# nh2/housescan

Hardware: AMD Instinct MI355X
Metric: frames/sec fused (640x480 into 512^3 TSDF): integrate+ICP+raycast (higher is better)
Workload: dtype f32 (int16 fixed-point TSDF storage, f64 ICP sums)

## Files before the change

### housescan_amd/_lib.py

```python
import ctypes as C
import importlib.util
import os
import sys

_HERE = os.path.dirname(os.path.abspath(__file__))
LIB_PATH = os.path.join(_HERE, "libhskinfu.so")

HSK_LEVELS = 3
HSK_NSTAGES = 4
HSK_KEY_NONE = 0x7FFFFFFF


class HskConfig(C.Structure):

    _fields_ = [
        ("vol_x", C.c_int), ("vol_y", C.c_int), ("vol_z", C.c_int),
        ("vol_size_m", C.c_float * 3),
        ("trunc_dist_m", C.c_float),
        ("width", C.c_int), ("height", C.c_int),
        ("fx", C.c_float), ("fy", C.c_float), ("cx", C.c_float), ("cy", C.c_float),
        ("icp_iters", C.c_int * HSK_LEVELS),
        ("icp_dist_thresh_m", C.c_float),
        ("icp_angle_thresh_sin", C.c_float),
        ("integrate_move_thresh", C.c_float),
# ... 35 lines not shown
        ("clip", (C.c_float * 4) * HSK_MAX_CLIP),
        ("cut_rgb", C.c_uint8 * 3),
    ]


class HskFuseStats(C.Structure):

    _fields_ = [
        ("n_fused", C.c_uint64), ("n_colored", C.c_uint64),
        ("chunks_total", C.c_uint64), ("chunks_swept", C.c_uint64),
        ("box", C.c_int32 * 6),
    ]


HSK_ALIGN_CONVERGED, HSK_ALIGN_MAX_ITERS, HSK_ALIGN_FEW, HSK_ALIGN_DEGENERATE, HSK_ALIGN_DIVERGED = 0, 1, 2, 3, 4
HSK_ALIGN_STATUS = ("converged", "max_iters", "few", "degenerate", "diverged")
HSK_ALIGN_MAX_ITERS_CAP = 64
HSK_ALIGN_DIRECT = -1


class HskAlignParams(C.Structure):

    _fields_ = [
        ("max_iters", C.c_int), ("probes", C.c_int),
        ("cos_gate", C.c_float),
        ("max_points", C.c_uint32), ("min_points", C.c_uint32),
        ("eps_rot", C.c_float), ("eps_trans_m", C.c_float), ("max_rot", C.c_float), ("max_shift_m", C.c_float),
    ]


class HskAlignStats(C.Structure):

    _fields_ = [
        ("status", C.c_int), ("iterations", C.c_int),
        ("n_points", C.c_uint32), ("stride", C.c_uint32),
        ("n_used", C.c_uint32 * HSK_ALIGN_MAX_ITERS_CAP),
        ("rms_m", C.c_float * HSK_ALIGN_MAX_ITERS_CAP),
        ("x_last", C.c_float * 6),
        ("sums_last", C.c_double * 28),
    ]


class HskVolumeInfo(C.Structure):

    _fields_ = [
        ("version", C.c_uint32), ("header_bytes", C.c_uint32), ("flags", C.c_uint32),
        ("dims", C.c_int32 * 3), ("z0", C.c_int32), ("nz", C.c_int32),
        ("size_m", C.c_float * 3),
        ("trunc_dist_m", C.c_float), ("trunc_eff_m", C.c_float),
        ("width", C.c_int32), ("height", C.c_int32),
        ("fx", C.c_float), ("fy", C.c_float), ("cx", C.c_float), ("cy", C.c_float),
        ("pose", C.c_float * 16),
        ("frame", C.c_int32),
        ("color_max_weight", C.c_int32), ("color_band_m", C.c_float),
        ("n_bricks", C.c_uint64),
        ("tsdf_bricks", C.c_uint64 * 4), ("color_bricks", C.c_uint64 * 2),
        ("tsdf_table_bytes", C.c_uint64), ("tsdf_payload_bytes", C.c_uint64),
        ("color_table_bytes", C.c_uint64), ("color_payload_bytes", C.c_uint64),
        ("total_bytes", C.c_uint64),
        ("pass_reused", C.c_int32),
    ]


_P = C.c_void_p
_F = C.POINTER(C.c_float)
_D = C.POINTER(C.c_double)
_I = C.POINTER(C.c_int)
SYMBOLS = {
    "hsk_build_id": (C.c_char_p, []),
    "hsk_default_config": (None, [C.POINTER(HskConfig), C.c_int]),
    "hsk_create": (C.c_int, [C.POINTER(HskConfig), C.POINTER(_P)]),
    "hsk_destroy": (None, [_P]),
    "hsk_reset": (C.c_int, [_P]),
    "hsk_last_error": (C.c_char_p, [_P]),
    "hsk_process_frame": (C.c_int, [_P, _P, C.c_int, C.c_int, _F, _I]),
    "hsk_process_frame_dev": (C.c_int, [_P, _P, C.c_int, C.c_int, _F, _I]),
    "hsk_submit_frame_dev": (C.c_int, [_P, _P, C.c_int, C.c_int]),
    "hsk_submit_frame": (C.c_int, [_P, _P, C.c_int, C.c_int]),
    "hsk_wait_frame": (C.c_int, [_P, _F, _I]),
    "hsk_integrate": (C.c_int, [_P, _P, C.c_int, C.c_int, _F]),
    "hsk_raycast": (C.c_int, [_P, _F, _P, _P, _P]),
    "hsk_preprocess": (C.c_int, [_P, _P, C.c_int, C.c_int]),
    "hsk_icp_accumulate": (C.c_int, [_P, C.c_int, _F, C.c_int, C.c_int, _D]),
    "hsk_icp_solve": (C.c_int, [_D, _F, _I]),
    "hsk_count_updates": (C.c_int, [_P, _P, C.c_int, C.c_int, _F, C.POINTER(C.c_uint64)]),
    "hsk_download_tsdf": (C.c_int, [_P, _P]),
    "hsk_upload_tsdf": (C.c_int, [_P, _P]),
    "hsk_flush_weights": (C.c_int, [_P]),
    "hsk_prepare_readout": (C.c_int, [_P, C.c_size_t]),
    "hsk_stored_planes": (C.c_int, [_P, _I, _I]),
    "hsk_get_pose": (C.c_int, [_P, _F]),
    "hsk_set_pose": (C.c_int, [_P, _F]),
    "hsk_download_map": (C.c_int, [_P, C.c_int, C.c_int, _P]),
    "hsk_upload_map": (C.c_int, [_P, C.c_int, C.c_int, _P]),
    "hsk_download_depth_level": (C.c_int, [_P, C.c_int, _P]),
    "hsk_download_scaled_depth": (C.c_int, [_P, _P]),
    "hsk_extract_cloud": (C.c_int, [_P, _P, C.c_size_t, C.POINTER(C.c_size_t)]),
    "hsk_extract_mesh": (C.c_int, [_P, _P, C.c_size_t, C.POINTER(C.c_size_t)]),
    "hsk_extract_mesh_cubes": (C.c_int, [_P, _P, C.c_size_t, C.POINTER(C.c_size_t)]),
    "hsk_enable_color": (C.c_int, [_P, C.c_int, C.c_float]),
    "hsk_process_frame_rgbd": (C.c_int, [_P, _P, _P, C.c_int, C.c_int, _F, _I]),
    "hsk_submit_frame_rgbd": (C.c_int, [_P, _P, _P, C.c_int, C.c_int]),
    "hsk_integrate_color": (C.c_int, [_P, _P, _P, C.c_int, C.c_int, _F]),
    "hsk_download_color": (C.c_int, [_P, _P]),
    "hsk_upload_color": (C.c_int, [_P, _P]),
    "hsk_extract_cloud_attrs": (C.c_int, [_P, _P, _P, _P, C.c_size_t, C.POINTER(C.c_size_t), C.POINTER(C.c_size_t)]),
    "hsk_extract_mesh_indexed": (C.c_int, [_P, _P, _P, _P, C.c_size_t, C.POINTER(C.c_size_t), _P, C.c_size_t, C.POINTER(C.c_size_t),
                                            C.POINTER(C.c_size_t)]),
    "hsk_default_view": (None, [_P, C.POINTER(HskView)]),
    "hsk_render_view": (C.c_int, [_P, C.POINTER(HskView), _P, _P, _P, _P, C.POINTER(C.c_size_t), C.POINTER(C.c_size_t)]),
    "hsk_default_section": (None, [_P, C.POINTER(HskSection)]),
    "hsk_render_section": (C.c_int, [_P, C.POINTER(HskSection), _P, _P, _P, _P, C.POINTER(C.c_size_t), C.POINTER(C.c_size_t),
                                      C.POINTER(C.c_size_t)]),
    "hsk_section_in_room": (C.c_int, [C.POINTER(HskSection), _F, C.POINTER(HskSection)]),
    "hsk_composite_views": (C.c_int, [C.c_int, C.POINTER(_P), C.POINTER(_P), C.c_int, C.c_int, _P, _P, _P, _P]),
    "hsk_fuse_volume": (C.c_int, [_P, _P, _F, C.POINTER(HskFuseStats)]),
    "hsk_pack_volume": (C.c_int, [_P, _P, C.c_size_t, C.POINTER(C.c_size_t), C.POINTER(HskVolumeInfo)]),
    "hsk_unpack_volume": (C.c_int, [_P, _P, C.c_size_t]),
    "hsk_save_volume": (C.c_int, [_P, C.c_char_p, C.POINTER(HskVolumeInfo)]),
    "hsk_load_volume": (C.c_int, [_P, C.c_char_p]),
    "hsk_volume_image_info": (C.c_int, [_P, C.c_size_t, C.POINTER(HskVolumeInfo)]),
    "hsk_volume_file_info": (C.c_int, [C.c_char_p, C.POINTER(HskVolumeInfo)]),
    "hsk_config_from_volume": (C.c_int, [C.POINTER(HskVolumeInfo), C.POINTER(HskConfig)]),
    "hsk_resume_scan": (C.c_int, [_P, _F]),
    "hsk_default_align_params": (None, [_P, C.POINTER(HskAlignParams)]),
    "hsk_align_cloud": (C.c_int, [_P, _P, _P, C.c_size_t, _F, C.POINTER(HskAlignParams), _F, C.POINTER(HskAlignStats)]),
    "hsk_align_volume": (C.c_int, [_P, _P, _F, C.POINTER(HskAlignParams), _F, C.POINTER(HskAlignStats)]),
    "hsk_align_step": (C.c_int, [_D, _F, _F, _F, _F, _I]),
    "hsk_invert_rigid": (C.c_int, [_F, _F]),
    "hsk_fuse_footprint": (C.c_int, [_I, _F, _I, _F, _F, C.POINTER(C.c_int32)]),
    "hsk_write_ppm": (C.c_int, [C.c_char_p, _P, C.c_int, C.c_int]),
    "hsk_write_pgm16": (C.c_int, [C.c_char_p, _P, C.c_int, C.c_int]),
    "hsk_mgpu_frame_begin": (C.c_int, [_P, _P, C.c_int, C.c_int]),
    "hsk_mgpu_prefetch": (C.c_int, [_P, _P, C.c_int, C.c_int]),
    "hsk_mgpu_frame_front": (C.c_int, [_P, _P, C.c_int, C.c_int, _P]),
    "hsk_mgpu_icp_accumulate": (C.c_int, [_P, C.c_int, C.c_int, C.c_int, _P]),
    "hsk_mgpu_icp_update": (C.c_int, [_P, _P]),
    "hsk_mgpu_icp_replicated": (C.c_int, [_P]),
    "hsk_mgpu_integrate": (C.c_int, [_P]),
    "hsk_mgpu_raycast_local": (C.c_int, [_P, _P]),
    "hsk_mgpu_raycast_resolve": (C.c_int, [_P, _P, _P]),
    "hsk_mgpu_raycast_push": (C.c_int, [_P, _P, C.POINTER(_P), C.c_int]),
    "hsk_mgpu_frame_end": (C.c_int, [_P, _P, _P, _F, _I]),
    "hsk_mgpu_frame_index": (C.c_int, [_P]),
    "hsk_mgpu_frame_end_async": (C.c_int, [_P, _P, _P]),
    "hsk_mgpu_restart_pending": (C.c_int, [_P]),
    "hsk_stream": (_P, [_P]),
    "hsk_set_stream": (C.c_int, [_P, _P]),
    "hsk_synchronize": (C.c_int, [_P]),
    "hsk_set_profiling": (C.c_int, [_P, C.c_int]),
    "hsk_stage_ms": (C.c_int, [_P, _D, C.POINTER(C.c_uint64), C.c_int]),
    "hsk_icp_level_ms": (C.c_int, [_P, _D]),
    "hsk_submit_host_us": (C.c_int, [_P, _D, C.POINTER(C.c_uint64), C.c_int]),
    "hsk_integrate_queue_entries": (C.c_int, [_P, C.POINTER(C.c_uint64)]),
    "hsk_integrate_light_entries": (C.c_int, [_P, C.POINTER(C.c_uint64)]),
    "hsk_integrate_coarse_counts": (C.c_int, [_P, C.POINTER(C.c_uint64)]),
    "hsk_bilateral_tables": (C.c_int, [_F, _F]),
    "hsk_selftest_exact_ops": (C.c_int, [C.c_int, C.POINTER(C.c_uint64)]),
    "hsk_group_create": (C.c_int, [C.POINTER(HskConfig), C.c_int, _I, C.c_int, C.POINTER(_P)]),
    "hsk_group_unique_id": (C.c_int, [_P]),
    "hsk_group_create_rank": (C.c_int, [C.POINTER(HskConfig), C.c_int, C.c_int, _P, C.c_int, C.POINTER(_P)]),
    "hsk_group_destroy": (None, [_P]),
    "hsk_group_last_error": (C.c_char_p, [_P]),
    "hsk_group_reset": (C.c_int, [_P]),
    "hsk_group_process_frame": (C.c_int, [_P, _P, C.c_int, C.c_int, _F, _I]),
    "hsk_group_submit_frame": (C.c_int, [_P, _P, C.c_int, C.c_int]),
    "hsk_group_submit_frame_dev": (C.c_int, [_P, C.POINTER(_P), C.c_int, C.c_int]),
    "hsk_group_wait_frame": (C.c_int, [_P, _F, _I]),
    "hsk_group_exchange_ms": (C.c_int, [_P, _D, _D, C.POINTER(C.c_ulonglong)]),
    "hsk_group_n_slabs": (C.c_int, [_P]),
    "hsk_group_ranks_seen": (C.c_int, [_P, _I]),
    "hsk_group_slab": (_P, [_P, C.c_int]),
    "hsk_group_download_tsdf": (C.c_int, [_P, _P]),
    "hsk_synth_pose": (C.c_int, [C.c_int, _F]),
    "hsk_synth_render": (C.c_int, [_F, C.c_int, C.c_int, C.c_float, C.c_float, C.c_float, C.c_float, _P]),
    "hsk_synth_room_extents": (C.c_int, [C.c_int, _F]),
    "hsk_synth_room_pose": (C.c_int, [C.c_int, C.c_int, C.c_int, _F]),
    "hsk_synth_room_render": (C.c_int, [C.c_int, _F, C.c_int, C.c_int, C.c_float, C.c_float, C.c_float, C.c_float, _P]),
    "hsk_synth_render_sensor": (C.c_int, [C.c_int, _F, C.c_int, C.c_int, C.c_float, C.c_float, C.c_float, C.c_float, C.c_uint64, C.c_float, C.c_float, C.c_int, _P, _D]),
    "hsk_synth_color_at": (C.c_int, [C.c_int, _F, _P]),
    "hsk_synth_render_rgb": (C.c_int, [C.c_int, _F, C.c_int, C.c_int, C.c_float, C.c_float, C.c_float, C.c_float, _P]),
    "hsk_write_pcd_xyz": (C.c_int, [C.c_char_p, _P, C.c_size_t]),
    "hsk_write_ply_mesh": (C.c_int, [C.c_char_p, _P, C.c_size_t, C.POINTER(C.c_size_t), C.POINTER(C.c_size_t)]),
    "hsk_weld_triangles": (C.c_int, [_P, C.c_size_t, _P, C.c_size_t, C.POINTER(C.c_size_t), _P]),
    "hsk_write_ply_indexed": (C.c_int, [C.c_char_p, _P, _P, _P, C.c_size_t, _P, C.c_size_t]),
    "hsk_voxel_downsample": (C.c_int, [_P, C.c_size_t, C.c_float, _P, C.c_size_t, C.POINTER(C.c_size_t)]),
    "hsk_voxel_downsample_attrs": (C.c_int, [_P, _P, _P, C.c_size_t, C.c_float, _P, _P, _P, C.c_size_t, C.POINTER(C.c_size_t)]),
    "hsk_write_pcd_xyzrgbnormal": (C.c_int, [C.c_char_p, _P, _P, _P, C.c_size_t]),
    "hsk_detect_planes": (C.c_int, [_P, C.c_size_t, C.c_float, C.c_float, C.c_int, C.c_int, _P, _P, _I]),
    "hsk_plane_hull": (C.c_int, [_P, C.c_size_t, _P, C.c_int, _F, _P, C.c_size_t, C.POINTER(C.c_size_t)]),
    "hsk_write_planes_txt": (C.c_int, [C.c_char_p, _P, C.c_int]),
    "hsk_write_xf": (C.c_int, [C.c_char_p, _F]),
    "hsk_read_xf": (C.c_int, [C.c_char_p, _F]),
    "hsk_transform_cloud": (C.c_int, [_P, C.c_size_t, _F, _P]),
    "hsk_transform_normals": (C.c_int, [_P, C.c_size_t, _F, _P]),
    "hsk_stream_create": (_P, [C.c_char_p, C.c_int, C.c_int, C.c_float, C.c_float, C.c_float, C.c_float]),
    "hsk_stream_open": (_P, [C.c_char_p, _I, _I, _I, _F]),
    "hsk_stream_write": (C.c_int, [_P, _P]),
    "hsk_stream_read": (C.c_int, [_P, C.c_int, _P]),
    "hsk_stream_close": (C.c_int, [_P]),
    "hsk_stream_info": (C.c_int, [_P, _I, _I, _I, _F]),
    "hsk_track_stream": (C.c_int, [_P, _P, C.c_int, C.c_int, _F, _I]),
}

_U32 = C.POINTER(C.c_uint32)
_SZ = C.POINTER(C.c_size_t)
HSH_OBJECTIVE = C.CFUNCTYPE(C.c_double, _D, C.c_int, _P)
HOUSE_SYMBOLS = {
    "hsh_create": (_P, []),
    "hsh_destroy": (None, [_P]),
    "hsh_last_error": (C.c_char_p, [_P]),
    "hsh_load_room": (C.c_int, [_P, C.c_char_p, _U32]),
    "hsh_add_room": (C.c_int, [_P, C.c_char_p, _P, C.c_size_t, _P, C.c_int, _P, _P, _U32]),
    "hsh_room_ids": (C.c_int, [_P, _P, C.c_int, _I]),
    "hsh_room_planes": (C.c_int, [_P, C.c_uint32, _P, _P, C.c_int, _I]),
    "hsh_plane_bounds": (C.c_int, [_P, C.c_uint32, _P, C.c_int, _I]),
    "hsh_room_corners": (C.c_int, [_P, C.c_uint32, C.c_int, _P, _P, C.c_int, _I]),
    "hsh_room_cloud": (C.c_int, [_P, C.c_uint32, _P, C.c_size_t, _SZ]),
    "hsh_room_means": (C.c_int, [_P, C.c_uint32, _P, _P]),
    "hsh_set_room_corners": (C.c_int, [_P, C.c_uint32, _P, C.c_int]),
    "hsh_accept_corner_suggestion": (C.c_int, [_P, C.c_uint32, C.c_uint32]),
    "hsh_translate_room": (C.c_int, [_P, C.c_uint32, _P]),
    "hsh_rotate_room": (C.c_int, [_P, C.c_uint32, _P]),
    "hsh_rotate_kinfu_room": (C.c_int, [_P, C.c_uint32]),
    "hsh_room_auto_align_axis": (C.c_int, [_P, C.c_uint32, _P]),
    "hsh_auto_align_floor": (C.c_int, [_P, C.c_uint32]),
    "hsh_remove_ceiling": (C.c_int, [_P, C.c_uint32]),
    "hsh_suggest_points": (C.c_int, [_P, C.c_uint32, C.c_float, _I, _I]),
    "hsh_fit_cuboid_to_room": (C.c_int, [_P, C.c_uint32, C.c_int, _I, _D, _D]),
    "hsh_connect_walls": (C.c_int, [_P, C.c_uint32, C.c_uint32, C.c_int, C.c_float, _I]),
    "hsh_disconnect_walls": (C.c_int, [_P, C.c_uint32, C.c_uint32]),
    "hsh_connected_walls": (C.c_int, [_P, _P, _P, _P, _P, _P, C.c_int, _I]),
    "hsh_optimize_room_positions": (C.c_int, [_P, _D]),
    "hsh_room_projection": (C.c_int, [_P, C.c_uint32, _F]),
    "hsh_room_projection_string": (C.c_int, [_P, C.c_uint32, C.c_int, C.c_char_p, C.c_size_t]),
    "hsh_export_all_room_xf_files": (C.c_int, [_P, C.c_char_p]),
    "hsh_plane_corner": (C.c_int, [_P, _P, _I]),
    "hsh_fit_plane": (C.c_int, [_P, C.c_int, _P]),
    "hsh_rotation_between": (C.c_int, [_P, _P, _P]),
    "hsh_cuboid_from_params": (C.c_int, [_P, _P]),
    "hsh_guess_dims": (C.c_int, [_P, _P]),
    "hsh_errfun": (C.c_int, [_P, _P, C.c_int, _D]),
    "hsh_fit_cuboid": (C.c_int, [_P, C.c_int, C.c_int, _P, _I, _D]),
    "hsh_nm_minimize": (C.c_int, [HSH_OBJECTIVE, _P, C.c_int, _P, _P, C.c_double, C.c_int, _P, _D, _I]),
    "hsh_lstsq_distances": (C.c_int, [_P, _P, _P, C.c_int, _P, _P, C.c_int, _I, _D]),
    "hsh_group_connected_components": (C.c_int, [_P, _P, C.c_int, _P, _I]),
    "hsh_show_float": (C.c_int, [C.c_float, C.c_char_p, C.c_size_t]),
    "hsh_read_pcd_xyz": (C.c_int, [C.c_char_p, _P, C.c_size_t, _SZ]),
    "hsh_read_planes_txt": (C.c_int, [C.c_char_p, _P, C.c_int, _I]),
    "hsh_write_ply_points": (C.c_int, [C.c_char_p, _P, C.c_size_t]),
    "hsh_read_ply_points": (C.c_int, [C.c_char_p, _P, C.c_size_t, _SZ]),
}

_lib = None


def _share_torch_hip_runtime():
    if "torch" in sys.modules:
        return
    try:
        spec = importlib.util.find_spec("torch")
    except (ImportError, ValueError):
        spec = None
    if spec is None or not spec.origin:
        return
    path = os.path.join(os.path.dirname(spec.origin), "lib", "libamdhip64.so")
    if os.path.exists(path):
        try:
            C.CDLL(path, mode=C.RTLD_GLOBAL)
        except OSError:
            return
        rccl = os.path.join(os.path.dirname(spec.origin), "lib", "librccl.so")
        if os.path.exists(rccl):
            os.environ.setdefault("HSK_RCCL_PATH", rccl)


def load():
    global _lib
    if _lib is not None:
        return _lib
    _share_torch_hip_runtime()
    if not os.path.exists(LIB_PATH):
        raise ImportError(
            f"{LIB_PATH} is missing: build it with `make -C housescan_amd/csrc` "
            "(or `python -c 'import __graft_entry__ as g; g.build()'`). There is no CPU fallback.")
    lib = C.CDLL(LIB_PATH)
    for name, (res, args) in list(SYMBOLS.items()) + list(HOUSE_SYMBOLS.items()):
        fn = getattr(lib, name)
        fn.restype = res
        fn.argtypes = args
    _lib = lib
    return lib
```

### housescan_amd/csrc/hsk_ctx.h

```cpp
#pragma once
#include <hip/hip_runtime.h>

#include <cstdio>
#include <cstring>
#include <string>

#include "../../include/hskinfu.h"
#include "hsk_dev.h"
#include "hsk_launch.h"
#include "hsk_volume_image.h"

struct ImgBufs {
  uint16_t* d_raw = nullptr;
  uint16_t* d_dep[HSK_NLEVELS] = {};
  float* d_scaled = nullptr;
  float* d_vcur[HSK_NLEVELS] = {};
  float* d_ncur[HSK_NLEVELS] = {};
  float* d_tmax = nullptr;
  unsigned char* d_rgb = nullptr;
};

struct hsk_ctx {
  hsk_config cfg;
  hipStream_t stream = nullptr;
  bool own_stream = false;
  VolParams vp;
  ImgLevel lv[HSK_NLEVELS];
  float init_R[9], init_t[3];
  void* d_vol = nullptr;
  size_t vol_bytes = 0;
  ImgBufs ib[2];
  int cur = 0;
  ImgBufs& B() { return ib[cur]; }
  float* d_vmod[HSK_NLEVELS] = {};
  float* d_nmod[HSK_NLEVELS] = {};
  TrackState* d_st = nullptr;
  TrackState* h_st = nullptr;
  double* d_partials = nullptr;
  double* d_partials2 = nullptr;
  void* d_icp_pose = nullptr;
  double* d_sums = nullptr;
  float h_ws[169] = {};
  float* d_wc = nullptr;
  int* d_keys = nullptr;
  unsigned* d_flags = nullptr;
  unsigned char* d_uni = nullptr;
  size_t uni_bytes = 0;
  bool weights_pending = false;
  size_t flags_bytes = 0;
  unsigned* d_queue = nullptr;
  CubeTable* d_cube_tab = nullptr;
  int2* d_zint = nullptr;
  uint16_t* h_stage = nullptr;
  unsigned stage_turn = 0;
  unsigned long long* d_counter = nullptr;
  unsigned* d_rowcnt = nullptr;
  unsigned long long* d_rowoff = nullptr;
  uint64_t vol_epoch = 1;
  int ro_kind = 0;
  uint64_t ro_epoch = 0;
  unsigned long long ro_totals[2] = {0, 0};
  void* d_out = nullptr;
  size_t out_bytes = 0;
  void* h_pin[2] = {nullptr, nullptr};
  size_t pin_bytes = 0;
  hipEvent_t ev_pin[2] = {};
  int frame = 0;
  std::string err;
  TrackState* h_ring = nullptr;
  int* h_slot_fifo = nullptr;
  unsigned* d_ring_seq = nullptr;
  unsigned ring_seq = 0;
  unsigned ring_expect[HSK_MAX_IN_FLIGHT + 1] = {};
  unsigned set_expect[2] = {0, 0};
  int set_slot[2] = {-1, -1};
  TrackState* d_ring_view = nullptr;
  int* d_fifo_view = nullptr;
  hipEvent_t ring_ev[HSK_MAX_IN_FLIGHT + 1] = {};
  int ring_kind[HSK_MAX_IN_FLIGHT + 1] = {};
  int ring_head = 0, ring_count = 0;
  bool pending_reset = false;
  hipStream_t pstream = nullptr;
  hipEvent_t ev_pre[2] = {}, ev_free[2] = {};
  hipEvent_t ev_src = nullptr;

  bool set_used[2] = {false, false};
  int async_set = 1;
  const void* pf_ptr = nullptr;
  int pf_set = -1;
  int mgpu_set = 0;
  hipGraph_t sgraph[2] = {};
  hipGraphExec_t sgexec[2] = {};
  void* sgraph_keys = nullptr;
  hipGraph_t graph = nullptr;
  hipGraphExec_t gexec = nullptr;
  bool graph_ready = false;
  hipGraph_t pgraph[2] = {};
  hipGraphExec_t pgexec[2] = {};
  bool prof = false;
  bool prof_levels = false;
  hipEvent_t ev[HSK_NSTAGES + 1] = {};
  hipEvent_t ev_icp[HSK_NLEVELS + 1] = {};
  double icp_level_ms[HSK_NLEVELS] = {};
  double stage_ms[HSK_NSTAGES] = {};
  double submit_us[4] = {};
  unsigned long long submit_n = 0;
  uint64_t prof_frames = 0;
  unsigned* d_color = nullptr;
  size_t color_bytes = 0;
  int* d_has_color = nullptr;
  unsigned char* h_rgb_stage = nullptr;
  const unsigned char* rgb_src = nullptr;
  int color_max_w = 0;
  bool group_slab = false;
  float color_band = 0.0f;
  void* d_mi = nullptr;
  size_t mi_bytes = 0;
  void* d_view = nullptr;
  void* h_view = nullptr;
  void* d_fuse = nullptr;
  size_t fuse_bytes = 0;
  void* d_align = nullptr;
  size_t align_bytes = 0;
  unsigned long long* h_align = nullptr;
  void* d_pack = nullptr;
  uint64_t pk_epoch = 0;
  bool pk_color = false;
  unsigned pk_counts[16] = {};
};

#define HIPCHK(k, call)                                                                        \
  do {                                                                                         \
    hipError_t e_ = (call);                                                                    \
    if (e_ != hipSuccess) {                                                                    \
      char buf_[512];                                                                          \
      snprintf(buf_, sizeof(buf_), "%s failed: %s (%s:%d)", #call, hipGetErrorString(e_), __FILE__, __LINE__); \
      (k)->err = buf_;                                                                         \
      return HSK_ERR_HIP;                                                                      \
    }                                                                                          \
  } while (0)

std::string& create_error();
int fail(hsk_ctx* k, int code, const char* msg);
void pose16_to_rt(const float m[16], float R[9], float t[3]);
void rt_to_pose16(const float R[9], const float t[3], float m[16]);
void flush_weights(hsk_ctx* k);
int upload_state(hsk_ctx* k);
int download_state(hsk_ctx* k);
void leave_slab_bookkeeping(hsk_ctx* k);
int set_pose_internal(hsk_ctx* k, const float pose[16]);
void enqueue_raycast_and_resize(hsk_ctx* k, int* keys, bool report = false);
void hsk_mark_group_slab(hsk_ctx* k);
int require_idle(const hsk_ctx* k, hsk_ctx* errs);
inline int require_idle(hsk_ctx* k) { return require_idle(k, k); }
int require_color(hsk_ctx* k);
int require_whole_volume(const hsk_ctx* k, hsk_ctx* errs, const char* who, const char* sentence = "a context that stores part of its volume");
int ensure_pinned(hsk_ctx* k);
void parallel_memcpy(void* dst, const void* src, size_t bytes);
int copy_out(hsk_ctx* k, void* dst, const void* src_dev, size_t bytes);
int ensure_product_bytes(hsk_ctx* k, size_t want, bool headroom = true);
int read_u64(hsk_ctx* k, unsigned long long* dst, const unsigned long long* src_dev, int n = 1);
struct ProductLayout {
  size_t bytes = 0;
  size_t take(size_t n) {
    const size_t at = bytes;
    bytes += (n + 255) & ~(size_t)255;
    return at;
  }
};
```

### housescan_amd/csrc/hsk_launch.h

```cpp
#pragma once
#include "hsk_dev.h"
#include "hsk_icp_dev.h"

void launch_integrate(hipStream_t s, void* vol, const float* scaled, const TrackState* st, const VolParams& vp, int W,
                      int H, Intr in, bool count_only, unsigned long long* counter, unsigned* flags,
                      const float* tmax, int2* zint, unsigned* queue, const IcpFinal* icp_final = nullptr,
                      unsigned char* uni = nullptr, const RingOut* early = nullptr);
size_t uniform_bytes(const VolParams& vp);
size_t uniform_lane_bytes(const VolParams& vp);
void launch_rebuild_uniform(hipStream_t s, const void* vol, const VolParams& vp, unsigned char* uni);
void launch_materialize(hipStream_t s, void* vol, const VolParams& vp, unsigned char* uni);
size_t integrate_queue_words(const VolParams& vp);
size_t integrate_queue_counter_words();
unsigned long long integrate_queue_entries(const unsigned* counter_words);
unsigned long long integrate_queue_light_entries(const unsigned* counter_words);
size_t integrate_cflag_offset_bytes(const VolParams& vp);
size_t integrate_chunk_count(const VolParams& vp);
size_t integrate_zint_entries(const VolParams& vp);
void launch_tile_max(hipStream_t s, const float* scaled, int W, int H, float* tmax);
void launch_tile_fine(hipStream_t s, const float* scaled, int W, int H, float* tiles);
void launch_tile_tables(hipStream_t s, int W, int H, float* tiles);
size_t tile_table_bytes(int W, int H);
void launch_rebuild_flags(hipStream_t s, const void* vol, const VolParams& vp, unsigned* flags);
void launch_vol_to_linear(hipStream_t s, const void* vol, const VolParams& vp, int zz0, int nz, void* lin);
void launch_vol_from_linear(hipStream_t s, void* vol, const VolParams& vp, int zz0, int nz, const void* lin);
void launch_raycast(hipStream_t s, const void* vol, const TrackState* st, const VolParams& vp, int W, int H, Intr in,
                    float* vmap, float* nmap, int* keys, const unsigned* flags, const MapPyramid* pyramid = nullptr,
                    const RingOut* ring = nullptr);
bool raycast_can_fuse_pyramid(const VolParams& vp, int W, int H);
struct ViewCam {
  float R[9], t[3];
};
#define HSK_VIEW_COUNT_SLOTS 64
void launch_render_view(hipStream_t s, const void* vol, const unsigned* colv, const ViewCam* cam, const VolParams& vp, int W, int H,
                        Intr in, const unsigned* flags, int mode, const float light[3], int light_in_camera,
                        const unsigned char background[3], unsigned char* rgb, unsigned short* depth, float* vmap, float* nmap,
                        unsigned long long* counts);
int view_warm();
struct SectionPlane {
  float a, b, c, d;
};
struct SectionClip {
  int projection, n_clip;
  SectionPlane plane[4];
};
void launch_render_section(hipStream_t s, const void* vol, const unsigned* colv, const ViewCam* cam, const VolParams& vp, int W, int H,
                           Intr in, const unsigned* flags, int mode, const float light[3], int light_in_camera, int light_directional,
                           const unsigned char background[3], const unsigned char cut_rgb[3], const SectionClip& clip,
                           unsigned char* rgb, unsigned short* depth, float* vmap, float* nmap, unsigned long long* counts);
int section_warm();
void launch_resolve(hipStream_t s, const int* keys_local, const int* keys_min, const float* vmap, const float* nmap,
                    int* bits, int P);
void launch_adopt_pyramid(hipStream_t s, const int* keys_min, const int* bits, int W, int H, float* v0, float* n0, float* v1, float* n1,
                          float* v2, float* n2, const TrackState* st, const RingOut* ring);
void launch_resolve_push(hipStream_t s, const int* keys_local, const int* keys_min, const float* vmap, const float* nmap,
                         const PushDests& dst, int P);
int extract_warm();
void launch_extract(hipStream_t s, const void* vol, const VolParams& vp, unsigned* row_count,
                    unsigned long long* row_offset, unsigned long long* total, float* xyz, unsigned long long cap,
                    const unsigned* flags);
size_t hsk_scan_scratch_entries(int nrows);
void launch_extract_attrs(hipStream_t s, const void* vol, const unsigned* colv, const VolParams& vp, const unsigned* row_count,
                          const unsigned long long* row_offset, float* xyz, float* normals, unsigned char* rgb,
                          unsigned long long cap, unsigned long long* n_uncolored, const unsigned* flags);
void launch_color_integrate(hipStream_t s, unsigned* col, const TrackState* st, const int* has_color, const float* scaled,
                            const unsigned char* rgb, const float* tiles, const VolParams& vp, int W, int H, Intr in, float band,
                            int max_w);
size_t fuse_table_words(const VolParams& sv);
void launch_fuse_bricks(hipStream_t s, const void* src_vol, const VolParams& sv, unsigned* tab);
void launch_fuse_sweep(hipStream_t s, const void* src_vol, const unsigned* src_col, void* dst_vol, unsigned* dst_col, const VolParams& sv,
                       const VolParams& dv, const float A[9], const float b[3], const int box[6], const unsigned* tab, int max_w,
                       unsigned long long* counts, unsigned long long* chunks_total);

#define HSK_ALIGN_SHARDS 16
#define HSK_ALIGN_ACC_WORDS (HSK_ALIGN_SHARDS * 32)
struct AlignPose {
  float R[9], t[3];
};
void launch_align_iter(hipStream_t s, const void* dst_vol, const VolParams& dv, const float* soa, unsigned n, unsigned pitch,
                       const AlignPose& m, int probes, float cos_gate, unsigned long long* acc);

size_t pack_bricks(const VolParams& vp);
size_t pack_scan_blocks(size_t n_bricks);
void launch_pack_classify(hipStream_t s, const void* vol, const VolParams& vp, unsigned char* cls, unsigned* size);
void launch_pack_classify_color(hipStream_t s, const unsigned* col, const VolParams& vp, unsigned char* cls, unsigned* size);
void launch_pack_sizes(hipStream_t s, const unsigned char* cls, size_t n_bricks, unsigned* size);
void launch_pack_scan(hipStream_t s, unsigned* size, size_t n_bricks, unsigned* bsum, unsigned* counts);
void launch_pack_gather(hipStream_t s, const void* vol, bool color, const VolParams& vp, const unsigned char* cls, const unsigned* off,
                        void* payload);
void launch_pack_scatter(hipStream_t s, void* vol, bool color, const VolParams& vp, const unsigned char* cls, const unsigned* off,
                         const void* payload);

void launch_bilateral_scale(hipStream_t s, const uint16_t* src, int W, int H, Intr in, const float* ws, const float* wc,
                            uint16_t* dst, float* scaled, float* tiles);
void launch_scale_depth(hipStream_t s, const uint16_t* src, int W, int H, Intr in, float* scaled);
void launch_pyrdown(hipStream_t s, const uint16_t* src, int W, int H, uint16_t* dst);
void launch_vmap_nmap_pyramid(hipStream_t s, uint16_t* const* depth, const ImgLevel* lv, float* const* vmap,
                              float* const* nmap);
void launch_pyramid_maps(hipStream_t s, uint16_t* const* depth, const ImgLevel* lv, float* const* vmap, float* const* nmap);
void launch_transform_maps(hipStream_t s, const float* vs, const float* ns, int P, const TrackState* st, float* vd,
                           float* nd);
void launch_resize_maps2(hipStream_t s, const float* v0, const float* n0, int W, int H, float* v1, float* n1, float* v2,
                         float* n2, const TrackState* st,
                         const RingOut* ring = nullptr);
int icp_num_blocks(int W, int rows);
void launch_icp_accumulate(hipStream_t s, const float* vcur, const float* ncur, const float* vprev, const float* nprev,
                           int W, int H, Intr in, const TrackState* st, float dist_thresh, float angle_thresh, int row0,
                           int row1, double* partials);
void launch_icp_reduce(hipStream_t s, const double* partials, int nblocks, double* out27);
void launch_icp_update(hipStream_t s, const double* sums27, TrackState* st);
void launch_begin_frame(hipStream_t s, TrackState* st, void* icp_pose_buf);
size_t icp_pose_bytes();
void launch_icp_fused(hipStream_t s, float* const* vcur, float* const* ncur, float* const* vmod, float* const* nmod,
                      const ImgLevel* lv, const int* iters, TrackState* st, float dist_thresh, float angle_thresh,
                      void* pose_buf, double* part_a, double* part_b, IcpFinal* defer_final = nullptr,
                      hipEvent_t* level_events = nullptr);
bool host_solve6(const double* in27, float* x6);
void host_pose_update(float* R, float* t, const float* x6);
void hsk_build_tet_table(TetTable* tt);
int hsk_build_cube_table(CubeTable* ct);
int hsk_mesh_z_end(const VolParams& vp);
void launch_extract_mesh(hipStream_t s, const void* vol, const VolParams& vp, const TetTable& tt, unsigned* row_count,
                         unsigned long long* row_offset, unsigned long long* total, float* tri, unsigned long long cap, const unsigned* flags);
void launch_extract_mesh_mc(hipStream_t s, const void* vol, const VolParams& vp, const CubeTable* ct_dev, unsigned* row_count,
                            unsigned long long* row_offset, unsigned long long* total, float* tri, unsigned long long cap, const unsigned* flags);
struct MeshIndexBufs {
  int rows;
  int nseg;
  unsigned long long* totals;
  unsigned long long* bits;
  unsigned long long* voff;
  unsigned* vcount;
  unsigned short* segbase;
};
size_t mesh_index_layout(const VolParams& vp, void* base , MeshIndexBufs* b);
void launch_mesh_index_count(hipStream_t s, const void* vol, const VolParams& vp, const CubeTable* ct_dev, unsigned* row_count,
                             unsigned long long* row_offset, const MeshIndexBufs& mb, const unsigned* flags);
void launch_mesh_index_write(hipStream_t s, const void* vol, const unsigned* colv, const VolParams& vp, const CubeTable* ct_dev,
                             const unsigned* row_count, const unsigned long long* row_offset, const MeshIndexBufs& mb, float* xyz,
                             float* normals, unsigned char* rgb, unsigned long long* n_uncolored, int* faces, const unsigned* flags);
```

### housescan_amd/csrc/hskinfu_api.hip

```cpp
#pragma clang fp contract(off)
#include <sched.h>

#include <chrono>
#include <cmath>
#include <cstdlib>

#include "hsk_ctx.h"

#include "build/build_id.h"
extern "C" const char* hsk_build_id(void) { return HSK_BUILD_ID; }

std::string& create_error() {
  static thread_local std::string err;
  return err;
}

int fail(hsk_ctx* k, int code, const char* msg) {
  if (k) k->err = msg;
  return code;
}
int require_idle(const hsk_ctx* k, hsk_ctx* errs) {
  return k->ring_count > 0 ? fail(errs, HSK_ERR_STATE, "frames are in flight: collect them with hsk_wait_frame first") : HSK_OK;
}
int require_color(hsk_ctx* k) { return k->d_color ? HSK_OK : fail(k, HSK_ERR_STATE, "colour is not enabled (hsk_enable_color)"); }
int require_whole_volume(const hsk_ctx* k, hsk_ctx* errs, const char* who, const char* sentence) {
  if (!k->group_slab && k->vp.zs0 == 0 && k->vp.nzs == k->vp.Z && k->vp.zo0 == 0 && k->vp.zo1 == k->vp.Z) return HSK_OK;
  return fail(errs, HSK_ERR_STATE, (std::string(who) + ": not for a slab (" + sentence + ")").c_str());
}

void pose16_to_rt(const float m[16], float R[9], float t[3]) {
  for (int i = 0; i < 3; ++i) {
    R[i * 3] = m[i * 4];
    R[i * 3 + 1] = m[i * 4 + 1];
    R[i * 3 + 2] = m[i * 4 + 2];
    t[i] = m[i * 4 + 3];
  }
}
void rt_to_pose16(const float R[9], const float t[3], float m[16]) {
  for (int i = 0; i < 3; ++i) {
    m[i * 4] = R[i * 3];
    m[i * 4 + 1] = R[i * 3 + 1];
    m[i * 4 + 2] = R[i * 3 + 2];
    m[i * 4 + 3] = t[i];
  }
  m[12] = m[13] = m[14] = 0.0f;
  m[15] = 1.0f;
}

extern "C" void hsk_default_config(hsk_config* c, int n) {
  memset(c, 0, sizeof(*c));
  c->vol_x = c->vol_y = c->vol_z = n;
  c->vol_size_m[0] = c->vol_size_m[1] = c->vol_size_m[2] = 3.0f;
  c->trunc_dist_m = 0.03f;
  c->width = 640;
  c->height = 480;
  c->fx = c->fy = 525.0f;
  c->cx = 319.5f;
  c->cy = 239.5f;
  c->icp_iters[0] = 10;
  c->icp_iters[1] = 5;
  c->icp_iters[2] = 4;
  c->icp_dist_thresh_m = 0.10f;
  c->icp_angle_thresh_sin = 0.3420201433256687f;
  c->integrate_move_thresh = 0.0f;
  float R[9] = {1, 0, 0, 0, 1, 0, 0, 0, 1};
  float t[3] = {c->vol_size_m[0] / 2.0f, c->vol_size_m[1] / 2.0f, c->vol_size_m[2] / 2.0f - 1.2f * c->vol_size_m[2] / 2.0f};
  rt_to_pose16(R, t, c->init_pose);
  c->device_id = 0;
  c->own_z0 = 0;
  c->own_z1 = n;
  c->halo = 0;
  c->use_graph = 0;
}

extern "C" int hsk_bilateral_tables(float ws[169], float wc[512]) {
  const float sig_s = 4.5f, sig_c = 30.0f;
  const float s2 = 0.5f / (sig_s * sig_s);
  const float c2 = 0.5f / (sig_c * sig_c);
  for (int dy = -6; dy <= 6; ++dy)
    for (int dx = -6; dx <= 6; ++dx) {
      const float arg = (float)(dx * dx + dy * dy) * s2;
      ws[(dy + 6) * 13 + (dx + 6)] = (float)std::exp(-(double)arg);
    }
  for (int k = 0; k < 512; ++k) {
    const float arg = (float)(k * k) * c2;
    wc[k] = (float)std::exp(-(double)arg);
  }
  return HSK_OK;
}

static void free_all(hsk_ctx* k) {
  if (!k) return;
  (void)hipSetDevice(k->cfg.device_id);
  if (k->gexec) (void)hipGraphExecDestroy(k->gexec);
  if (k->graph) (void)hipGraphDestroy(k->graph);
  for (auto& g : k->pgexec)
    if (g) (void)hipGraphExecDestroy(g);
  for (auto& g : k->pgraph)
    if (g) (void)hipGraphDestroy(g);
  for (auto& g : k->sgexec)
    if (g) (void)hipGraphExecDestroy(g);
  for (auto& g : k->sgraph)
    if (g) (void)hipGraphDestroy(g);
  for (auto& e : k->ev_pre)
    if (e) (void)hipEventDestroy(e);
  for (auto& e : k->ev_free)
    if (e) (void)hipEventDestroy(e);
  if (k->ev_src) (void)hipEventDestroy(k->ev_src);
  if (k->pstream) (void)hipStreamDestroy(k->pstream);
  auto F = [](void* p) {
    if (p) (void)hipFree(p);
  };
  F(k->d_vol);
  for (auto& b : k->ib) {
    F(b.d_raw);
    F(b.d_scaled);
    F(b.d_tmax);
    for (int l = 0; l < HSK_NLEVELS; ++l) {
      F(b.d_dep[l]);
      F(b.d_vcur[l]);
      F(b.d_ncur[l]);
    }
  }
  for (int l = 0; l < HSK_NLEVELS; ++l) {
    F(k->d_vmod[l]);
    F(k->d_nmod[l]);
  }
  F(k->d_st);
  F(k->d_partials);
  F(k->d_partials2);
  F(k->d_icp_pose);
  F(k->d_sums);
  F(k->d_wc);
  F(k->d_keys);
  F(k->d_flags);
  F(k->d_uni);
  F(k->d_zint);
  F(k->d_queue);
  F(k->d_cube_tab);
  F(k->d_counter);
  F(k->d_rowcnt);
  F(k->d_rowoff);
  F(k->d_out);
  F(k->d_color);
  F(k->d_has_color);
  F(k->d_mi);
  F(k->d_view);
  F(k->d_fuse);
  F(k->d_pack);
  F(k->d_align);
  if (k->h_align) (void)hipHostFree(k->h_align);
  if (k->h_view) (void)hipHostFree(k->h_view);
  for (auto& b : k->ib) F(b.d_rgb);
  if (k->h_rgb_stage) (void)hipHostFree(k->h_rgb_stage);
  for (auto& p : k->h_pin)
    if (p) (void)hipHostFree(p);
  for (auto& e : k->ev_pin)
    if (e) (void)hipEventDestroy(e);
  if (k->h_st) (void)hipHostFree(k->h_st);
  if (k->h_stage) (void)hipHostFree(k->h_stage);
  if (k->h_ring) (void)hipHostFree(k->h_ring);
  if (k->h_slot_fifo) (void)hipHostFree(k->h_slot_fifo);
  if (k->d_ring_seq) (void)hipFree(k->d_ring_seq);
  for (auto& e : k->ring_ev)
    if (e) (void)hipEventDestroy(e);
  for (auto& e : k->ev)
    if (e) (void)hipEventDestroy(e);
  for (auto& e : k->ev_icp)
    if (e) (void)hipEventDestroy(e);
  if (k->own_stream && k->stream) (void)hipStreamDestroy(k->stream);
}

void flush_weights(hsk_ctx* k) {
  if (!k->weights_pending) return;
  launch_materialize(k->stream, k->d_vol, k->vp, k->d_uni);
  k->weights_pending = false;
}

int upload_state(hsk_ctx* k) {
  HIPCHK(k, hipMemcpyAsync(k->d_st, k->h_st, sizeof(TrackState), hipMemcpyHostToDevice, k->stream));
  HIPCHK(k, hipStreamSynchronize(k->stream));
  return HSK_OK;
}
int download_state(hsk_ctx* k) {
  HIPCHK(k, hipMemcpyAsync(k->h_st, k->d_st, sizeof(TrackState), hipMemcpyDeviceToHost, k->stream));
  HIPCHK(k, hipStreamSynchronize(k->stream));
  return HSK_OK;
}

static int do_reset(hsk_ctx* k) {
  HIPCHK(k, hipSetDevice(k->cfg.device_id));
  HIPCHK(k, hipMemsetAsync(k->d_vol, 0, k->vol_bytes, k->stream));
  HIPCHK(k, hipMemsetAsync(k->d_flags, 0, k->flags_bytes, k->stream));
  HIPCHK(k, hipMemsetAsync(k->d_uni, 1, uniform_lane_bytes(k->vp), k->stream));
  HIPCHK(k, hipMemsetAsync(k->d_uni + uniform_lane_bytes(k->vp), 0, k->uni_bytes - uniform_lane_bytes(k->vp), k->stream));
  if (k->d_color) HIPCHK(k, hipMemsetAsync(k->d_color, 0, k->color_bytes, k->stream));
  memset(k->h_st, 0, sizeof(TrackState));
  memcpy(k->h_st->R, k->init_R, sizeof(k->init_R));
  memcpy(k->h_st->t, k->init_t, sizeof(k->init_t));
  memcpy(k->h_st->Rp, k->init_R, sizeof(k->init_R));
  memcpy(k->h_st->tp, k->init_t, sizeof(k->init_t));
  k->frame = 0;
  k->vol_epoch += 1;
  k->pending_reset = false;
  return upload_state(k);
}

extern "C" int hsk_create(const hsk_config* c, hsk_ctx** out) {
  if (!c || !out) {
    create_error() = "hsk_create: null argument";
    return HSK_ERR_ARG;
  }
  *out = nullptr;
  if (c->vol_x <= 0 || c->vol_y <= 0 || c->vol_z <= 0 || (c->vol_x % 8) != 0 || (c->vol_y % 8) != 0 || c->width <= 0 || c->height <= 0 ||
      (c->width % 4) != 0 || (c->height % 4) != 0 || c->own_z0 < 0 || c->own_z1 > c->vol_z || c->own_z0 >= c->own_z1 ||
      c->halo < 0) {
    create_error() = "hsk_create: invalid configuration (vol_x, vol_y must be multiples of 8, image dims of 4; 0 <= own_z0 < own_z1 <= vol_z)";
    return HSK_ERR_ARG;
  }
  int ndev = 0;
  if (hipGetDeviceCount(&ndev) != hipSuccess || ndev <= 0) {
    create_error() = "hsk_create: no HIP device available (this library has no CPU fallback)";
    return HSK_ERR_NOGPU;
  }
  if (c->device_id < 0 || c->device_id >= ndev) {
    create_error() = "hsk_create: device_id out of range";
    return HSK_ERR_ARG;
  }
  hsk_ctx* k = new hsk_ctx();
  k->cfg = *c;
  auto bail = [&](int code) {
    create_error() = k->err;
    free_all(k);
    delete k;
    return code;
  };
#define CK(call)                                   \
  do {                                             \
    int r_ = [&]() -> int {                        \
      HIPCHK(k, call);                             \
      return HSK_OK;                               \
    }();                                           \
    if (r_ != HSK_OK) return bail(r_);             \
  } while (0)
  CK(hipSetDevice(c->device_id));
  CK(hipStreamCreateWithFlags(&k->stream, hipStreamNonBlocking));
  k->own_stream = true;
  VolParams& vp = k->vp;
  vp.X = c->vol_x;
  vp.Y = c->vol_y;
  vp.Z = c->vol_z;
  vp.zo0 = c->own_z0;
  vp.zo1 = c->own_z1;
  vp.zs0 = c->own_z0 - c->halo < 0 ? 0 : c->own_z0 - c->halo;
  const int zs1 = c->own_z1 + c->halo > c->vol_z ? c->vol_z : c->own_z1 + c->halo;
  vp.nzs = zs1 - vp.zs0;
  for (int i = 0; i < 3; ++i) vp.size[i] = c->vol_size_m[i];
  vp.cell[0] = vp.size[0] / (float)vp.X;
  vp.cell[1] = vp.size[1] / (float)vp.Y;
  vp.cell[2] = vp.size[2] / (float)vp.Z;
  for (int a = 0; a < 3; ++a) vp.icell[a] = 1.0 / (double)vp.cell[a];
  vp.stream_nt = 0;
  vp.zchunk = 8;
  float m = vp.cell[0] > vp.cell[1] ? vp.cell[0] : vp.cell[1];
  m = m > vp.cell[2] ? m : vp.cell[2];
  const float lo = 2.1f * m;
  vp.tau = c->trunc_dist_m > lo ? c->trunc_dist_m : lo;
  vp.tau_inv = 1.0f / vp.tau;
  for (int l = 0; l < HSK_NLEVELS; ++l) {
    const float s = (float)(1 << l);
    k->lv[l].W = c->width >> l;
    k->lv[l].H = c->height >> l;
    k->lv[l].in = Intr{c->fx / s, c->fy / s, c->cx / s, c->cy / s};
  }
  pose16_to_rt(c->init_pose, k->init_R, k->init_t);
  k->vol_bytes = hsk_vol_words(vp) * 4;
  vp.stream_nt = k->vol_bytes > ((size_t)1 << 30) ? 1 : 0;
  vp.zchunk = hsk_pass_a_zchunk(vp.X, vp.Y, vp.nzs);
  CK(hipMalloc(&k->d_vol, k->vol_bytes));
  const size_t P0 = (size_t)c->width * c->height;
  for (auto& b : k->ib) {
    CK(hipMalloc((void**)&b.d_raw, P0 * 2));
    CK(hipMalloc((void**)&b.d_scaled, P0 * 4));
    CK(hipMalloc((void**)&b.d_tmax, tile_table_bytes(c->width, c->height)));
    CK(hipMemset(b.d_tmax, 0, tile_table_bytes(c->width, c->height)));
    for (int l = 0; l < HSK_NLEVELS; ++l) {
      const size_t P = (size_t)k->lv[l].W * k->lv[l].H;
      CK(hipMalloc((void**)&b.d_dep[l], P * 2));
      CK(hipMalloc((void**)&b.d_vcur[l], P * 12));
      CK(hipMalloc((void**)&b.d_ncur[l], P * 12));
    }
  }
  for (int l = 0; l < HSK_NLEVELS; ++l) {
    const size_t P = (size_t)k->lv[l].W * k->lv[l].H;
    CK(hipMalloc((void**)&k->d_vmod[l], P * 12));
    CK(hipMalloc((void**)&k->d_nmod[l], P * 12));
  }
  {
    int lo = 0, hi = 0;
    bool made = false;
    if (hipDeviceGetStreamPriorityRange(&lo, &hi) == hipSuccess && lo != hi)
      made = hipStreamCreateWithPriority(&k->pstream, hipStreamNonBlocking, lo) == hipSuccess;
    if (!made) {
      (void)hipGetLastError();
      CK(hipStreamCreateWithFlags(&k->pstream, hipStreamNonBlocking));
    }
  }
  for (auto& e : k->ev_pre) CK(hipEventCreateWithFlags(&e, hipEventDisableTiming));
  for (auto& e : k->ev_free) CK(hipEventCreateWithFlags(&e, hipEventDisableTiming));
  CK(hipEventCreateWithFlags(&k->ev_src, hipEventDisableTiming));

  CK(hipMalloc((void**)&k->d_st, sizeof(TrackState)));
  CK(hipHostMalloc((void**)&k->h_st, sizeof(TrackState), hipHostMallocDefault));
  CK(hipHostMalloc((void**)&k->h_stage, P0 * 2 * (HSK_MAX_IN_FLIGHT + 1), hipHostMallocDefault));
  CK(hipHostMalloc((void**)&k->h_ring, sizeof(TrackState) * (HSK_MAX_IN_FLIGHT + 1), hipHostMallocDefault));
  CK(hipHostMalloc((void**)&k->h_slot_fifo, sizeof(int) * HSK_RING_FIFO, hipHostMallocDefault));
  memset(k->h_slot_fifo, 0, sizeof(int) * HSK_RING_FIFO);
  CK(hipHostGetDevicePointer((void**)&k->d_ring_view, k->h_ring, 0));
  CK(hipHostGetDevicePointer((void**)&k->d_fifo_view, k->h_slot_fifo, 0));
  CK(hipMalloc((void**)&k->d_ring_seq, sizeof(unsigned)));
  CK(hipMemset(k->d_ring_seq, 0, sizeof(unsigned)));
  for (auto& e : k->ring_ev) CK(hipEventCreateWithFlags(&e, hipEventDisableTiming));
  const int nb0 = icp_num_blocks(c->width, c->height);
  CK(hipMalloc((void**)&k->d_partials, (size_t)nb0 * 27 * sizeof(double)));
  CK(hipMalloc((void**)&k->d_partials2, (size_t)nb0 * 27 * sizeof(double)));
  CK(hipMalloc(&k->d_icp_pose, icp_pose_bytes()));
  CK(hipMemset(k->d_icp_pose, 0, icp_pose_bytes()));
  CK(hipMalloc((void**)&k->d_sums, 27 * sizeof(double)));
  CK(hipMalloc((void**)&k->d_wc, 512 * 4));
  CK(hipMalloc((void**)&k->d_keys, P0 * 4));
  vp.bshift = 3;
  while (hsk_flag_words(vp) > HSK_FLAG_WORDS_MAX && vp.bshift < 6 && ((vp.X >> (vp.bshift + 1)) << (vp.bshift + 1)) == vp.X &&
         ((vp.Y >> (vp.bshift + 1)) << (vp.bshift + 1)) == vp.Y)
    ++vp.bshift;
  if ((size_t)((vp.nzs + 3) / 4) * vp.Y * (vp.X / 4) >= ((size_t)1 << 28)) {
    k->err = "hsk_create: volume too large for the 28-bit lane-block ids of integrate (more than 2^32 stored voxels)";
    return bail(HSK_ERR_ARG);
  }
  k->flags_bytes = (size_t)hsk_flag_words_total(vp) * 4;
  if (k->flags_bytes > 64u * 1024u) {
    k->err = "hsk_create: the brick bitfield of this volume does not fit the raycast's LDS (64 KiB): choose vol_x, vol_y divisible by a larger power of two";
    return bail(HSK_ERR_ARG);
  }
  CK(hipMalloc((void**)&k->d_flags, k->flags_bytes));
  k->uni_bytes = uniform_bytes(vp);
  CK(hipMalloc((void**)&k->d_uni, k->uni_bytes));
  CK(hipMalloc((void**)&k->d_queue, integrate_queue_words(vp) * sizeof(unsigned)));
  CK(hipMalloc((void**)&k->d_zint, integrate_zint_entries(vp) * sizeof(int2)));
  CK(hipMalloc((void**)&k->d_counter, 16));
  {
    float ws[169], wc[512];
    hsk_bilateral_tables(ws, wc);
    memcpy(k->h_ws, ws, sizeof(ws));
    CK(hipMemcpy(k->d_wc, wc, sizeof(wc), hipMemcpyHostToDevice));
  }
  for (auto& e : k->ev) CK(hipEventCreate(&e));
  for (auto& e : k->ev_icp) CK(hipEventCreate(&e));
#undef CK
  int r = do_reset(k);
  if (r != HSK_OK) return bail(r);
  *out = k;
  return HSK_OK;
}

static int wait_slot(hsk_ctx* k, int slot, bool pose_only = false);
static int reset_behind_lost_frame(hsk_ctx* k);
extern "C" int hsk_wait_frame(hsk_ctx* k, float pose_out[16], int* tracked);

extern "C" void hsk_destroy(hsk_ctx* k) {
  if (!k) return;
  if (k->pstream) (void)hipStreamSynchronize(k->pstream);
  if (k->stream) (void)hipStreamSynchronize(k->stream);
  free_all(k);
  delete k;
}

extern "C" int hsk_reset(hsk_ctx* k) {
  return k ? reset_behind_lost_frame(k) : HSK_ERR_ARG;
}

extern "C" const char* hsk_last_error(const hsk_ctx* k) { return k ? k->err.c_str() : create_error().c_str(); }

extern "C" void* hsk_stream(hsk_ctx* k) { return k ? (void*)k->stream : nullptr; }
extern "C" int hsk_set_stream(hsk_ctx* k, void* stream) {
  if (!k) return HSK_ERR_ARG;
  HIPCHK(k, hipSetDevice(k->cfg.device_id));
  if (k->stream) HIPCHK(k, hipStreamSynchronize(k->stream));
  if (k->own_stream && k->stream) (void)hipStreamDestroy(k->stream);
  k->stream = (hipStream_t)stream;
  k->own_stream = false;
  return HSK_OK;
}
extern "C" int hsk_synchronize(hsk_ctx* k) {
  if (!k) return HSK_ERR_ARG;
  HIPCHK(k, hipStreamSynchronize(k->stream));
  return HSK_OK;
}

static void enqueue_preprocess(hsk_ctx* k, hipStream_t s) {
  launch_bilateral_scale(s, k->B().d_raw, k->lv[0].W, k->lv[0].H, k->lv[0].in, k->h_ws, k->d_wc, k->B().d_dep[0], k->B().d_scaled,
                         k->B().d_tmax);
  launch_tile_tables(s, k->lv[0].W, k->lv[0].H, k->B().d_tmax);
  launch_pyramid_maps(s, k->B().d_dep, k->lv, k->B().d_vcur, k->B().d_ncur);
}

static void enqueue_icp(hsk_ctx* k, IcpFinal* fin = nullptr) {
  if (fin) *fin = IcpFinal{nullptr, nullptr, 0};
  launch_icp_fused(k->stream, k->B().d_vcur, k->B().d_ncur, k->d_vmod, k->d_nmod, k->lv, k->cfg.icp_iters, k->d_st,
                   k->cfg.icp_dist_thresh_m, k->cfg.icp_angle_thresh_sin, k->d_icp_pose, k->d_partials, k->d_partials2, fin,
                   (k->prof && k->prof_levels && !fin) ? k->ev_icp : nullptr);
}

static void enqueue_integrate(hsk_ctx* k, const IcpFinal* fin = nullptr, bool report_early = false) {
  k->weights_pending = true;
  k->vol_epoch += 1;
  const RingOut ring = {k->d_ring_view, k->d_fifo_view, k->d_ring_seq};
  launch_integrate(k->stream, k->d_vol, k->B().d_scaled, k->d_st, k->vp, k->lv[0].W, k->lv[0].H, k->lv[0].in, false,
                   k->d_counter, k->d_flags, k->B().d_tmax, k->d_zint, k->d_queue, (fin && fin->slots) ? fin : nullptr,
                   k->d_uni, report_early ? &ring : nullptr);
}

static void enqueue_color(hsk_ctx* k) {
  if (!k->d_color) return;
  launch_color_integrate(k->stream, k->d_color, k->d_st, k->d_has_color + k->cur, k->B().d_scaled, k->B().d_rgb, k->B().d_tmax, k->vp,
                         k->lv[0].W, k->lv[0].H, k->lv[0].in, k->color_band, k->color_max_w);
}

void enqueue_raycast_and_resize(hsk_ctx* k, int* keys, bool report) {
  hipStream_t s = k->stream;
  const RingOut ring = {k->d_ring_view, k->d_fifo_view, k->d_ring_seq};
  const RingOut* rp = report ? &ring : nullptr;
  if (raycast_can_fuse_pyramid(k->vp, k->lv[0].W, k->lv[0].H)) {
    const MapPyramid pyr = {k->d_vmod[1], k->d_nmod[1], k->d_vmod[2], k->d_nmod[2]};
    launch_raycast(s, k->d_vol, k->d_st, k->vp, k->lv[0].W, k->lv[0].H, k->lv[0].in, k->d_vmod[0], k->d_nmod[0], keys, k->d_flags,
                   &pyr, rp);
    return;
  }
  launch_raycast(s, k->d_vol, k->d_st, k->vp, k->lv[0].W, k->lv[0].H, k->lv[0].in, k->d_vmod[0], k->d_nmod[0], keys, k->d_flags,
                 nullptr, rp);
  launch_resize_maps2(s, k->d_vmod[0], k->d_nmod[0], k->lv[0].W, k->lv[0].H, k->d_vmod[1], k->d_nmod[1], k->d_vmod[2],
                      k->d_nmod[2], k->d_st);
}

static bool gate_passes(const TrackState* st, float thr) {
  if (!(thr > 0.0f)) return true;
  const float* a = st->R;
  const float* b = st->Rp;
  const float c0 = (a[0] * b[0] + a[3] * b[3]) + a[6] * b[6];
  const float c1 = (a[1] * b[1] + a[4] * b[4]) + a[7] * b[7];
  const float c2 = (a[2] * b[2] + a[5] * b[5]) + a[8] * b[8];
  float cs = (((c0 + c1) + c2) - 1.0f) / 2.0f;
  if (cs > 1.0f) cs = 1.0f;
  if (cs < -1.0f) cs = -1.0f;
  const float turn = acosf(cs);
  const float ex = st->t[0] - st->tp[0], ey = st->t[1] - st->tp[1], ez = st->t[2] - st->tp[2];
  const float shift = sqrtf((ex * ex + ey * ey) + ez * ez);
  return (turn + shift) / 2.0f >= thr;
}

static void enqueue_tracked_frame(hsk_ctx* k, bool with_events) {
  hipStream_t s = k->stream;
  if (with_events) (void)hipEventRecord(k->ev[0], s);
  enqueue_preprocess(k, k->stream);
  if (with_events) (void)hipEventRecord(k->ev[1], s);
  enqueue_icp(k);
  if (with_events) (void)hipEventRecord(k->ev[2], s);
  enqueue_integrate(k);
  enqueue_color(k);
  if (with_events) (void)hipEventRecord(k->ev[3], s);
  enqueue_raycast_and_resize(k, nullptr);
  if (with_events) (void)hipEventRecord(k->ev[4], s);
}

static void enqueue_tracked_rest(hsk_ctx* k) {
  IcpFinal fin;
  enqueue_icp(k, &fin);
  enqueue_integrate(k, &fin, true);
  enqueue_color(k);
  enqueue_raycast_and_resize(k, nullptr, true);
}

static int hand_back(const hsk_ctx* k, float pose_out[16], int* tracked, int verdict) {
  if (pose_out) rt_to_pose16(k->h_st->R, k->h_st->t, pose_out);
  if (tracked) *tracked = verdict;
  return HSK_OK;
}
static int end_tracked_frame(hsk_ctx* k, float pose_out[16], int* tracked) {
  if (k->h_st->lost) {
    const int r = do_reset(k);
    return r != HSK_OK ? r : hand_back(k, pose_out, tracked, 0);
  }
  k->frame += 1;
  return hand_back(k, pose_out, tracked, 1);
}

static int frame_common(hsk_ctx* k, float pose_out[16], int* tracked) {
  hipStream_t s = k->stream;
  const bool gated = k->cfg.integrate_move_thresh > 0.0f;
  if (k->frame == 0) {
    enqueue_preprocess(k, k->stream);
    enqueue_integrate(k);
    enqueue_color(k);
    for (int l = 0; l < HSK_NLEVELS; ++l)
      launch_transform_maps(s, k->B().d_vcur[l], k->B().d_ncur[l], k->lv[l].W * k->lv[l].H, k->d_st, k->d_vmod[l], k->d_nmod[l]);
    int r = download_state(k);
    if (r != HSK_OK) return r;
    HIPCHK(k, hipGetLastError());
    k->frame = 1;
    return hand_back(k, pose_out, tracked, 0);
  }
  if (gated) {
    enqueue_preprocess(k, k->stream);
    enqueue_icp(k);
    int r = download_state(k);
    if (r != HSK_OK) return r;
    if (!k->h_st->lost) {
      if (gate_passes(k->h_st, k->cfg.integrate_move_thresh)) {
        enqueue_integrate(k);
        enqueue_color(k);
      }
      enqueue_raycast_and_resize(k, nullptr);
    }
  } else if (k->prof) {
    enqueue_tracked_frame(k, true);
  } else if (k->cfg.use_graph == 1) {
    if (!k->graph_ready) {
      HIPCHK(k, hipStreamBeginCapture(s, hipStreamCaptureModeThreadLocal));
      enqueue_tracked_frame(k, false);
      HIPCHK(k, hipStreamEndCapture(s, &k->graph));
      HIPCHK(k, hipGraphInstantiate(&k->gexec, k->graph, nullptr, nullptr, 0));
      k->graph_ready = true;
    }
    HIPCHK(k, hipGraphLaunch(k->gexec, s));
    k->weights_pending = true;
    k->vol_epoch += 1;
  } else {
    enqueue_tracked_frame(k, false);
  }
  int r = download_state(k);
  if (r != HSK_OK) return r;
  HIPCHK(k, hipGetLastError());
  if (k->prof && !gated) {
    for (int i = 0; i < HSK_NSTAGES; ++i) {
      float ms = 0.0f;
      if (hipEventElapsedTime(&ms, k->ev[i], k->ev[i + 1]) == hipSuccess) k->stage_ms[i] += ms;
    }
    for (int i = 0; i < HSK_NLEVELS && k->prof_levels; ++i) {
      float ms = 0.0f;
      if (hipEventElapsedTime(&ms, k->ev_icp[i], k->ev_icp[i + 1]) == hipSuccess) k->icp_level_ms[HSK_NLEVELS - 1 - i] += ms;
    }
    k->prof_frames += 1;
  }
  return end_tracked_frame(k, pose_out, tracked);
}

void leave_slab_bookkeeping(hsk_ctx* k) {
  k->cur = 0;
  k->mgpu_set = 0;
  k->pf_ptr = nullptr;
  k->pf_set = -1;
}

static int check_dims(hsk_ctx* k, const void* depth, int w, int h) {
  if (!k) return HSK_ERR_ARG;
  if (!depth) return fail(k, HSK_ERR_ARG, "depth pointer is null");
  if (w != k->cfg.width || h != k->cfg.height) return fail(k, HSK_ERR_ARG, "depth frame size does not match the context");
  return HSK_OK;
}

static int stage_depth_host(hsk_ctx* k, const uint16_t* depth) {
  const size_t bytes = (size_t)k->cfg.width * k->cfg.height * 2;
  memcpy(k->h_stage, depth, bytes);
// ... 420 lines not shown
  if (k) k->group_slab = true;
}

static void drop_graphs(hsk_ctx* k) {
  if (k->gexec) (void)hipGraphExecDestroy(k->gexec);
  if (k->graph) (void)hipGraphDestroy(k->graph);
  k->gexec = nullptr;
  k->graph = nullptr;
  k->graph_ready = false;
  for (int i = 0; i < 2; ++i) {
    if (k->pgexec[i]) (void)hipGraphExecDestroy(k->pgexec[i]);
    if (k->pgraph[i]) (void)hipGraphDestroy(k->pgraph[i]);
    k->pgexec[i] = nullptr;
    k->pgraph[i] = nullptr;
  }
}

extern "C" int hsk_enable_color(hsk_ctx* k, int max_weight, float band_m) {
  if (!k) return HSK_ERR_ARG;
  if (max_weight < 0 || max_weight > 255) return fail(k, HSK_ERR_ARG, "hsk_enable_color: max_weight must lie in 0..255 (0: 64)");
  if (!(band_m == band_m)) return fail(k, HSK_ERR_ARG, "hsk_enable_color: band_m is NaN");
  if (k->group_slab)
    return fail(k, HSK_ERR_STATE, "hsk_enable_color: colour is not available for the slabs of a group");
  if (int ri = require_idle(k)) return ri;
  HIPCHK(k, hipSetDevice(k->cfg.device_id));
  float m = k->vp.cell[0] > k->vp.cell[1] ? k->vp.cell[0] : k->vp.cell[1];
  m = m > k->vp.cell[2] ? m : k->vp.cell[2];
  float band = band_m > 0.0f ? band_m : 2.0f * m;
  if (band > k->vp.tau) band = k->vp.tau;
  if (!k->d_color) {
    const size_t P0 = (size_t)k->cfg.width * k->cfg.height;
    const size_t bytes = (size_t)k->vp.X * k->vp.Y * (size_t)k->vp.nzs * 4;
    hipError_t e = hipMalloc((void**)&k->d_color, bytes);
    if (e == hipSuccess) e = hipMalloc((void**)&k->d_has_color, 2 * sizeof(int));
    for (auto& b : k->ib)
      if (e == hipSuccess) e = hipMalloc((void**)&b.d_rgb, P0 * 3);
    if (e == hipSuccess) e = hipHostMalloc((void**)&k->h_rgb_stage, P0 * 3, hipHostMallocDefault);
    if (e == hipSuccess) e = hipMemsetAsync(k->d_color, 0, bytes, k->stream);
    if (e == hipSuccess) e = hipMemsetAsync(k->d_has_color, 0, 2 * sizeof(int), k->stream);
    if (e == hipSuccess) e = hipStreamSynchronize(k->stream);
    if (e != hipSuccess) {
      auto F = [](void* p) {
        if (p) (void)hipFree(p);
      };
      F(k->d_color);
      F(k->d_has_color);
      for (auto& b : k->ib) {
        F(b.d_rgb);
        b.d_rgb = nullptr;
      }
      if (k->h_rgb_stage) (void)hipHostFree(k->h_rgb_stage);
      k->d_color = nullptr;
      k->d_has_color = nullptr;
      k->h_rgb_stage = nullptr;
      HIPCHK(k, e);
    }
    k->color_bytes = bytes;
  }
  k->color_max_w = max_weight == 0 ? 64 : max_weight;
  k->color_band = band;
  drop_graphs(k);
  return HSK_OK;
}

static int check_rgb(hsk_ctx* k, const uint8_t* rgb) {
  if (int rc = require_color(k)) return rc;
  if (!rgb) return fail(k, HSK_ERR_ARG, "rgb pointer is null");
  memcpy(k->h_rgb_stage, rgb, (size_t)k->cfg.width * k->cfg.height * 3);
  k->rgb_src = k->h_rgb_stage;
  return HSK_OK;
}

extern "C" int hsk_process_frame_rgbd(hsk_ctx* k, const uint16_t* depth, const uint8_t* rgb, int w, int h, float pose_out[16], int* tracked) {
  int r = check_dims(k, depth, w, h);
  if (r != HSK_OK) return r;
  if (int ri = require_idle(k)) return ri;
  r = check_rgb(k, rgb);
  if (r != HSK_OK) return r;
  r = hsk_process_frame(k, depth, w, h, pose_out, tracked);
  k->rgb_src = nullptr;
  return r;
}

extern "C" int hsk_submit_frame_rgbd(hsk_ctx* k, const uint16_t* depth, const uint8_t* rgb, int w, int h) {
  int r = check_dims(k, depth, w, h);
  if (r != HSK_OK) return r;
  if (k->ring_count >= HSK_MAX_IN_FLIGHT) return fail(k, HSK_ERR_STATE, "too many frames in flight: call hsk_wait_frame first");
  const auto t0 = std::chrono::steady_clock::now();
  r = check_rgb(k, rgb);
  if (r != HSK_OK) return r;
  k->submit_us[0] += std::chrono::duration<double, std::micro>(std::chrono::steady_clock::now() - t0).count();
  r = hsk_submit_frame(k, depth, w, h);
  k->rgb_src = nullptr;
  return r;
}

extern "C" int hsk_integrate_color(hsk_ctx* k, const uint16_t* depth, const uint8_t* rgb, int w, int h, const float pose[16]) {
  int r = check_dims(k, depth, w, h);
  if (r != HSK_OK) return r;
  if (!pose) return fail(k, HSK_ERR_ARG, "pose is null");
  if (int ri = require_idle(k)) return ri;
  r = check_rgb(k, rgb);
  if (r != HSK_OK) return r;
  HIPCHK(k, hipSetDevice(k->cfg.device_id));
  leave_slab_bookkeeping(k);
  r = set_pose_internal(k, pose);
  if (r == HSK_OK) r = stage_depth_host(k, depth);
  if (r != HSK_OK) {
    k->rgb_src = nullptr;
    return r;
  }
  launch_scale_depth(k->stream, k->B().d_raw, w, h, k->lv[0].in, k->B().d_scaled);
  launch_tile_max(k->stream, k->B().d_scaled, w, h, k->B().d_tmax);
  launch_tile_fine(k->stream, k->B().d_scaled, w, h, k->B().d_tmax);
  const hipError_t e = stage_color(k, k->cur, k->stream);
  k->rgb_src = nullptr;
  HIPCHK(k, e);
  enqueue_color(k);
  k->pk_epoch = 0;
  HIPCHK(k, hipStreamSynchronize(k->stream));
  HIPCHK(k, hipGetLastError());
  return HSK_OK;
}

extern "C" int hsk_set_profiling(hsk_ctx* k, int on) {
  if (!k) return HSK_ERR_ARG;
  k->prof = on != 0;
  k->prof_levels = on == 2;
  return HSK_OK;
}
extern "C" int hsk_stage_ms(hsk_ctx* k, double sum_ms[HSK_NSTAGES], uint64_t* n_frames, int reset) {
  if (!k) return HSK_ERR_ARG;
  if (sum_ms)
    for (int i = 0; i < HSK_NSTAGES; ++i) sum_ms[i] = k->stage_ms[i];
  if (n_frames) *n_frames = k->prof_frames;
  if (reset) {
    for (int i = 0; i < HSK_NSTAGES; ++i) k->stage_ms[i] = 0.0;
    for (int i = 0; i < HSK_NLEVELS; ++i) k->icp_level_ms[i] = 0.0;
    k->prof_frames = 0;
  }
  return HSK_OK;
}
extern "C" int hsk_submit_host_us(hsk_ctx* k, double sum_us[4], uint64_t* n_submissions, int reset) {
  if (!k) return HSK_ERR_ARG;
  if (sum_us)
    for (int i = 0; i < 4; ++i) sum_us[i] = k->submit_us[i];
  if (n_submissions) *n_submissions = k->submit_n;
  if (reset) {
    for (auto& v : k->submit_us) v = 0.0;
    k->submit_n = 0;
  }
  return HSK_OK;
}
extern "C" int hsk_icp_level_ms(hsk_ctx* k, double sum_ms[HSK_LEVELS]) {
  if (!k || !sum_ms) return HSK_ERR_ARG;
  for (int i = 0; i < HSK_NLEVELS; ++i) sum_ms[i] = k->icp_level_ms[i];
  return HSK_OK;
}

extern "C" int hsk_mgpu_frame_index(const hsk_ctx* k) { return k ? k->frame : -1; }

extern "C" int hsk_mgpu_prefetch(hsk_ctx* k, const void* depth_dev, int w, int h) {
  int r = check_dims(k, depth_dev, w, h);
  if (r != HSK_OK) return r;
  HIPCHK(k, hipSetDevice(k->cfg.device_id));
  const int set = k->mgpu_set ^ 1;
  if (k->set_used[set]) HIPCHK(k, hipStreamWaitEvent(k->pstream, k->ev_free[set], 0));
  const int keep = k->cur;
  k->cur = set;
  hipError_t e = hipMemcpyAsync(k->B().d_raw, depth_dev, (size_t)w * h * 2, hipMemcpyDefault, k->pstream);
  if (e == hipSuccess) {
    enqueue_preprocess(k, k->pstream);
    e = hipEventRecord(k->ev_pre[set], k->pstream);
  }
  k->cur = keep;
  HIPCHK(k, e);
  k->pf_ptr = depth_dev;
  k->pf_set = set;
  return HSK_OK;
}

extern "C" int hsk_mgpu_frame_begin(hsk_ctx* k, const void* depth_dev, int w, int h) {
  int r = check_dims(k, depth_dev, w, h);
  if (r != HSK_OK) return r;
  HIPCHK(k, hipSetDevice(k->cfg.device_id));
  if (k->pending_reset) {
    r = reset_behind_lost_frame(k);
    if (r != HSK_OK) return r;
  }
  if (k->pf_ptr == depth_dev && k->pf_set >= 0) {
    k->mgpu_set = k->pf_set;
    k->cur = k->mgpu_set;
    HIPCHK(k, hipStreamWaitEvent(k->stream, k->ev_pre[k->mgpu_set], 0));
  } else {
    k->cur = k->mgpu_set;
    HIPCHK(k, hipMemcpyAsync(k->B().d_raw, depth_dev, (size_t)w * h * 2, hipMemcpyDefault, k->stream));
    enqueue_preprocess(k, k->stream);
  }
  k->pf_ptr = nullptr;
  k->pf_set = -1;
  if (k->frame == 0) {
    enqueue_integrate(k);
    for (int l = 0; l < HSK_NLEVELS; ++l)
      launch_transform_maps(k->stream, k->B().d_vcur[l], k->B().d_ncur[l], k->lv[l].W * k->lv[l].H, k->d_st, k->d_vmod[l],
                            k->d_nmod[l]);
  } else {
    launch_begin_frame(k->stream, k->d_st, nullptr);
  }
  return HSK_OK;
}

extern "C" int hsk_mgpu_frame_front(hsk_ctx* k, const void* depth_dev, int w, int h, void* keys_dev) {
  if (!keys_dev) return k ? fail(k, HSK_ERR_ARG, "keys buffer is null") : HSK_ERR_ARG;
  int r = hsk_mgpu_frame_begin(k, depth_dev, w, h);
  if (r != HSK_OK) return r;
  if (k->frame == 0) return HSK_OK;
  const int set = k->cur;
  const size_t P0 = (size_t)k->lv[0].W * k->lv[0].H;
  auto body = [&]() {
    enqueue_icp(k);
    enqueue_integrate(k);
    launch_raycast(k->stream, k->d_vol, k->d_st, k->vp, k->lv[0].W, k->lv[0].H, k->lv[0].in, k->d_vmod[0], k->d_nmod[0], k->d_keys,
                   k->d_flags);
    (void)hipMemcpyAsync(keys_dev, k->d_keys, P0 * 4, hipMemcpyDeviceToDevice, k->stream);
  };
  if (!k->cfg.use_graph || k->stream == nullptr) {
    body();
    HIPCHK(k, hipGetLastError());
    return HSK_OK;
  }
  if (k->sgraph_keys != keys_dev) {
    for (int i = 0; i < 2; ++i) {
      if (k->sgexec[i]) (void)hipGraphExecDestroy(k->sgexec[i]);
      if (k->sgraph[i]) (void)hipGraphDestroy(k->sgraph[i]);
      k->sgexec[i] = nullptr;
      k->sgraph[i] = nullptr;
    }
    k->sgraph_keys = keys_dev;
  }
  if (!k->sgexec[set]) {
    HIPCHK(k, hipStreamBeginCapture(k->stream, hipStreamCaptureModeThreadLocal));
    body();
    HIPCHK(k, hipStreamEndCapture(k->stream, &k->sgraph[set]));
    HIPCHK(k, hipGraphInstantiate(&k->sgexec[set], k->sgraph[set], nullptr, nullptr, 0));
  }
  HIPCHK(k, hipGraphLaunch(k->sgexec[set], k->stream));
  k->weights_pending = true;
  k->vol_epoch += 1;
  return HSK_OK;
}

extern "C" int hsk_mgpu_icp_accumulate(hsk_ctx* k, int level, int row0, int row1, void* sums27_dev) {
  if (!k || !sums27_dev || level < 0 || level >= HSK_NLEVELS) return HSK_ERR_ARG;
  if (row0 < 0 || row1 > k->lv[level].H || row0 > row1) return fail(k, HSK_ERR_ARG, "row range out of bounds");
  if (row0 == row1) {
    HIPCHK(k, hipMemsetAsync(sums27_dev, 0, 27 * sizeof(double), k->stream));
    return HSK_OK;
  }
  const int nb = icp_num_blocks(k->lv[level].W, row1 - row0);
  launch_icp_accumulate(k->stream, k->B().d_vcur[level], k->B().d_ncur[level], k->d_vmod[level], k->d_nmod[level],
                        k->lv[level].W, k->lv[level].H, k->lv[level].in, k->d_st, k->cfg.icp_dist_thresh_m,
                        k->cfg.icp_angle_thresh_sin, row0, row1, k->d_partials);
  launch_icp_reduce(k->stream, k->d_partials, nb, (double*)sums27_dev);
  return HSK_OK;
}

extern "C" int hsk_mgpu_icp_update(hsk_ctx* k, const void* sums27_dev) {
  if (!k || !sums27_dev) return HSK_ERR_ARG;
  launch_icp_update(k->stream, (const double*)sums27_dev, k->d_st);
  return HSK_OK;
}

extern "C" int hsk_mgpu_icp_replicated(hsk_ctx* k) {
  if (!k) return HSK_ERR_ARG;
  if (k->frame == 0) return fail(k, HSK_ERR_STATE, "no model maps yet: the first frame has no ICP");
  enqueue_icp(k);
  return HSK_OK;
}

extern "C" int hsk_mgpu_integrate(hsk_ctx* k) {
  if (!k) return HSK_ERR_ARG;
  enqueue_integrate(k);
  return HSK_OK;
}

extern "C" int hsk_mgpu_raycast_local(hsk_ctx* k, void* keys_dev) {
  if (!k || !keys_dev) return HSK_ERR_ARG;
  launch_raycast(k->stream, k->d_vol, k->d_st, k->vp, k->lv[0].W, k->lv[0].H, k->lv[0].in, k->d_vmod[0], k->d_nmod[0],
                 k->d_keys, k->d_flags);
  HIPCHK(k, hipMemcpyAsync(keys_dev, k->d_keys, (size_t)k->lv[0].W * k->lv[0].H * 4, hipMemcpyDeviceToDevice, k->stream));
  return HSK_OK;
}

extern "C" int hsk_mgpu_raycast_resolve(hsk_ctx* k, const void* keys_min_dev, void* maps_bits_dev) {
  if (!k || !keys_min_dev || !maps_bits_dev) return HSK_ERR_ARG;
  launch_resolve(k->stream, k->d_keys, (const int*)keys_min_dev, k->d_vmod[0], k->d_nmod[0], (int*)maps_bits_dev,
                 k->lv[0].W * k->lv[0].H);
  return HSK_OK;
}

extern "C" int hsk_mgpu_raycast_push(hsk_ctx* k, const void* keys_min_dev, void* const* dest_bits, int n_dest) {
  if (!k || !keys_min_dev || !dest_bits || n_dest < 1 || n_dest > HSK_PUSH_MAX) return HSK_ERR_ARG;
  PushDests d;
  d.n = n_dest;
  for (int i = 0; i < HSK_PUSH_MAX; ++i) d.p[i] = i < n_dest ? (int*)dest_bits[i] : nullptr;
  launch_resolve_push(k->stream, k->d_keys, (const int*)keys_min_dev, k->d_vmod[0], k->d_nmod[0], d, k->lv[0].W * k->lv[0].H);
// ... 51 lines not shown
```

### housescan_amd/csrc/integrate.hip

```cpp
#pragma clang fp contract(off)
#include "hsk_dev.h"
#include "hsk_launch.h"

#define HSK_TILE 16
#define HSK_NQUEUES 256
#define HSK_QCOUNT_STRIDE 64
#define HSK_CF_MIXED 0u
#define HSK_CF_SKIP 1u
#define HSK_CF_FREE 2u
#ifndef INTEGRATE_WPE
#define INTEGRATE_WPE 8
#endif
#ifndef INTEGRATE_WPE_LONG
#define INTEGRATE_WPE_LONG 7
#endif

__global__ void k_tile_max(const float* __restrict__ scaled, int W, int H, float* __restrict__ tmax,
                           float* __restrict__ tmin, int tw, unsigned short* __restrict__ vmask16) {
  __shared__ float shx[4], shn[4];
  const int tx = blockIdx.x, ty = blockIdx.y;
  const int x = tx * HSK_TILE + (threadIdx.x & 15), y = ty * HSK_TILE + (threadIdx.x >> 4);
  const bool in = x < W && y < H;
  const float v = in ? scaled[y * W + x] : 0.0f;
  {
    const unsigned long long inv = __ballot(v == 0.0f);
    if ((threadIdx.x & 63) == 0) {
      const int pitch16 = 2 * hsk_mask_pitch32(W);
#pragma unroll
      for (int r = 0; r < 4; ++r) {
        const int yy = ty * HSK_TILE + (int)(threadIdx.x >> 6) * 4 + r;
        if (yy < H) vmask16[(size_t)yy * pitch16 + tx] = (unsigned short)(inv >> (16 * r));
      }
    }
  }
  float mx = v, mn = v;
#pragma unroll
  for (int o = 32; o > 0; o >>= 1) {
    mx = fmaxf(mx, __shfl_xor(mx, o, 64));
    mn = fminf(mn, __shfl_xor(mn, o, 64));
  }
  if ((threadIdx.x & 63) == 0) {
    shx[threadIdx.x >> 6] = mx;
    shn[threadIdx.x >> 6] = mn;
  }
  __syncthreads();
  if (threadIdx.x == 0) {
    tmax[ty * tw + tx] = fmaxf(fmaxf(shx[0], shx[1]), fmaxf(shx[2], shx[3]));
    tmin[ty * tw + tx] = fminf(fminf(shn[0], shn[1]), fminf(shn[2], shn[3]));
  }
}
void launch_tile_max(hipStream_t s, const float* scaled, int W, int H, float* tiles) {
  const int tw = (W + HSK_TILE - 1) / HSK_TILE, th = (H + HSK_TILE - 1) / HSK_TILE;
  const int n = tw * th;
  hipLaunchKernelGGL(k_tile_max, dim3(tw, th), dim3(256), 0, s, scaled, W, H, tiles, tiles + n, tw, (unsigned short*)(tiles + hsk_tiles_mask_offset(W, H)));
}

#define HSK_FTILE 8
__global__ void k_tile_fine(const float* __restrict__ scaled, int W, int H, float2* __restrict__ ftab, int fw, int fh,
                            float2* __restrict__ qtab) {
  const int t = blockIdx.x * blockDim.x + threadIdx.x;
  if (t >= fw * fh) return;
  const int ty = t / fw, tx = t - ty * fw;
  float mx = 0.0f, mn = 1e30f;
  bool hole = false;
#pragma unroll
  for (int qy = 0; qy < 2; ++qy)
#pragma unroll
    for (int qx = 0; qx < 2; ++qx) {
      float qmx = 0.0f, qmn = 1e30f;
      bool qhole = false;
      for (int dy = 0; dy < 4; ++dy)
        for (int dx = 0; dx < 4; ++dx) {
          const int x = tx * HSK_FTILE + qx * 4 + dx, y = ty * HSK_FTILE + qy * 4 + dy;
          const float v = (x < W && y < H) ? scaled[(size_t)y * W + x] : 0.0f;
          qmx = fmaxf(qmx, v);
          qmn = v != 0.0f ? fminf(qmn, v) : qmn;
          qhole = qhole | (v == 0.0f);
        }
      qtab[(size_t)(2 * ty + qy) * (2 * fw) + (2 * tx + qx)] = make_float2(qmx, qhole ? -qmn : qmn);
      mx = fmaxf(mx, qmx);
      mn = fminf(mn, qmn);
      hole = hole | qhole;
    }
  ftab[t] = make_float2(mx, hole ? -mn : mn);
}


#define HSK_SPARSE_LEVELS 4

__global__ void k_tile_tables(const float* __restrict__ tmax, const float* __restrict__ tmin, int tw, int th, const float2* __restrict__ ftab,
                              const float2* __restrict__ qtab, int fw, int fh, float2* __restrict__ fwin, float2* __restrict__ sparse) {
  const int t = blockIdx.x * blockDim.x + threadIdx.x;
  const int job = blockIdx.y;
  if (job < 18) {
    const bool fine = job >= 9;
    const float2* __restrict__ tab = fine ? qtab : ftab;
    const int tbw = fine ? 2 * fw : fw, tbh = fine ? 2 * fh : fh;
    if (t >= tbw * tbh) return;
    const int shape = fine ? job - 9 : job;
    const int nx = shape % 3 + 1, ny = shape / 3 + 1;
    const int ty = t / tbw, tx = t - ty * tbw;
    float mx = 0.0f, mn = 1e30f;
    bool hole = false;
    for (int a = 0; a < ny; ++a)
      for (int b = 0; b < nx; ++b) {
        const float2 v = tab[min(ty + a, tbh - 1) * tbw + min(tx + b, tbw - 1)];
        mx = fmaxf(mx, v.x);
        mn = fminf(mn, fabsf(v.y));
        hole = hole | (v.y < 0.0f);
      }
    float2* __restrict__ win = fine ? fwin + (size_t)9 * fw * fh : fwin;
    win[(size_t)shape * tbw * tbh + t] = make_float2(mx, hole ? -mn : mn);
  } else {
    if (t >= tw * th) return;
    const int lv = job - 18;
    const int kx = lv % HSK_SPARSE_LEVELS, ky = lv / HSK_SPARSE_LEVELS;
    const int ty = t / tw, tx = t - ty * tw;
    float mx = 0.0f, mn = 1e30f;
    for (int a = ty; a < min(ty + (1 << ky), th); ++a)
      for (int b = tx; b < min(tx + (1 << kx), tw); ++b) {
        mx = fmaxf(mx, tmax[a * tw + b]);
        mn = fminf(mn, tmin[a * tw + b]);
      }
    sparse[(size_t)lv * tw * th + t] = make_float2(mx, mn);
  }
}

static __device__ __forceinline__ void clip_interval(float c, float m, float& lo, float& hi) {
  if (m > 0.0f) {
    lo = fmaxf(lo, -c * __builtin_amdgcn_rcpf(m));
  } else if (m < 0.0f) {
    hi = fminf(hi, -c * __builtin_amdgcn_rcpf(m));
  } else if (c < 0.0f) {
    lo = 1e30f;
    hi = -1e30f;
  }
}

struct CoarseArgs {
  unsigned char* cflag;
  unsigned char* cs;
  const float2* sparse;
  unsigned dirty_off;
  int zchunk;
  float free_thr, cull_thr;
};
__global__ void k_column_zrange(IcpFinal fin, const float* __restrict__ tmax, const float* __restrict__ tmin,
                                float2* __restrict__ dtab, int tw, int th, int dil_blocks, unsigned* __restrict__ qcount,
                                const TrackState* __restrict__ st, VolParams vp, int W, int H, Intr in,
                                int2* __restrict__ zint, TrackState* __restrict__ st_out, int2* __restrict__ wgz, RingOut early,
                                CoarseArgs ca) {
  __shared__ double fin_tot[27];
  __shared__ IcpPose fin_pose;
  double sums_in[16];
  if (fin.slots && threadIdx.x < 64) shard_load27_wave(fin.slots + (size_t)((fin.iter + 2) % 3) * ICP_SLOT_DOUBLES, sums_in);
  {
    if (blockIdx.x == 0)
      for (int q = threadIdx.x; q < HSK_NQUEUES; q += blockDim.x) *(unsigned long long*)&qcount[q * HSK_QCOUNT_STRIDE] = 0ull;
    const int i = blockIdx.x * blockDim.x + threadIdx.x;
    if (i < tw * th && (int)blockIdx.x < dil_blocks) {
      const int ty = i / tw, tx = i - ty * tw;
      float mx = 0.0f, mn = 1e30f;
      for (int dy = -1; dy <= 1; ++dy)
        for (int dx = -1; dx <= 1; ++dx) {
          const int yy = min(max(ty + dy, 0), th - 1), xx = min(max(tx + dx, 0), tw - 1);
          mx = fmaxf(mx, tmax[yy * tw + xx]);
          mn = fminf(mn, tmin[yy * tw + xx]);
        }
      dtab[i] = make_float2(mx, mn);
    }
  }
  if (fin.slots) {
    if (threadIdx.x < 64) {
      shard_sum27_wave(sums_in, fin_tot);
      IcpPose p = *fin.pose_in;
      icp_solve_step(fin_tot, p);
      if (threadIdx.x == 0) {
        fin_pose = p;
        if (blockIdx.x == 0) {
          for (int k = 0; k < 27; ++k) st_out->sums[k] = fin_tot[k];
          if (p.lost) {
            st_out->lost = 1;
            st_out->need_reset = 1;
          } else {
            for (int i = 0; i < 9; ++i) st_out->R[i] = p.R[i];
            for (int i = 0; i < 3; ++i) st_out->t[i] = p.t[i];
          }
          st_out->n_iter = p.n_iter;
        }
        if (early.slots && blockIdx.x == gridDim.x - 1) {
          const unsigned n = *early.seq;
          TrackState* dst = early.slots + early.slot_fifo[n % HSK_RING_FIFO];
          const bool use_new = !p.lost;
          for (int i = 0; i < 9; ++i) dst->R[i] = use_new ? p.R[i] : st->R[i];
          for (int i = 0; i < 3; ++i) dst->t[i] = use_new ? p.t[i] : st->t[i];
          for (int i = 0; i < 9; ++i) dst->Rp[i] = st->Rp[i];
          for (int i = 0; i < 3; ++i) dst->tp[i] = st->tp[i];
          dst->lost = p.lost ? 1 : st->lost;
          dst->frame = st->frame;
          dst->n_iter = p.n_iter;
          dst->need_reset = p.lost ? 1 : st->need_reset;
          for (int k = 0; k < 27; ++k) dst->sums[k] = fin_tot[k];
          __threadfence_system();
          __hip_atomic_store(&dst->pose_mark, (n + 1u) | 0x80000000u, __ATOMIC_RELEASE, __HIP_MEMORY_SCOPE_SYSTEM);
        }
      }
    }
    __syncthreads();
    if (early.slots && blockIdx.x == gridDim.x - 1) return;
  }
  __shared__ int4 wv_sh[4];
  const int ncol = vp.X / 4;
  const int gxn = (vp.X + 63) / 64, gyn = (vp.Y + 15) / 16;
  const bool fp_block = (int)blockIdx.x < gxn * gyn;
  const int fby = (int)blockIdx.x / gxn, fbx = (int)blockIdx.x - fby * gxn;
  const int y = fby * 16 + (int)((threadIdx.x & 63) >> 2), lc = fbx * 16 + (int)(threadIdx.x >> 6) * 4 + (int)(threadIdx.x & 3);
  const bool col_ok = fp_block && y < vp.Y && lc < ncol;
  const int x0 = lc * 4;
  int zl = 0x7fffffff, zh = -0x7fffffff;
  if (col_ok) {
    const bool own = fin.slots != nullptr && !fin_pose.lost;
    const float* __restrict__ Rm = own ? fin_pose.R : st->R;
    const float* __restrict__ tm = own ? fin_pose.t : st->t;
    const float tx = tm[0], ty = tm[1], tz = tm[2];
    const float i00 = Rm[0], i01 = Rm[3], i02 = Rm[6];
    const float i10 = Rm[1], i11 = Rm[4], i12 = Rm[7];
    const float i20 = Rm[2], i21 = Rm[5], i22 = Rm[8];
    const float gy = ((float)y + 0.5f) * vp.cell[1] - ty;
    float glo = 1e30f, ghi = -1e30f;
#pragma unroll
    for (int j = 0; j < 4; ++j) {
      const float gx = ((float)(x0 + j) + 0.5f) * vp.cell[0] - tx;
      const float ax = i00 * gx + i01 * gy, ay = i10 * gx + i11 * gy, az = i20 * gx + i21 * gy;
      float lo = -1e30f, hi = 1e30f;
      clip_interval(az, i22, lo, hi);
      const float ul = 1.5f + in.cx, uh = ((float)W + 0.5f) - in.cx;
      const float vl = 1.5f + in.cy, vh = ((float)H + 0.5f) - in.cy;
      clip_interval(ax * in.fx + ul * az, i02 * in.fx + ul * i22, lo, hi);
      clip_interval(uh * az - ax * in.fx, uh * i22 - i02 * in.fx, lo, hi);
      clip_interval(ay * in.fy + vl * az, i12 * in.fy + vl * i22, lo, hi);
      clip_interval(vh * az - ay * in.fy, vh * i22 - i12 * in.fy, lo, hi);
      if (lo <= hi) {
        glo = fminf(glo, lo);
        ghi = fmaxf(ghi, hi);
      }
    }
    if (glo <= ghi) {
      const float inv_cz = __builtin_amdgcn_rcpf(vp.cell[2]);
      const float fl = (glo + tz) * inv_cz - 2.5f, fh = (ghi + tz) * inv_cz + 1.5f;
      const int a = fl < -1e9f ? -1000000000 : (fl > 1e9f ? 1000000000 : (int)floorf(fl));
      const int b = fh < -1e9f ? -1000000000 : (fh > 1e9f ? 1000000000 : (int)ceilf(fh));
      zl = a - vp.zs0;
      zh = b - vp.zs0;
    }
    zint[(size_t)y * ncol + lc] = make_int2(zl, zh);
  }
  if (fp_block) {
    int lo = zl, hi = zh;
    int lo_all = col_ok ? zl : -0x7fffffff, hi_all = col_ok ? zh : 0x7fffffff;
#pragma unroll
    for (int o = 32; o > 0; o >>= 1) {
      lo = min(lo, __shfl_xor(lo, o, 64));
      hi = max(hi, __shfl_xor(hi, o, 64));
      lo_all = max(lo_all, __shfl_xor(lo_all, o, 64));
      hi_all = min(hi_all, __shfl_xor(hi_all, o, 64));
    }
    if ((threadIdx.x & 63) == 0) {
      ((int4*)(wgz + (((size_t)gxn * gyn + 1) & ~(size_t)1)))[(size_t)blockIdx.x * 4 + (threadIdx.x >> 6)] = make_int4(lo, hi, lo_all, hi_all);
      wv_sh[threadIdx.x >> 6] = make_int4(lo, hi, lo_all, hi_all);
    }
    __syncthreads();
    if (ca.cflag != nullptr) {
      const bool own = fin.slots != nullptr && !fin_pose.lost;
      const bool lost = fin.slots != nullptr ? fin_pose.lost != 0 : st->lost != 0;
      const float* __restrict__ Rm = own ? fin_pose.R : st->R;
      const float* __restrict__ tm = own ? fin_pose.t : st->t;
      const int zchunks = (vp.nzs + ca.zchunk - 1) / ca.zchunk;
      const int tw16 = tw;
      for (int item = threadIdx.x; item < 4 * zchunks; item += blockDim.x) {
        const int w = item & 3, zc = item >> 2;
        const int4 r = wv_sh[w];
        const int zbeg = zc * ca.zchunk, zend = min(zbeg + ca.zchunk, vp.nzs);
        const size_t ci = (((size_t)zc * gyn + fby) * gxn + fbx) * 4 + w;
        const unsigned c_now = ca.cs != nullptr ? (unsigned)ca.cs[ci] : 0u;
        unsigned verdict = HSK_CF_MIXED;
        if ((zbeg > r.y) | (zend - 1 < r.x)) {
          verdict = HSK_CF_SKIP;
        } else {
          const int xa = fbx * 64 + w * 16, ya = fby * 16;
          const int xb = min(xa + 15, vp.X - 1), yb = min(ya + 15, vp.Y - 1);
          const bool full = (xa + 15 < vp.X) & (ya + 15 < vp.Y) & (zbeg + vp.zchunk <= vp.nzs) & (ca.zchunk == vp.zchunk);
          const float g0[3] = {((float)xa + 0.5f) * vp.cell[0] - tm[0], ((float)ya + 0.5f) * vp.cell[1] - tm[1],
                               ((float)(vp.zs0 + zbeg) + 0.5f) * vp.cell[2] - tm[2]};
          const float g1[3] = {((float)xb + 0.5f) * vp.cell[0] - tm[0], ((float)yb + 0.5f) * vp.cell[1] - tm[1],
                               ((float)(vp.zs0 + zend - 1) + 0.5f) * vp.cell[2] - tm[2]};
          float umin = 1e30f, umax = -1e30f, vmin = 1e30f, vmax = -1e30f, zmn = 1e30f;
#pragma unroll
          for (int c = 0; c < 8; ++c) {
            const float gx = (c & 1) ? g1[0] : g0[0], gy = (c & 2) ? g1[1] : g0[1], gz = (c & 4) ? g1[2] : g0[2];
            const float cxm = (Rm[0] * gx + Rm[3] * gy) + Rm[6] * gz, cym = (Rm[1] * gx + Rm[4] * gy) + Rm[7] * gz;
            const float czm = (Rm[2] * gx + Rm[5] * gy) + Rm[8] * gz;
            const float rq = __builtin_amdgcn_rcpf(czm);
            const float uq = (cxm * in.fx) * rq + in.cx, vq = (cym * in.fy) * rq + in.cy;
            zmn = fminf(zmn, czm);
            umin = fminf(umin, uq);
            umax = fmaxf(umax, uq);
            vmin = fminf(vmin, vq);
            vmax = fmaxf(vmax, vq);
          }
          if (zmn > 0.05f) {
            umin -= 1.0f; vmin -= 1.0f; umax += 1.0f; vmax += 1.0f;
            float d_hi2 = 0.0f, d_lo2 = 0.0f;
#pragma unroll
            for (int a = 0; a < 3; ++a) {
              const float p0 = g0[a] * g0[a], p1 = g1[a] * g1[a];
              d_hi2 += fmaxf(p0, p1);
              d_lo2 += (g0[a] <= 0.0f && g1[a] >= 0.0f) ? 0.0f : fminf(p0, p1);
            }
            const float d_hi = __builtin_amdgcn_sqrtf(d_hi2), d_lo = __builtin_amdgcn_sqrtf(d_lo2);
            const bool in_img = (umin >= 0.0f) & (vmin >= 0.0f) & (umax <= (float)(W - 1)) & (vmax <= (float)(H - 1));
            const bool off_img = (umax < 0.0f) | (vmax < 0.0f) | (umin > (float)(W - 1)) | (vmin > (float)(H - 1));
            if (off_img) {
              verdict = HSK_CF_SKIP;
            } else {
              const int tu0 = (int)fminf(fmaxf(umin, 0.0f), (float)(W - 1)) >> 4, tu1 = (int)fminf(fmaxf(umax, 0.0f), (float)(W - 1)) >> 4;
              const int tv0 = (int)fminf(fmaxf(vmin, 0.0f), (float)(H - 1)) >> 4, tv1 = (int)fminf(fmaxf(vmax, 0.0f), (float)(H - 1)) >> 4;
              const int nx = tu1 - tu0 + 1, ny = tv1 - tv0 + 1;
              if ((nx <= (2 << (HSK_SPARSE_LEVELS - 1))) & (ny <= (2 << (HSK_SPARSE_LEVELS - 1)))) {
                const int kx = min(31 - __clz(nx), HSK_SPARSE_LEVELS - 1), ky = min(31 - __clz(ny), HSK_SPARSE_LEVELS - 1);
                const float2* __restrict__ lv = ca.sparse + (size_t)(ky * HSK_SPARSE_LEVELS + kx) * tw16 * th;
                const int ub = tu1 - (1 << kx) + 1, vb = tv1 - (1 << ky) + 1;
                const float2 q00 = lv[tv0 * tw16 + tu0], q01 = lv[tv0 * tw16 + ub], q10 = lv[vb * tw16 + tu0], q11 = lv[vb * tw16 + ub];
                const float Dx = fmaxf(fmaxf(q00.x, q01.x), fmaxf(q10.x, q11.x)), Dn = fminf(fminf(q00.y, q01.y), fminf(q10.y, q11.y));
                const bool dead = d_lo * 0.99999f - Dx > ca.cull_thr;
                const bool in_all = (r.z <= zbeg) & (r.w >= zend - 1);
                const bool fre = full & in_img & in_all & (d_hi * 1.00001f + ca.free_thr <= Dn);
                verdict = dead ? HSK_CF_SKIP : (fre ? HSK_CF_FREE : HSK_CF_MIXED);
              }
            }
          }
        }
        if (verdict == HSK_CF_FREE && ca.cs != nullptr && !lost) {
          const unsigned c = c_now;
          if (c >= 1u && c < 255u) {
            ca.cs[ci] = (unsigned char)(c + 1u);
            ca.cs[ca.dirty_off + ci] = 1;
            verdict = HSK_CF_SKIP;
          }
        }
        ca.cflag[ci] = (unsigned char)verdict;
      }
    }
  }
}

struct ColumnTerms {
  float axfc, ayfc, azc, pnc;
};
struct IntegrateConst {
  float hw, hh;
  float rk4, zmin4, cull_thr4, free_thr4;
  float cull_thr2, free_thr2;
};
static IntegrateConst integrate_const(const VolParams& vp, int W, int H, const Intr& in) {
  IntegrateConst k;
  const float cellm = fmaxf(vp.cell[0], fmaxf(vp.cell[1], vp.cell[2]));
  const float rk = 1.06f * 2.75f * cellm * fmaxf(in.fx, in.fy);
  k.hw = 0.5f * (float)(W - 1);
  k.hh = 0.5f * (float)(H - 1);
  k.rk4 = rk * 1.47f;
  k.zmin4 = fmaxf(fmaxf(0.1f, 40.0f * cellm), k.rk4 / ((float)HSK_TILE - 2.5f));
  k.cull_thr4 = vp.tau * 1.001f + 1e-4f + 2.3f * cellm;
  k.free_thr4 = vp.tau * 1.0002f + 1e-4f + 2.3f * cellm;
  k.cull_thr2 = vp.tau * 1.001f + 1e-4f;
  k.free_thr2 = vp.tau * 1.0002f + 1e-4f;
  return k;
}

static __device__ __forceinline__ void mark_brick_negative(unsigned* __restrict__ flags, const VolParams& vp, int x, int y, int zz) {
  const int bs = vp.bshift, bxn = vp.X >> bs, byn = vp.Y >> bs;
  const int bx = x >> bs, by = y >> bs, bz = zz >> bs;
  const int bit = (bz * byn + by) * bxn + bx;
  if ((flags[bit >> 5] >> (bit & 31)) & 1u) return;
  __hip_atomic_fetch_or(&flags[bit >> 5], 1u << (bit & 31), __ATOMIC_RELAXED, __HIP_MEMORY_SCOPE_AGENT);
  if (hsk_super_ok(vp)) {
    const int sb = ((bz >> HSK_SUPER_SHIFT) * hsk_super_dim(vp.Y, bs) + (by >> HSK_SUPER_SHIFT)) * hsk_super_dim(vp.X, bs) + (bx >> HSK_SUPER_SHIFT);
    __hip_atomic_fetch_or(&flags[hsk_flag_words(vp) + (sb >> 5)], 1u << (sb & 31), __ATOMIC_RELAXED, __HIP_MEMORY_SCOPE_AGENT);
  }
}

#define HSK_SUM_RAGGED 130u
#define HSK_SUM_MAX 255u
#define HSK_LIGHT_PEND 15u
static __host__ __device__ __forceinline__ size_t hsk_chunk_count(const VolParams& vp) {
  return (size_t)((vp.nzs + vp.zchunk - 1) / vp.zchunk) * ((vp.Y + 15) / 16) * ((vp.X + 63) / 64) * 4;
}
static __host__ __device__ __forceinline__ size_t hsk_lane_sum_bytes(const VolParams& vp) {
  return hsk_chunk_count(vp) * (size_t)(64 * (vp.zchunk >> 2));
}
static __host__ __device__ __forceinline__ size_t hsk_chunk_bytes_padded(const VolParams& vp) { return (hsk_chunk_count(vp) + 255) & ~(size_t)255; }
template <int NS>
static __host__ __device__ __forceinline__ size_t hsk_sum_index_ns(const VolParams& vp, int x0, int y, int zb) {
  static_assert(NS == 2 || NS == 4, "8 or 16 planes per chunk");
  const size_t tiles_x = (size_t)(vp.X + 63) / 64, tiles_y = (size_t)(vp.Y + 15) / 16;
  const size_t wg = ((size_t)(zb >> (NS == 4 ? 4 : 3)) * tiles_y + (size_t)(y >> 4)) * tiles_x + (size_t)(x0 >> 6);
  const size_t wave = (size_t)((x0 >> 4) & 3), lane = (size_t)(((y & 15) << 2) | ((x0 >> 2) & 3));
  return ((wg * 4 + wave) * 64 + lane) * (size_t)NS + (size_t)((zb >> 2) & (NS - 1));
}
static __host__ __device__ __forceinline__ size_t hsk_sum_index(const VolParams& vp, int x0, int y, int zb) {
  return vp.zchunk == 16 ? hsk_sum_index_ns<4>(vp, x0, y, zb) : hsk_sum_index_ns<2>(vp, x0, y, zb);
}
static __host__ __device__ __forceinline__ unsigned hsk_sum_push(unsigned s, unsigned k) {
  return s < HSK_SUM_RAGGED ? (s + k < (unsigned)HSK_MAX_WEIGHT + 1u ? s + k : (unsigned)HSK_MAX_WEIGHT + 1u) : s + k;
}
static __device__ __forceinline__ size_t hsk_bbase(const VolParams& vp, int x0, int y, int zb) {
  return ((((size_t)(zb >> 2) * vp.Y + (size_t)y) * (size_t)(vp.X >> 2)) + (size_t)(x0 >> 2)) << 2;
}
#define VIDX(zbv, u) (hsk_bbase(vp, x0, y, (zbv)) + (size_t)(u))
static __device__ __forceinline__ unsigned hsk_uniform_code(unsigned word) {
  const unsigned w = word >> 16;
  if (word == 0u) return 1u;
  return ((word & 0xffffu) == (unsigned)HSK_DIVISOR && w >= 1u && w <= (unsigned)HSK_MAX_WEIGHT) ? w + 1u : 0u;
}
static __device__ __forceinline__ bool hsk_vector_is(const uint4& q, unsigned word) {
  return q.x == word && q.y == word && q.z == word && q.w == word;
}
static __device__ __forceinline__ unsigned hsk_sum_classify(const uint4 q[4]) {
  const unsigned word = q[0].x;
  if (hsk_vector_is(q[0], word) && hsk_vector_is(q[1], word) && hsk_vector_is(q[2], word) && hsk_vector_is(q[3], word))
    return hsk_uniform_code(word);
  unsigned a = 0xffffffffu, o = 0u, m = 0xffffffffu;
#pragma unroll
  for (int u = 0; u < 4; ++u) {
    a &= q[u].x & q[u].y & q[u].z & q[u].w;
    o |= q[u].x | q[u].y | q[u].z | q[u].w;
    m = min(m, min(min(q[u].x, q[u].y), min(q[u].z, q[u].w)));
  }
  return ((a & 0x7fffu) == 0x7fffu && (o & 0x8000u) == 0u && m >= 0x10000u && (o >> 16) <= (unsigned)HSK_MAX_WEIGHT) ? HSK_SUM_RAGGED : 0u;
}
static __device__ __forceinline__ void hsk_vector_add_weight(uint4& q, unsigned p) {
  const unsigned cap = ((unsigned)HSK_MAX_WEIGHT << 16) | (unsigned)HSK_DIVISOR, inc = p << 16;
  q.x = min(q.x + inc, cap);
  q.y = min(q.y + inc, cap);
  q.z = min(q.z + inc, cap);
  q.w = min(q.w + inc, cap);
}

static __device__ __forceinline__ bool update_vector_free4(uint4& q) {
  const unsigned cap = ((unsigned)HSK_MAX_WEIGHT << 16) | (unsigned)HSK_DIVISOR;
  const unsigned w4[4] = {q.x, q.y, q.z, q.w};
  unsigned nw[4];
  bool gen[4], gen_any = false;
#pragma unroll
  for (int j = 0; j < 4; ++j) {
    const bool unseen = (w4[j] >> 16) == 0u;
    const bool simple = unseen || (w4[j] & 0xffffu) == (unsigned)HSK_DIVISOR;
    nw[j] = unseen ? (0x10000u | (unsigned)HSK_DIVISOR) : min(w4[j] + 0x10000u, cap);
    gen[j] = !simple;
    gen_any = gen_any || gen[j];
  }
  if (__ballot(gen_any) != 0ull) {
#pragma unroll
    for (int j = 0; j < 4; ++j) {
      const int tp = (int)(short)(w4[j] & 0xffffu);
      const unsigned wp = w4[j] >> 16;
      const float Wp = (float)wp;
      const float Fn = hsk_div_small_exact(hsk_tsdf_unpack(tp) * Wp + 1.0f, Wp + 1.0f);
      int fixed = (int)(Fn * 32767.0f);
      fixed = min(max(fixed, -HSK_DIVISOR), HSK_DIVISOR);
      const unsigned wg = ((unsigned)fixed & 0xffffu) | (min(wp + 1u, (unsigned)HSK_MAX_WEIGHT) << 16);
      nw[j] = gen[j] ? wg : nw[j];
    }
  }
  q = make_uint4(nw[0], nw[1], nw[2], nw[3]);
  return nw[0] != w4[0] || nw[1] != w4[1] || nw[2] != w4[2] || nw[3] != w4[3];
}

struct DetailPose {
  float tx, ty, tz;
  float i00, i01, i02, i10, i11, i12, i20, i21, i22;
};
static __device__ __forceinline__ DetailPose detail_pose(const TrackState* __restrict__ st) {
  DetailPose p;
  p.tx = st->t[0]; p.ty = st->t[1]; p.tz = st->t[2];
  p.i00 = st->R[0]; p.i01 = st->R[3]; p.i02 = st->R[6];
  p.i10 = st->R[1]; p.i11 = st->R[4]; p.i12 = st->R[7];
  p.i20 = st->R[2]; p.i21 = st->R[5]; p.i22 = st->R[8];
  return p;
}

#ifdef HSK_PA_TIMING
#define HSK_PA_SLOTS 65536u
__device__ unsigned long long g_pa_times[HSK_PA_SLOTS * 8];
extern "C" int hsk_debug_pa_times(unsigned long long* out, int n) {
  return (int)hipMemcpyFromSymbol(out, HIP_SYMBOL(g_pa_times), (size_t)n * 8);
}
extern "C" int hsk_debug_pa_clear() {
  static unsigned long long zeros[HSK_PA_SLOTS * 8];
  return (int)hipMemcpyToSymbol(HIP_SYMBOL(g_pa_times), zeros, sizeof(zeros));
}
#define PA_STAMP(k) do { if (!COUNT_ONLY && lane == 0 && pa_slot < HSK_PA_SLOTS) g_pa_times[pa_slot * 8 + (k)] = __builtin_amdgcn_s_memrealtime(); } while (0)
#else
#define PA_STAMP(k) do { } while (0)
// ... 486 lines not shown
    float pn[4];
#pragma unroll
    for (int j = 0; j < 4; ++j) {
      const float gx = ((float)(x0 + j) + 0.5f) * vp.cell[0] - P.tx;
      const float axj = P.i00 * gx + P.i01 * gy, ayj = P.i10 * gx + P.i11 * gy, azj = P.i20 * gx + P.i21 * gy;
      pn[j] = gx * gx + gy * gy;
      const float camz = azj + bz;
      const float inv_z = hsk_rcp_exact(camz);
      const float fu = ((axj + bx) * in.fx) * inv_z + in.cx;
      const float fv = ((ayj + by) * in.fy) * inv_z + in.cy;
      const int uu = (int)rintf(fu), vv = (int)rintf(fv);
      const bool ok = LIGHT ? true : (inr && camz >= 1.17549435e-38f && (unsigned)uu < (unsigned)W && (unsigned)vv < (unsigned)H);
      pix[j] = ok ? min(max(vv * W + uu, 0), last) : -1;
    }
    float D[4];
#pragma unroll
    for (int j = 0; j < 4; ++j) D[j] = scaled[max(pix[j], 0)];
#pragma unroll
    for (int j = 0; j < 4; ++j) {
      const float Ds = pix[j] >= 0 ? D[j] : 0.0f;
      if (LIGHT) {
        D[j] = (inr && Ds != 0.0f) ? 1.0f : -4.0f;
      } else {
        const float sdf = Ds - hsk_sqrt_exact(gz2 + pn[j]);
        const float f = sdf * vp.tau_inv;
        D[j] = (Ds != 0.0f && sdf >= -vp.tau) ? (f < 1.0f ? f : 1.0f) : -4.0f;
      }
    }
    if (COUNT_ONLY) {
#pragma unroll
      for (int j = 0; j < 4; ++j) cnt += D[j] > -2.0f ? 1u : 0u;
      return;
    }
    uint4 q1 = q;
    if (LIGHT && code != 0u) hsk_vector_add_weight(q1, code);
    const unsigned w4[4] = {q1.x, q1.y, q1.z, q1.w};
    unsigned nw[4];
    bool gen[4], gen_any = false;
#pragma unroll
    for (int j = 0; j < 4; ++j) {
      const bool upd = D[j] > -2.0f;
      const bool unseen = (w4[j] >> 16) == 0u;
      const bool simple = D[j] == 1.0f && (unseen || (w4[j] & 0xffffu) == (unsigned)HSK_DIVISOR);
      const unsigned ws = unseen ? (0x10000u | (unsigned)HSK_DIVISOR) : min(w4[j] + 0x10000u, cap);
      nw[j] = (upd && simple) ? ws : w4[j];
      gen[j] = upd && !simple;
      gen_any = gen_any || gen[j];
    }
    bool neg = false;
    if (__ballot(gen_any) != 0ull) {
#pragma unroll
      for (int j = 0; j < 4; ++j) {
        const int tp = (int)(short)(w4[j] & 0xffffu);
        const unsigned wp = w4[j] >> 16;
        const float Wp = (float)wp;
        const float Fn = hsk_div_small_exact(hsk_tsdf_unpack(tp) * Wp + D[j], Wp + 1.0f);
        int fixed = (int)(Fn * 32767.0f);
        fixed = min(max(fixed, -HSK_DIVISOR), HSK_DIVISOR);
        const unsigned wg = ((unsigned)fixed & 0xffffu) | (min(wp + 1u, (unsigned)HSK_MAX_WEIGHT) << 16);
        nw[j] = gen[j] ? wg : nw[j];
        neg = neg || (gen[j] && fixed < 0);
      }
    }
    if (inr && (nw[0] != q.x || nw[1] != q.y || nw[2] != q.z || nw[3] != q.w)) vol[VIDX(zb, u)] = make_uint4(nw[0], nw[1], nw[2], nw[3]);
    if (!LIGHT) {
      const unsigned negq = quad_or(neg ? 1u : 0u), fw = quad_or(flag_word);
      if (negq != 0u && u == 0 && ((fw >> (fbit & 31)) & 1u) == 0u) mark_brick_negative(flags, vp, x0, y, zb);
    } else if (uni != nullptr) {
      const unsigned word = nw[0];
      const unsigned same = (nw[1] == word && nw[2] == word && nw[3] == word) ? 1u : 0u;
      const unsigned w_first = (unsigned)__shfl((int)word, lane & ~3, 64);
      const unsigned all_same = quad_and((same != 0u && word == w_first) ? 1u : 0u);
      const unsigned a = quad_and(nw[0] & nw[1] & nw[2] & nw[3]), o = quad_or(nw[0] | nw[1] | nw[2] | nw[3]);
      const unsigned m = quad_min(min(min(nw[0], nw[1]), min(nw[2], nw[3])));
      const unsigned ragged = ((a & 0x7fffu) == 0x7fffu && (o & 0x8000u) == 0u && m >= 0x10000u && (o >> 16) <= (unsigned)HSK_MAX_WEIGHT) ? HSK_SUM_RAGGED : 0u;
      const unsigned state = all_same != 0u ? hsk_uniform_code(w_first) : ragged;
      if (have && u == 0 && state != 0u) uni[hsk_sum_index(vp, x0, y, zb)] = (unsigned char)state;
    }
  };
  {
    unsigned e0 = wave * 16u;
    unsigned id_next = entry_at(pre, n, false, e0 + (unsigned)(lane >> 2));
    for (; e0 < n; e0 += stride) {
      const unsigned id = id_next;
      id_next = entry_at(pre, n, false, e0 + stride + (unsigned)(lane >> 2));
      work(e0 + (unsigned)(lane >> 2) < n, id, false);
    }
  }
  if (n2 != 0u) {
    unsigned g0 = (nwaves - 1u - wave) * 16u;
    unsigned id_next = entry_at(pre2, n2, true, g0 + (unsigned)(lane >> 2));
    for (; g0 < n2; g0 += stride) {
      const unsigned id = id_next;
      id_next = entry_at(pre2, n2, true, g0 + stride + (unsigned)(lane >> 2));
      work(g0 + (unsigned)(lane >> 2) < n2, id, true);
    }
  }
  if (COUNT_ONLY) {
#pragma unroll
    for (int o = 32; o > 0; o >>= 1) cnt += __shfl_down(cnt, o, 64);
    if (lane == 0 && cnt) atomicAdd(counter, cnt);
  }
}

void launch_tile_tables(hipStream_t s, int W, int H, float* tiles) {
  const int tw = (W + HSK_TILE - 1) / HSK_TILE, th = (H + HSK_TILE - 1) / HSK_TILE;
  const int fw = (W + HSK_FTILE - 1) / HSK_FTILE, fh = (H + HSK_FTILE - 1) / HSK_FTILE;
  float2* ftab = (float2*)(tiles + 4 * tw * th);
  float2* qtab = ftab + (size_t)fw * fh;
  float2* fwin = qtab + (size_t)4 * fw * fh;
  float2* sparse = fwin + (size_t)45 * fw * fh;
  hipLaunchKernelGGL(k_tile_tables, dim3((4 * fw * fh + 255) / 256, 18 + HSK_SPARSE_LEVELS * HSK_SPARSE_LEVELS), dim3(256), 0, s, tiles, tiles + tw * th, tw,
                     th, (const float2*)ftab, (const float2*)qtab, fw, fh, fwin, sparse);
}
void launch_tile_fine(hipStream_t s, const float* scaled, int W, int H, float* tiles) {
  const int tw = (W + HSK_TILE - 1) / HSK_TILE, th = (H + HSK_TILE - 1) / HSK_TILE;
  const int fw = (W + HSK_FTILE - 1) / HSK_FTILE, fh = (H + HSK_FTILE - 1) / HSK_FTILE;
  float2* ftab = (float2*)(tiles + 4 * tw * th);
  float2* qtab = ftab + (size_t)fw * fh;
  hipLaunchKernelGGL(k_tile_fine, dim3((fw * fh + 255) / 256), dim3(256), 0, s, scaled, W, H, ftab, fw, fh, qtab);
  launch_tile_tables(s, W, H, tiles);
}
size_t tile_table_bytes(int W, int H) { return hsk_tiles_floats(W, H) * sizeof(float); }

size_t integrate_zint_entries(const VolParams& vp) {
  const size_t fp = (size_t)((vp.X + 63) / 64) * ((vp.Y + 15) / 16);
  return (size_t)(vp.X / 4) * vp.Y + ((fp + 1) & ~(size_t)1) + 8 * fp + (hsk_chunk_count(vp) + 7) / 8;
}
size_t integrate_cflag_offset_bytes(const VolParams& vp) {
  const size_t fp = (size_t)((vp.X + 63) / 64) * ((vp.Y + 15) / 16);
  return ((size_t)(vp.X / 4) * vp.Y + ((fp + 1) & ~(size_t)1) + 8 * fp) * sizeof(int2);
}
size_t integrate_chunk_count(const VolParams& vp) { return hsk_chunk_count(vp); }
size_t integrate_queue_counter_words() { return (size_t)HSK_NQUEUES * HSK_QCOUNT_STRIDE; }
unsigned long long integrate_queue_entries(const unsigned* counter_words) {
  unsigned long long n = 0;
  for (size_t q = 0; q < HSK_NQUEUES; ++q) n += counter_words[q * HSK_QCOUNT_STRIDE];
  return n;
}
unsigned long long integrate_queue_light_entries(const unsigned* counter_words) {
  unsigned long long n = 0;
  for (size_t q = 0; q < HSK_NQUEUES; ++q) n += counter_words[q * HSK_QCOUNT_STRIDE + 1];
  return n;
}
size_t integrate_queue_words(const VolParams& vp) {
  const int zchunk = vp.nzs >= vp.zchunk ? vp.zchunk : vp.nzs;
  const size_t nblk = (size_t)((vp.X + 63) / 64) * ((vp.Y + 15) / 16) * ((vp.nzs + zchunk - 1) / zchunk);
  const size_t qcap = ((nblk + HSK_NQUEUES - 1) / HSK_NQUEUES) * 256u * (size_t)((zchunk + 3) / 4);
  return (size_t)HSK_NQUEUES * HSK_QCOUNT_STRIDE + (size_t)HSK_NQUEUES * qcap;
}

void launch_integrate(hipStream_t s, void* vol, const float* scaled, const TrackState* st, const VolParams& vp, int W,
                      int H, Intr in, bool count_only, unsigned long long* counter, unsigned* flags,
                      const float* tmax, int2* zint, unsigned* queue, const IcpFinal* icp_final, unsigned char* uni, const RingOut* early) {
  const int zchunk = vp.nzs >= vp.zchunk ? vp.zchunk : vp.nzs;
  const int zchunks = (vp.nzs + zchunk - 1) / zchunk;
  const int tw = (W + HSK_TILE - 1) / HSK_TILE, th = (H + HSK_TILE - 1) / HSK_TILE;
  const int ncols = (vp.X / 4) * vp.Y;
  const int fw = (W + HSK_FTILE - 1) / HSK_FTILE, fh = (H + HSK_FTILE - 1) / HSK_FTILE;
  const float2* ftab = (const float2*)(tmax + 4 * tw * th) + (size_t)5 * fw * fh;
  const float2* qtab = ftab + (size_t)9 * fw * fh;
  const int col_blocks = ((vp.X + 63) / 64) * ((vp.Y + 15) / 16), dil_blocks = (tw * th + 255) / 256;
  unsigned* qcount = queue;
  const IcpFinal none = {nullptr, nullptr, 0};
  const IcpFinal fin = (icp_final && !count_only) ? *icp_final : none;
  int2* wgz = zint + ncols;
  const int4* wvz = (const int4*)(wgz + (((size_t)col_blocks + 1) & ~(size_t)1));
  unsigned char* cflag = (unsigned char*)(wvz + (size_t)col_blocks * 4);
  const IntegrateConst kc = integrate_const(vp, W, H, in);
  const float2* sparse = (const float2*)(tmax + 4 * tw * th) + (size_t)50 * fw * fh;
  const unsigned* vmask = (const unsigned*)(tmax + hsk_tiles_mask_offset(W, H));
  const CoarseArgs ca = {cflag, (count_only || uni == nullptr) ? nullptr : uni + hsk_lane_sum_bytes(vp), sparse, (unsigned)hsk_chunk_bytes_padded(vp), zchunk, kc.free_thr2, kc.cull_thr2};
  const RingOut quiet_ring = {nullptr, nullptr, nullptr};
  const RingOut early_ring = (early && fin.slots && !count_only) ? *early : quiet_ring;
  hipLaunchKernelGGL(k_column_zrange, dim3((col_blocks > dil_blocks ? col_blocks : dil_blocks) + (early_ring.slots ? 1 : 0)), dim3(256), 0, s, fin, tmax,
                     tmax + tw * th, (float2*)(tmax + 2 * tw * th), tw, th, dil_blocks, qcount, st, vp, W, H, in, zint,
                     const_cast<TrackState*>(st), wgz, early_ring, ca);
  dim3 block(64, 4, 1);
  const dim3 grid((vp.X + 63) / 64, (vp.Y + 15) / 16, zchunks);
  const float2* dil = (const float2*)(tmax + 2 * tw * th);
  unsigned* qdata = queue + HSK_NQUEUES * HSK_QCOUNT_STRIDE;
  const unsigned nblk = grid.x * grid.y * (unsigned)zchunks;
  const unsigned qcap = ((nblk + HSK_NQUEUES - 1) / HSK_NQUEUES) * 256u * (unsigned)((zchunk + 3) / 4);
  const unsigned gmagic = grid.x > 1u ? (unsigned)(0x100000000ull / grid.x) + 1u : 0u;
  const unsigned long long qmag_x = (1ull << 40) / (unsigned long long)(vp.X / 4) + 1ull, qmag_y = (1ull << 40) / (unsigned long long)vp.Y + 1ull;
  const dim3 detail_grid(DETAIL3_GX * HSK_NQUEUES);
  if (count_only) {
    if (vp.zchunk == 16)
      hipLaunchKernelGGL((k_integrate<true, 4>), grid, block, 0, s, st, (const unsigned*)cflag, wvz, zchunk, grid.x, gmagic, (double*)nullptr, (unsigned char*)nullptr, dil,
                         W, H, tw, th, grid.y, (uint4*)vol, scaled, vp, in, counter, flags, qdata, qcount, qcap, ftab, fw, fh, qtab, kc, (const int2*)zint, vmask, hsk_mask_pitch32(W));
    else
      hipLaunchKernelGGL((k_integrate<true, 2>), grid, block, 0, s, st, (const unsigned*)cflag, wvz, zchunk, grid.x, gmagic, (double*)nullptr, (unsigned char*)nullptr, dil,
                         W, H, tw, th, grid.y, (uint4*)vol, scaled, vp, in, counter, flags, qdata, qcount, qcap, ftab, fw, fh, qtab, kc, (const int2*)zint, vmask, hsk_mask_pitch32(W));
    hipLaunchKernelGGL(k_integrate_detail3<true>, detail_grid, dim3(256), 0, s, st, qcount, qdata, qcap, W, H, (uint4*)vol, scaled, in, vp,
                       counter, flags, qmag_x, qmag_y, (unsigned char*)nullptr);
  } else {
    if (vp.zchunk == 16)
      hipLaunchKernelGGL((k_integrate<false, 4>), grid, block, 0, s, st, (const unsigned*)cflag, wvz, zchunk, grid.x, gmagic, fin.slots, uni, dil, W, H, tw, th, grid.y,
                         (uint4*)vol, scaled, vp, in, counter, flags, qdata, qcount, qcap, ftab, fw, fh, qtab, kc, (const int2*)zint, vmask, hsk_mask_pitch32(W));
    else
      hipLaunchKernelGGL((k_integrate<false, 2>), grid, block, 0, s, st, (const unsigned*)cflag, wvz, zchunk, grid.x, gmagic, fin.slots, uni, dil, W, H, tw, th, grid.y,
                         (uint4*)vol, scaled, vp, in, counter, flags, qdata, qcount, qcap, ftab, fw, fh, qtab, kc, (const int2*)zint, vmask, hsk_mask_pitch32(W));
    hipLaunchKernelGGL(k_integrate_detail3<false>, detail_grid, dim3(256), 0, s, st, qcount, qdata, qcap, W, H, (uint4*)vol, scaled, in, vp,
                       counter, flags, qmag_x, qmag_y, uni);
  }
}

__global__ void k_rebuild_flags(const short2* __restrict__ vol, VolParams vp, unsigned* __restrict__ flags) {
  const size_t n = (size_t)vp.X * vp.Y * vp.nzs;
  const size_t i = (size_t)blockIdx.x * blockDim.x + threadIdx.x;
  if (i >= n) return;
  const int x = (int)(i % vp.X), y = (int)((i / vp.X) % vp.Y), zz = (int)(i / ((size_t)vp.X * vp.Y));
  if (vol[hsk_vox_index(vp, x, y, zz)].x < 0) mark_brick_negative(flags, vp, x, y, zz);
}
template <bool TO_LINEAR>
__global__ void k_vol_convert(uint4* __restrict__ vol, VolParams vp, int zz0, int nz, uint4* __restrict__ lin) {
  const int qx = vp.X >> 2;
  const size_t n = (size_t)qx * vp.Y * nz;
  const size_t i = (size_t)blockIdx.x * blockDim.x + threadIdx.x;
  if (i >= n) return;
  const int xl = (int)(i % qx), y = (int)((i / qx) % vp.Y), zr = (int)(i / ((size_t)qx * vp.Y));
  const size_t at = hsk_vox_index(vp, xl * 4, y, zz0 + zr) >> 2;
  if (TO_LINEAR)
    lin[i] = vol[at];
  else
    vol[at] = lin[i];
}
void launch_vol_to_linear(hipStream_t s, const void* vol, const VolParams& vp, int zz0, int nz, void* lin) {
  const size_t n = (size_t)(vp.X >> 2) * vp.Y * nz;
  hipLaunchKernelGGL(k_vol_convert<true>, dim3((unsigned)((n + 255) / 256)), dim3(256), 0, s, (uint4*)const_cast<void*>(vol), vp, zz0, nz, (uint4*)lin);
}
void launch_vol_from_linear(hipStream_t s, void* vol, const VolParams& vp, int zz0, int nz, const void* lin) {
  const size_t n = (size_t)(vp.X >> 2) * vp.Y * nz;
  hipLaunchKernelGGL(k_vol_convert<false>, dim3((unsigned)((n + 255) / 256)), dim3(256), 0, s, (uint4*)vol, vp, zz0, nz, (uint4*)const_cast<void*>(lin));
}
void launch_rebuild_flags(hipStream_t s, const void* vol, const VolParams& vp, unsigned* flags) {
  const size_t n = (size_t)vp.X * vp.Y * vp.nzs;
  hipLaunchKernelGGL(k_rebuild_flags, dim3((unsigned)((n + 255) / 256)), dim3(256), 0, s, (const short2*)vol, vp, flags);
}

size_t uniform_bytes(const VolParams& vp) { return hsk_lane_sum_bytes(vp) + 2 * hsk_chunk_bytes_padded(vp); }
size_t uniform_lane_bytes(const VolParams& vp) { return hsk_lane_sum_bytes(vp); }
template <bool MATERIALIZE, int NS>
__global__ __launch_bounds__(256) void k_summaries(uint4* __restrict__ vol, VolParams vp, unsigned char* __restrict__ uni) {
  const size_t cw = (size_t)blockIdx.x * 4 + (threadIdx.x >> 6);
  if (cw >= hsk_chunk_count(vp)) return;
  const int lane = threadIdx.x & 63, w = (int)(cw & 3);
  const int tiles_x = (vp.X + 63) / 64, tiles_y = (vp.Y + 15) / 16;
  const size_t wg = cw >> 2;
  const int fbx = (int)(wg % tiles_x), fby = (int)((wg / tiles_x) % tiles_y), zc = (int)(wg / ((size_t)tiles_x * tiles_y));
  const int x0 = (fbx * 16 + w * 4 + (lane & 3)) * 4, y = fby * 16 + (lane >> 2);
  const bool active = x0 < vp.X && y < vp.Y;
  unsigned char* const cs = uni + hsk_lane_sum_bytes(vp);
  unsigned char* const dirty = cs + hsk_chunk_bytes_padded(vp);
  unsigned char* const sum_at = uni + (cw * 64 + (size_t)lane) * NS;
  if (MATERIALIZE && dirty[cw] == 0) return;
  if (!MATERIALIZE) {
    bool quiet = active;
#pragma unroll
    for (int g = 0; g < NS; ++g) {
      const int zb = zc * vp.zchunk + 4 * g;
      unsigned code = 0u;
      if (active && zb + 3 < vp.nzs) {
        uint4 q[4];
        for (int u = 0; u < 4; ++u) q[u] = vol[VIDX(zb, u)];
        code = hsk_sum_classify(q);
      }
      sum_at[g] = (unsigned char)code;
      quiet = quiet && code >= 2u;
    }
    const bool all_quiet = __ballot(quiet) == ~0ull;
    if (lane == 0) {
      cs[cw] = (zc * vp.zchunk + vp.zchunk <= vp.nzs && all_quiet) ? 1 : 0;
      dirty[cw] = 0;
    }
    return;
  }
  const unsigned c = cs[cw];
  const unsigned kpend = c >= 2u ? c - 1u : 0u;
#pragma unroll
  for (int g = 0; g < NS; ++g) {
    const int zb = zc * vp.zchunk + 4 * g;
    if (!active || zb >= vp.nzs) continue;
    const unsigned s0 = sum_at[g], sm = hsk_sum_push(s0, kpend);
    if (sm >= 2u && sm < HSK_SUM_RAGGED) {
      const unsigned word = ((sm - 1u) << 16) | (unsigned)HSK_DIVISOR;
      for (int u = 0; u < 4; ++u) vol[VIDX(zb, u)] = make_uint4(word, word, word, word);
      if (sm != s0) sum_at[g] = (unsigned char)sm;
    } else if (sm > HSK_SUM_RAGGED) {
      uint4 q[4];
      for (int u = 0; u < 4; ++u) q[u] = vol[VIDX(zb, u)];
      for (int u = 0; u < 4; ++u) {
        hsk_vector_add_weight(q[u], sm - HSK_SUM_RAGGED);
        vol[VIDX(zb, u)] = q[u];
      }
      sum_at[g] = (unsigned char)hsk_sum_classify(q);
    }
  }
  if (lane == 0) {
    if (kpend != 0u) cs[cw] = 1;
    dirty[cw] = 0;
  }
}
void launch_rebuild_uniform(hipStream_t s, const void* vol, const VolParams& vp, unsigned char* uni) {
  const unsigned nb = (unsigned)((hsk_chunk_count(vp) + 3) / 4);
  if (vp.zchunk == 16)
    hipLaunchKernelGGL((k_summaries<false, 4>), dim3(nb), dim3(256), 0, s, (uint4*)const_cast<void*>(vol), vp, uni);
  else
    hipLaunchKernelGGL((k_summaries<false, 2>), dim3(nb), dim3(256), 0, s, (uint4*)const_cast<void*>(vol), vp, uni);
}
void launch_materialize(hipStream_t s, void* vol, const VolParams& vp, unsigned char* uni) {
  const unsigned nb = (unsigned)((hsk_chunk_count(vp) + 3) / 4);
  if (vp.zchunk == 16)
    hipLaunchKernelGGL((k_summaries<true, 4>), dim3(nb), dim3(256), 0, s, (uint4*)vol, vp, uni);
  else
    hipLaunchKernelGGL((k_summaries<true, 2>), dim3(nb), dim3(256), 0, s, (uint4*)vol, vp, uni);
}
```

### housescan_amd/kinfu.py

```python
import ctypes as C

import numpy as np

from . import _lib


class KinfuError(RuntimeError):
    pass


def default_config(n=512, **over):
    lib = _lib.load()
    cfg = _lib.HskConfig()
    lib.hsk_default_config(C.byref(cfg), int(n))
    for k, v in over.items():
        if k in ("vol_size_m", "icp_iters", "init_pose"):
            arr = getattr(cfg, k)
            for i, x in enumerate(np.asarray(v).reshape(-1)):
                arr[i] = x
        else:
            setattr(cfg, k, v)
    return cfg


def _fp(a):
    return a.ctypes.data_as(C.POINTER(C.c_float))


def _apply_view_fields(v, width, height, fx, fy, cx, cy, pose, mode, light, light_in_camera, background):
    for name, val in (("width", width), ("height", height), ("fx", fx), ("fy", fy), ("cx", cx), ("cy", cy), ("mode", mode),
                      ("light_in_camera", light_in_camera)):
        if val is not None:
            setattr(v, name, val)
    if pose is not None:
        v.pose[:] = [float(x) for x in np.asarray(pose, np.float32).reshape(16)]
        v.follow = 0
    if light is not None:
        v.light[:] = [float(x) for x in light]
    if background is not None:
        v.background[:] = [int(x) for x in background]


def _image_arrays(w, h, rgb, depth, vmap, nmap):
    shapes = (("rgb", rgb, (h, w, 3), np.uint8), ("depth", depth, (h, w), np.uint16), ("vmap", vmap, (3, h, w), np.float32),
              ("nmap", nmap, (3, h, w), np.float32))
    ok = 1 <= w <= 4096 and 1 <= h <= 4096
    out = {key: np.empty(shape, dt) for key, want, shape, dt in shapes if want and ok}
    return out, lambda k: out[k].ctypes.data if k in out else None


class KinfuTracker:

    def __init__(self, cfg=None, **over):
        self.lib = _lib.load()
        self.cfg = cfg if cfg is not None else default_config(**over)
        h = C.c_void_p()
        rc = self.lib.hsk_create(C.byref(self.cfg), C.byref(h))
        if rc != 0:
            raise KinfuError(f"hsk_create failed ({rc}): {self.lib.hsk_last_error(None).decode()}")
        self.h = h
        self.w, self.hgt = self.cfg.width, self.cfg.height
        z0, nz = C.c_int(), C.c_int()
        self.lib.hsk_stored_planes(self.h, C.byref(z0), C.byref(nz))
        self.stored_z0, self.stored_nz = z0.value, nz.value

    def close(self):
        if getattr(self, "h", None):
            self.lib.hsk_destroy(self.h)
            self.h = None

    def __del__(self):
        try:
            self.close()
        except Exception:
            pass

    def _ck(self, rc):
        if rc != 0:
            raise KinfuError(f"hskinfu error {rc}: {self.lib.hsk_last_error(self.h).decode()}")

    @staticmethod
    def _depth(depth):
        d = np.ascontiguousarray(depth, dtype=np.uint16)
        if d.ndim != 2:
            raise KinfuError("depth must be a (h, w) uint16 array")
        return d

    def process_frame(self, depth):
        d = self._depth(depth)
        pose = np.empty(16, np.float32)
        tracked = C.c_int()
        self._ck(self.lib.hsk_process_frame(self.h, d.ctypes.data, d.shape[1], d.shape[0], _fp(pose), C.byref(tracked)))
        return pose.reshape(4, 4), bool(tracked.value)

    def process_frame_dev(self, depth_dev_ptr):
        pose = np.empty(16, np.float32)
        tracked = C.c_int()
        self._ck(self.lib.hsk_process_frame_dev(self.h, C.c_void_p(depth_dev_ptr), self.w, self.hgt, _fp(pose),
                                                C.byref(tracked)))
        return pose.reshape(4, 4), bool(tracked.value)

    def submit_frame_dev(self, depth_dev_ptr):
        self._ck(self.lib.hsk_submit_frame_dev(self.h, C.c_void_p(depth_dev_ptr), self.w, self.hgt))

    def submit_frame(self, depth):
        d = self._depth(depth)
        self._ck(self.lib.hsk_submit_frame(self.h, d.ctypes.data, d.shape[1], d.shape[0]))

    def wait_frame(self):
        pose = np.empty(16, np.float32)
        tracked = C.c_int()
        self._ck(self.lib.hsk_wait_frame(self.h, _fp(pose), C.byref(tracked)))
        return pose.reshape(4, 4), bool(tracked.value)

    def track_stream(self, reader, first=0, count=None):
        if count is None:
            count = len(reader) - first
        poses = np.empty((count, 16), np.float32)
        tracked = np.zeros(count, np.int32)
        self._ck(self.lib.hsk_track_stream(self.h, reader.h, int(first), int(count), _fp(poses), tracked.ctypes.data_as(C.POINTER(C.c_int))))
        return poses.reshape(count, 4, 4), tracked.astype(bool)

    def flush_weights(self):
        self._ck(self.lib.hsk_flush_weights(self.h))

    def prepare_readout(self, product_bytes=0):
        self._ck(self.lib.hsk_prepare_readout(self.h, int(product_bytes)))

    def reset(self):
        self._ck(self.lib.hsk_reset(self.h))

    def integrate(self, depth, pose):
        d = self._depth(depth)
        p = np.ascontiguousarray(pose, np.float32).reshape(16)
        self._ck(self.lib.hsk_integrate(self.h, d.ctypes.data, d.shape[1], d.shape[0], _fp(p)))

    def count_updates(self, depth, pose):
        d = self._depth(depth)
        p = np.ascontiguousarray(pose, np.float32).reshape(16)
        n = C.c_uint64()
        self._ck(self.lib.hsk_count_updates(self.h, d.ctypes.data, d.shape[1], d.shape[0], _fp(p), C.byref(n)))
        return n.value

    def integrate_coarse_counts(self):
        c = (C.c_uint64 * 4)()
        self._ck(self.lib.hsk_integrate_coarse_counts(self.h, c))
        return tuple(int(x) for x in c)

    def integrate_queue_entries(self):
        n = C.c_uint64()
        self._ck(self.lib.hsk_integrate_queue_entries(self.h, C.byref(n)))
        return n.value

    def submit_host_us(self, reset=False):
        us = (C.c_double * 4)()
        n = C.c_uint64()
        self._ck(self.lib.hsk_submit_host_us(self.h, us, C.byref(n), int(reset)))
        return list(us), n.value

    def integrate_light_entries(self):
        n = C.c_uint64()
        self._ck(self.lib.hsk_integrate_light_entries(self.h, C.byref(n)))
        return n.value

    def raycast(self, pose, want_keys=False):
        p = np.ascontiguousarray(pose, np.float32).reshape(16)
        v = np.empty((3, self.hgt, self.w), np.float32)
        n = np.empty((3, self.hgt, self.w), np.float32)
        keys = np.empty((self.hgt, self.w), np.int32) if want_keys else None
        self._ck(self.lib.hsk_raycast(self.h, _fp(p), v.ctypes.data, n.ctypes.data, keys.ctypes.data if want_keys else None))
        return (v, n, keys) if want_keys else (v, n)

    def preprocess(self, depth):
        d = self._depth(depth)
        self._ck(self.lib.hsk_preprocess(self.h, d.ctypes.data, d.shape[1], d.shape[0]))

    def icp_accumulate(self, level, pose_est, row0=0, row1=None):
        p = np.ascontiguousarray(pose_est, np.float32).reshape(16)
        if row1 is None:
            row1 = self.hgt >> level
        out = np.empty(27, np.float64)
        self._ck(self.lib.hsk_icp_accumulate(self.h, level, _fp(p), row0, row1, out.ctypes.data_as(C.POINTER(C.c_double))))
        return out

    def icp_solve(self, sums27):
        s = np.ascontiguousarray(sums27, np.float64)
        x = np.empty(6, np.float32)
        ok = C.c_int()
        self._ck(self.lib.hsk_icp_solve(s.ctypes.data_as(C.POINTER(C.c_double)), _fp(x), C.byref(ok)))
        return x, bool(ok.value)

    def download_tsdf(self, out=None):
        if out is None:
            out = np.empty((self.stored_nz, self.cfg.vol_y, self.cfg.vol_x, 2), np.int16)
        want = self.stored_nz * self.cfg.vol_y * self.cfg.vol_x * 2
        if not (isinstance(out, np.ndarray) and out.dtype == np.int16 and out.flags.c_contiguous and out.flags.writeable and out.size == want):
            raise ValueError(f"download_tsdf(out=...): a writeable C-contiguous int16 array of {want} elements is needed (the C side takes a bare pointer)")
        self._ck(self.lib.hsk_download_tsdf(self.h, out.ctypes.data))
        return out

    def upload_tsdf(self, vol):
        v = np.ascontiguousarray(vol, np.int16)
        if v.size != self.stored_nz * self.cfg.vol_y * self.cfg.vol_x * 2:
            raise ValueError(f"upload_tsdf: {self.stored_nz * self.cfg.vol_y * self.cfg.vol_x * 2} int16 elements are needed, got {v.size}")
        self._ck(self.lib.hsk_upload_tsdf(self.h, v.ctypes.data))

    def get_pose(self):
        p = np.empty(16, np.float32)
        self._ck(self.lib.hsk_get_pose(self.h, _fp(p)))
        return p.reshape(4, 4)

    def set_pose(self, pose):
        p = np.ascontiguousarray(pose, np.float32).reshape(16)
        self._ck(self.lib.hsk_set_pose(self.h, _fp(p)))

    def download_map(self, kind, level):
        out = np.empty((3, self.hgt >> level, self.w >> level), np.float32)
        self._ck(self.lib.hsk_download_map(self.h, kind, level, out.ctypes.data))
        return out

    def upload_map(self, kind, level, arr):
        a = np.ascontiguousarray(arr, np.float32)
        self._ck(self.lib.hsk_upload_map(self.h, kind, level, a.ctypes.data))

    def download_depth_level(self, level):
        out = np.empty((self.hgt >> level, self.w >> level), np.uint16)
        self._ck(self.lib.hsk_download_depth_level(self.h, level, out.ctypes.data))
        return out

    def download_scaled_depth(self):
        out = np.empty((self.hgt, self.w), np.float32)
        self._ck(self.lib.hsk_download_scaled_depth(self.h, out.ctypes.data))
        return out

    def extract_cloud(self, cap=None):
        n = C.c_size_t()
        self._ck(self.lib.hsk_extract_cloud(self.h, None, 0, C.byref(n)))
        total = n.value
        m = total if cap is None else min(cap, total)
        out = np.empty((m, 3), np.float32)
        if m:
            self._ck(self.lib.hsk_extract_cloud(self.h, out.ctypes.data, m, C.byref(n)))
        return out, total

    def extract_mesh(self, cap=None, cubes=False):
        fn = self.lib.hsk_extract_mesh_cubes if cubes else self.lib.hsk_extract_mesh
        n = C.c_size_t()
        self._ck(fn(self.h, None, 0, C.byref(n)))
        total = n.value
        m = total if cap is None else min(cap, total)
        out = np.empty((m, 3, 3), np.float32)
        if m:
            self._ck(fn(self.h, out.ctypes.data, m, C.byref(n)))
        return out, total

    def _rgb(self, rgb):
        c = np.ascontiguousarray(rgb, dtype=np.uint8)
        if c.shape != (self.hgt, self.w, 3):
            raise KinfuError(f"rgb must be a ({self.hgt}, {self.w}, 3) uint8 array registered to the depth grid")
        return c

    def enable_color(self, max_weight=0, band_m=0.0):
        self._ck(self.lib.hsk_enable_color(self.h, int(max_weight), C.c_float(band_m)))

    def process_frame_rgbd(self, depth, rgb):
        d, c = self._depth(depth), self._rgb(rgb)
        pose = np.empty(16, np.float32)
        tracked = C.c_int()
        self._ck(self.lib.hsk_process_frame_rgbd(self.h, d.ctypes.data, c.ctypes.data, d.shape[1], d.shape[0], _fp(pose), C.byref(tracked)))
        return pose.reshape(4, 4), bool(tracked.value)

    def submit_frame_rgbd(self, depth, rgb):
        d, c = self._depth(depth), self._rgb(rgb)
        self._ck(self.lib.hsk_submit_frame_rgbd(self.h, d.ctypes.data, c.ctypes.data, d.shape[1], d.shape[0]))

    def integrate_color(self, depth, rgb, pose):
        d, c = self._depth(depth), self._rgb(rgb)
        p = np.ascontiguousarray(pose, np.float32).reshape(16)
        self._ck(self.lib.hsk_integrate_color(self.h, d.ctypes.data, c.ctypes.data, d.shape[1], d.shape[0], _fp(p)))

    def download_color(self):
        out = np.empty((self.stored_nz, self.cfg.vol_y, self.cfg.vol_x, 4), np.uint8)
        self._ck(self.lib.hsk_download_color(self.h, out.ctypes.data))
        return out

    def upload_color(self, rgbw):
        a = np.ascontiguousarray(rgbw, np.uint8)
        if a.size != self.stored_nz * self.cfg.vol_y * self.cfg.vol_x * 4:
            raise ValueError(f"upload_color: {self.stored_nz * self.cfg.vol_y * self.cfg.vol_x * 4} uint8 elements are needed, got {a.size}")
        self._ck(self.lib.hsk_upload_color(self.h, a.ctypes.data))

    def extract_cloud_attrs(self, cap=None, normals=True, rgb=True):
        n, nu = C.c_size_t(), C.c_size_t()
        self._ck(self.lib.hsk_extract_cloud_attrs(self.h, None, None, None, 0, C.byref(n), None))
        total = n.value
        m = total if cap is None else min(cap, total)
        xyz = np.empty((m, 3), np.float32)
        nrm = np.empty((m, 3), np.float32) if normals else None
        col = np.empty((m, 3), np.uint8) if rgb else None
        if m:
            self._ck(self.lib.hsk_extract_cloud_attrs(self.h, xyz.ctypes.data, None if nrm is None else nrm.ctypes.data,
                                                      None if col is None else col.ctypes.data, m, C.byref(n), C.byref(nu)))
        return xyz, nrm, col, total, nu.value

    def extract_mesh_indexed(self, normals=True, rgb=True):
        nv, nf, nu = C.c_size_t(), C.c_size_t(), C.c_size_t()
        self._ck(self.lib.hsk_extract_mesh_indexed(self.h, None, None, None, 0, C.byref(nv), None, 0, C.byref(nf), None))
        verts = np.empty((nv.value, 3), np.float32)
        faces = np.empty((nf.value, 3), np.int32)
        nrm = np.empty((nv.value, 3), np.float32) if normals else None
        col = np.empty((nv.value, 3), np.uint8) if rgb else None
# ... 415 lines not shown
```

### include/hskinfu.h

```cpp
#ifndef HSKINFU_H
#define HSKINFU_H
#include <stddef.h>
#include <stdint.h>

#ifdef __cplusplus
extern "C" {
#endif

#define HSK_OK 0
#define HSK_ERR_ARG (-1)
#define HSK_ERR_HIP (-2)
#define HSK_ERR_STATE (-3)
#define HSK_ERR_NOGPU (-4)
#define HSK_ERR_TIMEOUT (-5)

#define HSK_LEVELS 3
#define HSK_KEY_NONE 0x7fffffff

typedef struct hsk_ctx hsk_ctx;

typedef struct {
  int vol_x, vol_y, vol_z;
  float vol_size_m[3];
  float trunc_dist_m;
// ... 78 lines not shown
void hsk_default_view(const hsk_ctx* k, hsk_view* v);
int hsk_render_view(hsk_ctx* k, const hsk_view* v, uint8_t* rgb , uint16_t* depth_mm , float* vmap ,
                    float* nmap , size_t* n_hit, size_t* n_uncolored);
int hsk_write_ppm(const char* path, const uint8_t* rgb, int w, int h);
int hsk_write_pgm16(const char* path, const uint16_t* depth_mm, int w, int h);

#define HSK_PROJ_PINHOLE 0
#define HSK_PROJ_ORTHO   1
#define HSK_MAX_CLIP     4
typedef struct {
  hsk_view view;
  int projection;
  int light_directional;
  int n_clip;
  float clip[HSK_MAX_CLIP][4];
  uint8_t cut_rgb[3];
} hsk_section;
void hsk_default_section(const hsk_ctx* k, hsk_section* s);
int hsk_render_section(hsk_ctx* k, const hsk_section* s, uint8_t* rgb , uint16_t* depth_mm ,
                       float* vmap , float* nmap , size_t* n_hit, size_t* n_cut, size_t* n_uncolored);
int hsk_section_in_room(const hsk_section* house, const float room_xf[16], hsk_section* room);
int hsk_composite_views(int n, const uint8_t* const* rgb, const uint16_t* const* depth_mm, int w, int h,
                        const uint8_t background[3], uint8_t* out_rgb, uint16_t* out_depth_mm, int32_t* out_index);

typedef struct {
  uint64_t n_fused;
  uint64_t n_colored;
  uint64_t chunks_total;
  uint64_t chunks_swept;
  int32_t  box[6];
} hsk_fuse_stats;

int hsk_fuse_volume(hsk_ctx* dst, hsk_ctx* src, const float src_to_dst[16], hsk_fuse_stats* stats);

int hsk_invert_rigid(const float m[16], float inv[16]);

int hsk_fuse_footprint(const int src_dims[3], const float src_size_m[3], const int dst_dims[3], const float dst_size_m[3],
                       const float src_to_dst[16], int32_t box[6]);

typedef struct {
  uint32_t version, header_bytes;
  uint32_t flags;
  int32_t dims[3];
  int32_t z0, nz;
  float size_m[3];
  float trunc_dist_m;
  float trunc_eff_m;
  int32_t width, height;
  float fx, fy, cx, cy;
  float pose[16];
  int32_t frame;
  int32_t color_max_weight;
  float color_band_m;
  uint64_t n_bricks;
  uint64_t tsdf_bricks[4];
  uint64_t color_bricks[2];
  uint64_t tsdf_table_bytes, tsdf_payload_bytes, color_table_bytes, color_payload_bytes;
  uint64_t total_bytes;
  int32_t pass_reused;
} hsk_volume_info;

int hsk_pack_volume(hsk_ctx* k, void* buf, size_t cap_bytes, size_t* n_bytes, hsk_volume_info* info);
int hsk_unpack_volume(hsk_ctx* k, const void* buf, size_t n_bytes);
int hsk_save_volume(hsk_ctx* k, const char* path, hsk_volume_info* info );
int hsk_load_volume(hsk_ctx* k, const char* path);
int hsk_volume_image_info(const void* buf, size_t n_bytes, hsk_volume_info* info);
int hsk_volume_file_info(const char* path, hsk_volume_info* info);
int hsk_config_from_volume(const hsk_volume_info* info, hsk_config* c);
int hsk_resume_scan(hsk_ctx* k, const float pose[16]);

#define HSK_ALIGN_CONVERGED 0
#define HSK_ALIGN_MAX_ITERS 1
#define HSK_ALIGN_FEW 2
#define HSK_ALIGN_DEGENERATE 3
#define HSK_ALIGN_DIVERGED 4
#define HSK_ALIGN_MAX_ITERS_CAP 64
#define HSK_ALIGN_DIRECT (-1)
typedef struct {
  int max_iters;
  int probes;
  float cos_gate;
  uint32_t max_points;
  uint32_t min_points;
  float eps_rot;
  float eps_trans_m;
  float max_rot;
  float max_shift_m;
} hsk_align_params;
typedef struct {
  int status;
  int iterations;
  uint32_t n_points, stride;
  uint32_t n_used[HSK_ALIGN_MAX_ITERS_CAP];
  float rms_m[HSK_ALIGN_MAX_ITERS_CAP];
  float x_last[6];
  double sums_last[28];
} hsk_align_stats;

void hsk_default_align_params(const hsk_ctx* dst, hsk_align_params* p);
int hsk_align_cloud(hsk_ctx* dst, const float* xyz, const float* normals, size_t n, const float src_to_dst[16],
                    const hsk_align_params* params, float out[16], hsk_align_stats* stats);
int hsk_align_volume(hsk_ctx* dst, hsk_ctx* src, const float src_to_dst[16], const hsk_align_params* params, float out[16],
                     hsk_align_stats* stats);
int hsk_align_step(const double sums27[27], const float m[16], const float centre[3], float m_next[16], float x6[6], int* ok);

int hsk_mgpu_frame_begin(hsk_ctx* k, const void* depth_dev, int w, int h);
int hsk_mgpu_prefetch(hsk_ctx* k, const void* depth_dev, int w, int h);
int hsk_mgpu_frame_front(hsk_ctx* k, const void* depth_dev, int w, int h, void* keys_dev);
int hsk_mgpu_icp_accumulate(hsk_ctx* k, int level, int row0, int row1, void* sums27_dev );
int hsk_mgpu_icp_update(hsk_ctx* k, const void* sums27_dev);
int hsk_mgpu_icp_replicated(hsk_ctx* k);
int hsk_mgpu_integrate(hsk_ctx* k);
int hsk_mgpu_raycast_local(hsk_ctx* k, void* keys_dev );
int hsk_mgpu_raycast_resolve(hsk_ctx* k, const void* keys_min_dev, void* maps_bits_dev );
int hsk_mgpu_raycast_push(hsk_ctx* k, const void* keys_min_dev, void* const* dest_bits, int n_dest);
int hsk_mgpu_frame_end(hsk_ctx* k, const void* keys_min_dev, const void* maps_bits_dev, float pose_out[16], int* tracked);
int hsk_mgpu_frame_index(const hsk_ctx* k);
int hsk_mgpu_frame_end_async(hsk_ctx* k, const void* keys_min_dev, const void* maps_bits_dev);
int hsk_mgpu_restart_pending(const hsk_ctx* k);

typedef struct hsk_group hsk_group;
#define HSK_GROUP_FORCE_RCCL 1
#define HSK_GROUP_ICP_ALLREDUCE 2
#define HSK_GROUP_DIRECT 4
#define HSK_GROUP_PROFILE 8
int hsk_group_create(const hsk_config* c, int n_slabs, const int* device_ids, int flags, hsk_group** out);
int hsk_group_unique_id(void* id128);
int hsk_group_create_rank(const hsk_config* c, int rank, int world, const void* comm_id, int flags, hsk_group** out);
void hsk_group_destroy(hsk_group* g);
const char* hsk_group_last_error(const hsk_group* g);
int hsk_group_reset(hsk_group* g);
int hsk_group_process_frame(hsk_group* g, const uint16_t* depth, int w, int h, float pose_out[16], int* tracked);
int hsk_group_submit_frame(hsk_group* g, const uint16_t* depth, int w, int h);
int hsk_group_submit_frame_dev(hsk_group* g, const void* const* depth_dev, int w, int h);
int hsk_group_wait_frame(hsk_group* g, float pose_out[16], int* tracked);
int hsk_group_exchange_ms(hsk_group* g, double* sum_ms, double* front_sum_ms, unsigned long long* n_frames);
int hsk_group_n_slabs(const hsk_group* g);
int hsk_group_ranks_seen(hsk_group* g, int* n_ranks);
hsk_ctx* hsk_group_slab(hsk_group* g, int i);
int hsk_group_download_tsdf(hsk_group* g, int16_t* full_tsdf_weight_pairs);

void* hsk_stream(hsk_ctx* k);
int hsk_set_stream(hsk_ctx* k, void* stream);
int hsk_synchronize(hsk_ctx* k);
#define HSK_STAGE_PRE 0
#define HSK_STAGE_ICP 1
#define HSK_STAGE_INTEGRATE 2
#define HSK_STAGE_RAYCAST 3
#define HSK_NSTAGES 4
int hsk_set_profiling(hsk_ctx* k, int on);
int hsk_stage_ms(hsk_ctx* k, double sum_ms[HSK_NSTAGES], uint64_t* n_frames, int reset);
int hsk_icp_level_ms(hsk_ctx* k, double sum_ms[HSK_LEVELS]);
int hsk_submit_host_us(hsk_ctx* k, double sum_us[4], uint64_t* n_submissions, int reset);
int hsk_integrate_queue_entries(hsk_ctx* k, uint64_t* n_entries);
int hsk_integrate_light_entries(hsk_ctx* k, uint64_t* n_entries);
int hsk_integrate_coarse_counts(hsk_ctx* k, uint64_t counts[4]);
int hsk_bilateral_tables(float ws[169], float wc[512]);
int hsk_selftest_exact_ops(int device_id, uint64_t counts[8]);

int hsk_synth_pose(int frame, float pose[16]);
int hsk_synth_render(const float pose[16], int w, int h, float fx, float fy, float cx, float cy, uint16_t* depth);
int hsk_synth_room_extents(int variant, float extents[6] );
int hsk_synth_room_pose(int variant, int frame, int n_frames, float pose[16]);
int hsk_synth_room_render(int variant, const float pose[16], int w, int h, float fx, float fy, float cx, float cy, uint16_t* depth);
int hsk_synth_render_sensor(int scene, const float pose[16], int w, int h, float fx, float fy, float cx, float cy, uint64_t seed,
                            float sigma_mm, float range_cut_m, int absorbing, uint16_t* depth, double* hole_fraction);
int hsk_synth_color_at(int scene, const float p[3], uint8_t rgb[3]);
int hsk_synth_render_rgb(int scene, const float pose[16], int w, int h, float fx, float fy, float cx, float cy, uint8_t* rgb);

int hsk_write_pcd_xyz(const char* path, const float* xyz, size_t n_points);
int hsk_write_ply_mesh(const char* path, const float* tri_xyz, size_t n_triangles, size_t* n_vertices_out, size_t* n_faces_out);
int hsk_weld_triangles(const float* tri_xyz, size_t n_triangles, float* vertices, size_t cap_vertices, size_t* n_vertices, int32_t* indices);
int hsk_write_ply_indexed(const char* path, const float* vertices, const float* normals, const uint8_t* rgb, size_t n_vertices,
                          const int32_t* faces, size_t n_faces);
int hsk_voxel_downsample(const float* xyz, size_t n, float leaf_m, float* out, size_t cap, size_t* n_out);
int hsk_voxel_downsample_attrs(const float* xyz, const uint8_t* rgb, const float* normals, size_t n, float leaf_m, float* out_xyz,
                               uint8_t* out_rgb, float* out_normals, size_t cap, size_t* n_out);
int hsk_write_pcd_xyzrgbnormal(const char* path, const float* xyz, const uint8_t* rgb, const float* normals, size_t n);
int hsk_detect_planes(const float* xyz, size_t n, float dist_thresh_m, float min_fraction, int max_planes, int iterations,
                      float* planes_abcd , int* labels , int* n_planes);
int hsk_plane_hull(const float* xyz, size_t n, const int* labels, int plane, const float abcd[4], float* hull_xyz,
                   size_t cap, size_t* n_hull);
int hsk_write_planes_txt(const char* path, const float* planes_abcd, int n_planes);

int hsk_write_xf(const char* path, const float m[16]);
int hsk_read_xf(const char* path, float m[16]);
int hsk_transform_cloud(const float* xyz, size_t n, const float m[16], float* out );
int hsk_transform_normals(const float* n, size_t count, const float m[16], float* out );

typedef struct hsk_depth_stream hsk_depth_stream;
hsk_depth_stream* hsk_stream_create(const char* path, int w, int h, float fx, float fy, float cx, float cy);
hsk_depth_stream* hsk_stream_open(const char* path, int* w, int* h, int* n_frames, float intr[4]);
int hsk_stream_write(hsk_depth_stream* s, const uint16_t* depth);
int hsk_stream_read(hsk_depth_stream* s, int index, uint16_t* depth);
int hsk_stream_close(hsk_depth_stream* s);
int hsk_stream_info(const hsk_depth_stream* s, int* w, int* h, int* n_frames, float intr[4]);
int hsk_track_stream(hsk_ctx* k, hsk_depth_stream* s, int first, int count, float* poses_out, int* tracked_out);

#ifdef __cplusplus
}
#endif
#endif
```

Before: 4558.

## Speculatively compute integrate column tables from predicted pose while ICP solve finishes

```diff
diff --git a/housescan_amd/_lib.py b/housescan_amd/_lib.py
--- a/housescan_amd/_lib.py
+++ b/housescan_amd/_lib.py
@@ -211,6 +211,8 @@
     "hsk_stage_ms": (C.c_int, [_P, _D, C.POINTER(C.c_uint64), C.c_int]),
     "hsk_icp_level_ms": (C.c_int, [_P, _D]),
     "hsk_submit_host_us": (C.c_int, [_P, _D, C.POINTER(C.c_uint64), C.c_int]),
+    "hsk_debug_set_table_slack": (C.c_int, [_P, C.c_float]),
+    "hsk_debug_table_fallbacks": (C.c_int, [_P, C.POINTER(C.c_uint64)]),
     "hsk_integrate_queue_entries": (C.c_int, [_P, C.POINTER(C.c_uint64)]),
     "hsk_integrate_light_entries": (C.c_int, [_P, C.POINTER(C.c_uint64)]),
     "hsk_integrate_coarse_counts": (C.c_int, [_P, C.POINTER(C.c_uint64)]),
diff --git a/housescan_amd/csrc/hsk_ctx.h b/housescan_amd/csrc/hsk_ctx.h
--- a/housescan_amd/csrc/hsk_ctx.h
+++ b/housescan_amd/csrc/hsk_ctx.h
@@ -70,6 +70,7 @@
   TrackState* h_ring = nullptr;
   int* h_slot_fifo = nullptr;
   unsigned* d_ring_seq = nullptr;
+  TableSlack* d_slack = nullptr;
   unsigned ring_seq = 0;
   unsigned ring_expect[HSK_MAX_IN_FLIGHT + 1] = {};
   unsigned set_expect[2] = {0, 0};
diff --git a/housescan_amd/csrc/hsk_frame_tables.h b/housescan_amd/csrc/hsk_frame_tables.h
--- /dev/null
+++ b/housescan_amd/csrc/hsk_frame_tables.h
@@ -0,0 +1,188 @@
+#pragma once
+#include <math.h>
+#include <stddef.h>
+#ifndef HSK_HD
+#if defined(__HIPCC__)
+#define HSK_HD static __host__ __device__ __forceinline__
+#else
+#define HSK_HD static inline
+#endif
+#endif
+#if defined(__HIPCC__)
+#define HSK_FT_UNROLL _Pragma("unroll")
+#else
+#define HSK_FT_UNROLL
+#endif
+#if defined(__HIP_DEVICE_COMPILE__)
+#define HSK_FT_RCP(x) __builtin_amdgcn_rcpf(x)
+#define HSK_FT_SQRT(x) __builtin_amdgcn_sqrtf(x)
+#define HSK_FT_LOG2(n) (31 - __clz(n))
+#else
+#define HSK_FT_RCP(x) (1.0f / (x))
+#define HSK_FT_SQRT(x) sqrtf(x)
+#define HSK_FT_LOG2(n) (31 - __builtin_clz((unsigned)(n)))
+#endif
+
+#define HSK_FT_SPARSE_LEVELS 4
+#define HSK_FT_MIXED 0u
+#define HSK_FT_SKIP 1u
+#define HSK_FT_FREE 2u
+#define HSK_FT_EMPTY_LO 0x7fffffff
+
+HSK_HD int hsk_ft_min_i(int a, int b) { return a < b ? a : b; }
+HSK_HD int hsk_ft_max_i(int a, int b) { return a > b ? a : b; }
+
+HSK_HD float hsk_ft_margin(const float size[3], const float* tm, float eR, float eT) {
+  float g2 = 0.0f;
+  for (int a = 0; a < 3; ++a) {
+    const float lo = fabsf(tm[a]), hi = fabsf(size[a] - tm[a]);
+    const float m = fmaxf(lo, hi);
+    g2 += m * m;
+  }
+  const float G = HSK_FT_SQRT(g2) * 1.000001f;
+  return (1.7320509f * (eR * G + eT) + 3.0f * eR * eT) * 1.0625f + 6.103515625e-05f;
+}
+HSK_HD bool hsk_ft_pose_within(const float* Ra, const float* ta, const float* Rb, const float* tb, float eR, float eT) {
+  bool ok = true;
+  for (int i = 0; i < 9; ++i) ok = ok & (fabsf(Ra[i] - Rb[i]) <= eR);
+  for (int i = 0; i < 3; ++i) ok = ok & (fabsf(ta[i] - tb[i]) <= eT);
+  return ok;
+}
+
+HSK_HD void hsk_ft_clip(float c, float m, float& lo, float& hi) {
+  if (m > 0.0f) {
+    lo = fmaxf(lo, -c * HSK_FT_RCP(m));
+  } else if (m < 0.0f) {
+    hi = fminf(hi, -c * HSK_FT_RCP(m));
+  } else if (c < 0.0f) {
+    lo = 1e30f;
+    hi = -1e30f;
+  }
+}
+
+template <class Vol, class Cam>
+HSK_HD void hsk_ft_column_range(const Vol& vp, const Cam& in, int W, int H, const float* Rm, const float* tm, int x0, int y, float s,
+                                int& zl, int& zh) {
+  const float tx = tm[0], ty = tm[1], tz = tm[2];
+  const float i00 = Rm[0], i01 = Rm[3], i02 = Rm[6];
+  const float i10 = Rm[1], i11 = Rm[4], i12 = Rm[7];
+  const float i20 = Rm[2], i21 = Rm[5], i22 = Rm[8];
+  const float gy = ((float)y + 0.5f) * vp.cell[1] - ty;
+  const bool all = s < 0.0f;
+  float glo = all ? -1e30f : 1e30f, ghi = all ? 1e30f : -1e30f;
+  bool none = false;
+HSK_FT_UNROLL
+  for (int j = 0; j < 4; ++j) {
+    const float gx = ((float)(x0 + j) + 0.5f) * vp.cell[0] - tx;
+    const float ax = i00 * gx + i01 * gy, ay = i10 * gx + i11 * gy, az = i20 * gx + i21 * gy;
+    float lo = -1e30f, hi = 1e30f;
+    const float ul = 1.5f + in.cx, uh = ((float)W + 0.5f) - in.cx;
+    const float vl = 1.5f + in.cy, vh = ((float)H + 0.5f) - in.cy;
+    if (s == 0.0f) {
+      hsk_ft_clip(az, i22, lo, hi);
+      hsk_ft_clip(ax * in.fx + ul * az, i02 * in.fx + ul * i22, lo, hi);
+      hsk_ft_clip(uh * az - ax * in.fx, uh * i22 - i02 * in.fx, lo, hi);
+      hsk_ft_clip(ay * in.fy + vl * az, i12 * in.fy + vl * i22, lo, hi);
+      hsk_ft_clip(vh * az - ay * in.fy, vh * i22 - i12 * in.fy, lo, hi);
+    } else {
+      hsk_ft_clip(az + s, i22, lo, hi);
+      hsk_ft_clip((ax * in.fx + ul * az) + s * (in.fx + fabsf(ul)), i02 * in.fx + ul * i22, lo, hi);
+      hsk_ft_clip((uh * az - ax * in.fx) + s * (in.fx + fabsf(uh)), uh * i22 - i02 * in.fx, lo, hi);
+      hsk_ft_clip((ay * in.fy + vl * az) + s * (in.fy + fabsf(vl)), i12 * in.fy + vl * i22, lo, hi);
+      hsk_ft_clip((vh * az - ay * in.fy) + s * (in.fy + fabsf(vh)), vh * i22 - i12 * in.fy, lo, hi);
+    }
+    if (all) {
+      none = none | !(lo <= hi);
+      glo = fmaxf(glo, lo);
+      ghi = fminf(ghi, hi);
+    } else if (lo <= hi) {
+      glo = fminf(glo, lo);
+      ghi = fmaxf(ghi, hi);
+    }
+  }
+  zl = HSK_FT_EMPTY_LO;
+  zh = -HSK_FT_EMPTY_LO;
+  if ((glo <= ghi) & !none) {
+    const float inv_cz = HSK_FT_RCP(vp.cell[2]);
+    const float fl = (glo + tz) * inv_cz - 2.5f, fh = (ghi + tz) * inv_cz + 1.5f;
+    const int a = fl < -1e9f ? -1000000000 : (fl > 1e9f ? 1000000000 : (int)floorf(fl));
+    const int b = fh < -1e9f ? -1000000000 : (fh > 1e9f ? 1000000000 : (int)ceilf(fh));
+    zl = a - vp.zs0;
+    zh = b - vp.zs0;
+  }
+}
+
+struct HskFtRange {
+  int x, y, z, w;
+};
+template <class Vol, class Cam, class Tab>
+HSK_HD unsigned hsk_ft_chunk_verdict(const Vol& vp, const Cam& in, int W, int H, const float* Rm, const float* tm, int fbx, int fby, int w,
+                                     int zbeg, int zend, int zchunk, const HskFtRange& r, const Tab* sparse, int tw, int th, float free_thr,
+                                     float cull_thr, float D) {
+  unsigned verdict = HSK_FT_MIXED;
+  if ((zbeg > r.y) | (zend - 1 < r.x)) return HSK_FT_SKIP;
+  const int xa = fbx * 64 + w * 16, ya = fby * 16;
+  const int xb = hsk_ft_min_i(xa + 15, vp.X - 1), yb = hsk_ft_min_i(ya + 15, vp.Y - 1);
+  const bool full = (xa + 15 < vp.X) & (ya + 15 < vp.Y) & (zbeg + vp.zchunk <= vp.nzs) & (zchunk == vp.zchunk);
+  const float g0[3] = {((float)xa + 0.5f) * vp.cell[0] - tm[0], ((float)ya + 0.5f) * vp.cell[1] - tm[1],
+                       ((float)(vp.zs0 + zbeg) + 0.5f) * vp.cell[2] - tm[2]};
+  const float g1[3] = {((float)xb + 0.5f) * vp.cell[0] - tm[0], ((float)yb + 0.5f) * vp.cell[1] - tm[1],
+                       ((float)(vp.zs0 + zend - 1) + 0.5f) * vp.cell[2] - tm[2]};
+  float umin = 1e30f, umax = -1e30f, vmin = 1e30f, vmax = -1e30f, zmn = 1e30f;
+HSK_FT_UNROLL
+  for (int c = 0; c < 8; ++c) {
+    const float gx = (c & 1) ? g1[0] : g0[0], gy = (c & 2) ? g1[1] : g0[1], gz = (c & 4) ? g1[2] : g0[2];
+    const float cxm = (Rm[0] * gx + Rm[3] * gy) + Rm[6] * gz, cym = (Rm[1] * gx + Rm[4] * gy) + Rm[7] * gz;
+    const float czm = (Rm[2] * gx + Rm[5] * gy) + Rm[8] * gz;
+    const float rq = HSK_FT_RCP(czm);
+    const float uq = (cxm * in.fx) * rq + in.cx, vq = (cym * in.fy) * rq + in.cy;
+    zmn = fminf(zmn, czm);
+    umin = fminf(umin, uq);
+    umax = fmaxf(umax, uq);
+    vmin = fminf(vmin, vq);
+    vmax = fmaxf(vmax, vq);
+  }
+  if (D > 0.0f) zmn -= D;
+  if (zmn > 0.05f) {
+    umin -= 1.0f; vmin -= 1.0f; umax += 1.0f; vmax += 1.0f;
+    if (D > 0.0f) {
+      const float dz = D * HSK_FT_RCP(zmn);
+      const float wu = (in.fx + fmaxf(fabsf(umin - in.cx), fabsf(umax - in.cx))) * dz * 1.001f;
+      const float wv = (in.fy + fmaxf(fabsf(vmin - in.cy), fabsf(vmax - in.cy))) * dz * 1.001f;
+      umin -= wu; umax += wu; vmin -= wv; vmax += wv;
+    }
+    float d_hi2 = 0.0f, d_lo2 = 0.0f;
+HSK_FT_UNROLL
+    for (int a = 0; a < 3; ++a) {
+      const float p0 = g0[a] * g0[a], p1 = g1[a] * g1[a];
+      d_hi2 += fmaxf(p0, p1);
+      d_lo2 += (g0[a] <= 0.0f && g1[a] >= 0.0f) ? 0.0f : fminf(p0, p1);
+    }
+    float d_hi = HSK_FT_SQRT(d_hi2), d_lo = HSK_FT_SQRT(d_lo2);
+    if (D > 0.0f) {
+      d_hi += D;
+      d_lo -= D;
+    }
+    const bool in_img = (umin >= 0.0f) & (vmin >= 0.0f) & (umax <= (float)(W - 1)) & (vmax <= (float)(H - 1));
+    const bool off_img = (umax < 0.0f) | (vmax < 0.0f) | (umin > (float)(W - 1)) | (vmin > (float)(H - 1));
+    if (off_img) {
+      verdict = HSK_FT_SKIP;
+    } else {
+      const int tu0 = (int)fminf(fmaxf(umin, 0.0f), (float)(W - 1)) >> 4, tu1 = (int)fminf(fmaxf(umax, 0.0f), (float)(W - 1)) >> 4;
+      const int tv0 = (int)fminf(fmaxf(vmin, 0.0f), (float)(H - 1)) >> 4, tv1 = (int)fminf(fmaxf(vmax, 0.0f), (float)(H - 1)) >> 4;
+      const int nx = tu1 - tu0 + 1, ny = tv1 - tv0 + 1;
+      if ((nx <= (2 << (HSK_FT_SPARSE_LEVELS - 1))) & (ny <= (2 << (HSK_FT_SPARSE_LEVELS - 1)))) {
+        const int kx = hsk_ft_min_i(HSK_FT_LOG2(nx), HSK_FT_SPARSE_LEVELS - 1), ky = hsk_ft_min_i(HSK_FT_LOG2(ny), HSK_FT_SPARSE_LEVELS - 1);
+        const Tab* lv = sparse + (size_t)(ky * HSK_FT_SPARSE_LEVELS + kx) * tw * th;
+        const int ub = tu1 - (1 << kx) + 1, vb = tv1 - (1 << ky) + 1;
+        const Tab q00 = lv[tv0 * tw + tu0], q01 = lv[tv0 * tw + ub], q10 = lv[vb * tw + tu0], q11 = lv[vb * tw + ub];
+        const float Dx = fmaxf(fmaxf(q00.x, q01.x), fmaxf(q10.x, q11.x)), Dn = fminf(fminf(q00.y, q01.y), fminf(q10.y, q11.y));
+        const bool dead = d_lo * 0.99999f - Dx > cull_thr;
+        const bool in_all = (r.z <= zbeg) & (r.w >= zend - 1);
+        const bool fre = full & in_img & in_all & (d_hi * 1.00001f + free_thr <= Dn);
+        verdict = dead ? HSK_FT_SKIP : (fre ? HSK_FT_FREE : HSK_FT_MIXED);
+      }
+    }
+  }
+  return verdict;
+}
diff --git a/housescan_amd/csrc/hsk_launch.h b/housescan_amd/csrc/hsk_launch.h
--- a/housescan_amd/csrc/hsk_launch.h
+++ b/housescan_amd/csrc/hsk_launch.h
@@ -2,10 +2,16 @@
 #include "hsk_dev.h"
 #include "hsk_icp_dev.h"
 
+#define HSK_TABLE_EPS_R 0.0009765625f
+#define HSK_TABLE_EPS_T 0.0009765625f
+struct TableSlack {
+  float eps_r, eps_t;
+  unsigned fallbacks, pad;
+};
 void launch_integrate(hipStream_t s, void* vol, const float* scaled, const TrackState* st, const VolParams& vp, int W,
                       int H, Intr in, bool count_only, unsigned long long* counter, unsigned* flags,
                       const float* tmax, int2* zint, unsigned* queue, const IcpFinal* icp_final = nullptr,
-                      unsigned char* uni = nullptr, const RingOut* early = nullptr);
+                      unsigned char* uni = nullptr, const RingOut* early = nullptr, TableSlack* slack = nullptr);
 size_t uniform_bytes(const VolParams& vp);
 size_t uniform_lane_bytes(const VolParams& vp);
 void launch_rebuild_uniform(hipStream_t s, const void* vol, const VolParams& vp, unsigned char* uni);
diff --git a/housescan_amd/csrc/hskinfu_api.hip b/housescan_amd/csrc/hskinfu_api.hip
--- a/housescan_amd/csrc/hskinfu_api.hip
+++ b/housescan_amd/csrc/hskinfu_api.hip
@@ -162,6 +162,7 @@
   if (k->h_ring) (void)hipHostFree(k->h_ring);
   if (k->h_slot_fifo) (void)hipHostFree(k->h_slot_fifo);
   if (k->d_ring_seq) (void)hipFree(k->d_ring_seq);
+  if (k->d_slack) (void)hipFree(k->d_slack);
   for (auto& e : k->ring_ev)
     if (e) (void)hipEventDestroy(e);
   for (auto& e : k->ev)
@@ -320,6 +321,11 @@
   CK(hipHostGetDevicePointer((void**)&k->d_fifo_view, k->h_slot_fifo, 0));
   CK(hipMalloc((void**)&k->d_ring_seq, sizeof(unsigned)));
   CK(hipMemset(k->d_ring_seq, 0, sizeof(unsigned)));
+  {
+    const TableSlack slack = {HSK_TABLE_EPS_R, HSK_TABLE_EPS_T, 0u, 0u};
+    CK(hipMalloc((void**)&k->d_slack, sizeof(TableSlack)));
+    CK(hipMemcpy(k->d_slack, &slack, sizeof(TableSlack), hipMemcpyHostToDevice));
+  }
   for (auto& e : k->ring_ev) CK(hipEventCreateWithFlags(&e, hipEventDisableTiming));
   const int nb0 = icp_num_blocks(c->width, c->height);
   CK(hipMalloc((void**)&k->d_partials, (size_t)nb0 * 27 * sizeof(double)));
@@ -417,7 +423,7 @@
   const RingOut ring = {k->d_ring_view, k->d_fifo_view, k->d_ring_seq};
   launch_integrate(k->stream, k->d_vol, k->B().d_scaled, k->d_st, k->vp, k->lv[0].W, k->lv[0].H, k->lv[0].in, false,
                    k->d_counter, k->d_flags, k->B().d_tmax, k->d_zint, k->d_queue, (fin && fin->slots) ? fin : nullptr,
-                   k->d_uni, report_early ? &ring : nullptr);
+                   k->d_uni, report_early ? &ring : nullptr, k->d_slack);
 }
 
 static void enqueue_color(hsk_ctx* k) {
@@ -1144,6 +1150,23 @@
   }
   return HSK_OK;
 }
+extern "C" int hsk_debug_set_table_slack(hsk_ctx* k, float scale) {
+  if (!k || !(scale >= 0.0f)) return HSK_ERR_ARG;
+  (void)hipSetDevice(k->cfg.device_id);
+  const float sc = scale > 1.0f ? 1.0f : scale;
+  const float eps[2] = {HSK_TABLE_EPS_R * sc, HSK_TABLE_EPS_T * sc};
+  if (hipStreamSynchronize(k->stream) != hipSuccess) return HSK_ERR_HIP;
+  return hipMemcpy(k->d_slack, eps, sizeof(eps), hipMemcpyHostToDevice) == hipSuccess ? HSK_OK : HSK_ERR_HIP;
+}
+extern "C" int hsk_debug_table_fallbacks(hsk_ctx* k, uint64_t* n_fallbacks) {
+  if (!k || !n_fallbacks) return HSK_ERR_ARG;
+  (void)hipSetDevice(k->cfg.device_id);
+  unsigned n = 0;
+  if (hipStreamSynchronize(k->stream) != hipSuccess) return HSK_ERR_HIP;
+  if (hipMemcpy(&n, &k->d_slack->fallbacks, sizeof(n), hipMemcpyDeviceToHost) != hipSuccess) return HSK_ERR_HIP;
+  *n_fallbacks = n;
+  return HSK_OK;
+}
 extern "C" int hsk_icp_level_ms(hsk_ctx* k, double sum_ms[HSK_LEVELS]) {
   if (!k || !sum_ms) return HSK_ERR_ARG;
   for (int i = 0; i < HSK_NLEVELS; ++i) sum_ms[i] = k->icp_level_ms[i];
diff --git a/housescan_amd/csrc/integrate.hip b/housescan_amd/csrc/integrate.hip
--- a/housescan_amd/csrc/integrate.hip
+++ b/housescan_amd/csrc/integrate.hip
@@ -1,6 +1,7 @@
 #pragma clang fp contract(off)
 #include "hsk_dev.h"
 #include "hsk_launch.h"
+#include "hsk_frame_tables.h"
 
 #define HSK_TILE 16
 #define HSK_NQUEUES 256
@@ -126,17 +127,6 @@
   }
 }
 
-static __device__ __forceinline__ void clip_interval(float c, float m, float& lo, float& hi) {
-  if (m > 0.0f) {
-    lo = fmaxf(lo, -c * __builtin_amdgcn_rcpf(m));
-  } else if (m < 0.0f) {
-    hi = fminf(hi, -c * __builtin_amdgcn_rcpf(m));
-  } else if (c < 0.0f) {
-    lo = 1e30f;
-    hi = -1e30f;
-  }
-}
-
 struct CoarseArgs {
   unsigned char* cflag;
   unsigned char* cs;
@@ -145,19 +135,96 @@
   int zchunk;
   float free_thr, cull_thr;
 };
+static __device__ __forceinline__ void coarse_store(const CoarseArgs& ca, size_t ci, unsigned verdict, unsigned c_now, bool lost) {
+  if (verdict == HSK_CF_FREE && ca.cs != nullptr && !lost) {
+    const unsigned c = c_now;
+    if (c >= 1u && c < 255u) {
+      ca.cs[ci] = (unsigned char)(c + 1u);
+      ca.cs[ca.dirty_off + ci] = 1;
+      verdict = HSK_CF_SKIP;
+    }
+  }
+  ca.cflag[ci] = (unsigned char)verdict;
+}
 __global__ void k_column_zrange(IcpFinal fin, const float* __restrict__ tmax, const float* __restrict__ tmin,
                                 float2* __restrict__ dtab, int tw, int th, int dil_blocks, unsigned* __restrict__ qcount,
                                 const TrackState* __restrict__ st, VolParams vp, int W, int H, Intr in,
                                 int2* __restrict__ zint, TrackState* __restrict__ st_out, int2* __restrict__ wgz, RingOut early,
-                                CoarseArgs ca) {
+                                CoarseArgs ca, TableSlack* __restrict__ slack) {
   __shared__ double fin_tot[27];
   __shared__ IcpPose fin_pose;
+  __shared__ int4 wv_sh[4];
+  const bool solves = fin.slots != nullptr;
+  const int tid = (int)threadIdx.x;
+  const bool table_thread = tid < 256;
+  const bool reporter = early.slots != nullptr && blockIdx.x == gridDim.x - 1;
+  const int ncol = vp.X / 4;
+  const int gxn = (vp.X + 63) / 64, gyn = (vp.Y + 15) / 16;
+  const bool fp_block = (int)blockIdx.x < gxn * gyn;
+  const int fby = (int)blockIdx.x / gxn, fbx = (int)blockIdx.x - fby * gxn;
+  const int y = fby * 16 + ((tid & 63) >> 2), lc = fbx * 16 + (tid >> 6) * 4 + (tid & 3);
+  const bool col_ok = table_thread && fp_block && y < vp.Y && lc < ncol;
+  const int x0 = lc * 4;
+  const int zchunks = (vp.nzs + ca.zchunk - 1) / ca.zchunk;
+  int4* __restrict__ wvz_out = (int4*)(wgz + (((size_t)gxn * gyn + 1) & ~(size_t)1));
+  bool assumed = false;
+  float aR[9], at[3];
+  float eps_r = 0.0f, eps_t = 0.0f;
+  int azl = HSK_FT_EMPTY_LO, azh = -HSK_FT_EMPTY_LO;
+  int4 awv = make_int4(0, 0, 0, 0);
+  unsigned averdict = HSK_CF_MIXED, ac_now = 0u;
   double sums_in[16];
-  if (fin.slots && threadIdx.x < 64) shard_load27_wave(fin.slots + (size_t)((fin.iter + 2) % 3) * ICP_SLOT_DOUBLES, sums_in);
-  {
+  if (solves && !table_thread) shard_load27_wave(fin.slots + (size_t)((fin.iter + 2) % 3) * ICP_SLOT_DOUBLES, sums_in);
+  if (solves && !reporter && fp_block && ca.cflag != nullptr && zchunks <= 64) {
+    eps_r = slack->eps_r;
+    eps_t = slack->eps_t;
+    const IcpPose* __restrict__ pin = fin.pose_in;
+    assumed = eps_r > 0.0f && eps_t > 0.0f && !pin->lost;
+    if (assumed) {
+#pragma unroll
+      for (int k = 0; k < 9; ++k) aR[k] = pin->R[k];
+#pragma unroll
+      for (int k = 0; k < 3; ++k) at[k] = pin->t[k];
+    }
+  }
+  if (solves && !table_thread) {
+    shard_sum27_wave(sums_in, fin_tot);
+    IcpPose p = *fin.pose_in;
+    icp_solve_step(fin_tot, p);
+    if ((tid & 63) == 0) {
+      fin_pose = p;
+      if (blockIdx.x == 0) {
+        for (int k = 0; k < 27; ++k) st_out->sums[k] = fin_tot[k];
+        if (p.lost) {
+          st_out->lost = 1;
+          st_out->need_reset = 1;
+        } else {
+          for (int i = 0; i < 9; ++i) st_out->R[i] = p.R[i];
+          for (int i = 0; i < 3; ++i) st_out->t[i] = p.t[i];
+        }
+        st_out->n_iter = p.n_iter;
+      }
+      if (reporter) {
+        const unsigned n = *early.seq;
+        TrackState* dst = early.slots + early.slot_fifo[n % HSK_RING_FIFO];
+        const bool use_new = !p.lost;
+        for (int i = 0; i < 9; ++i) dst->R[i] = use_new ? p.R[i] : st->R[i];
+        for (int i = 0; i < 3; ++i) dst->t[i] = use_new ? p.t[i] : st->t[i];
+        for (int i = 0; i < 9; ++i) dst->Rp[i] = st->Rp[i];
+        for (int i = 0; i < 3; ++i) dst->tp[i] = st->tp[i];
+        dst->lost = p.lost ? 1 : st->lost;
+        dst->frame = st->frame;
+        dst->n_iter = p.n_iter;
+        dst->need_reset = p.lost ? 1 : st->need_reset;
+        for (int k = 0; k < 27; ++k) dst->sums[k] = fin_tot[k];
+        __threadfence_system();
+        __hip_atomic_store(&dst->pose_mark, (n + 1u) | 0x80000000u, __ATOMIC_RELEASE, __HIP_MEMORY_SCOPE_SYSTEM);
+      }
+    }
+  } else {
     if (blockIdx.x == 0)
-      for (int q = threadIdx.x; q < HSK_NQUEUES; q += blockDim.x) *(unsigned long long*)&qcount[q * HSK_QCOUNT_STRIDE] = 0ull;
-    const int i = blockIdx.x * blockDim.x + threadIdx.x;
+      for (int q = tid; q < HSK_NQUEUES; q += 256) *(unsigned long long*)&qcount[q * HSK_QCOUNT_STRIDE] = 0ull;
+    const int i = (int)blockIdx.x * 256 + tid;
     if (i < tw * th && (int)blockIdx.x < dil_blocks) {
       const int ty = i / tw, tx = i - ty * tw;
       float mx = 0.0f, mn = 1e30f;
@@ -169,90 +236,54 @@
         }
       dtab[i] = make_float2(mx, mn);
     }
-  }
-  if (fin.slots) {
-    if (threadIdx.x < 64) {
-      shard_sum27_wave(sums_in, fin_tot);
-      IcpPose p = *fin.pose_in;
-      icp_solve_step(fin_tot, p);
-      if (threadIdx.x == 0) {
-        fin_pose = p;
-        if (blockIdx.x == 0) {
-          for (int k = 0; k < 27; ++k) st_out->sums[k] = fin_tot[k];
-          if (p.lost) {
-            st_out->lost = 1;
-            st_out->need_reset = 1;
-          } else {
-            for (int i = 0; i < 9; ++i) st_out->R[i] = p.R[i];
-            for (int i = 0; i < 3; ++i) st_out->t[i] = p.t[i];
-          }
-          st_out->n_iter = p.n_iter;
+    {
+      if (assumed) {
+        const float D = hsk_ft_margin(vp.size, at, eps_r, eps_t);
+        int tlo = HSK_FT_EMPTY_LO, thi = -HSK_FT_EMPTY_LO;
+        if (col_ok) {
+          hsk_ft_column_range(vp, in, W, H, aR, at, x0, y, D, azl, azh);
+          hsk_ft_column_range(vp, in, W, H, aR, at, x0, y, -D, tlo, thi);
         }
-        if (early.slots && blockIdx.x == gridDim.x - 1) {
-          const unsigned n = *early.seq;
-          TrackState* dst = early.slots + early.slot_fifo[n % HSK_RING_FIFO];
-          const bool use_new = !p.lost;
-          for (int i = 0; i < 9; ++i) dst->R[i] = use_new ? p.R[i] : st->R[i];
-          for (int i = 0; i < 3; ++i) dst->t[i] = use_new ? p.t[i] : st->t[i];
-          for (int i = 0; i < 9; ++i) dst->Rp[i] = st->Rp[i];
-          for (int i = 0; i < 3; ++i) dst->tp[i] = st->tp[i];
-          dst->lost = p.lost ? 1 : st->lost;
-          dst->frame = st->frame;
-          dst->n_iter = p.n_iter;
-          dst->need_reset = p.lost ? 1 : st->need_reset;
-          for (int k = 0; k < 27; ++k) dst->sums[k] = fin_tot[k];
-          __threadfence_system();
-          __hip_atomic_store(&dst->pose_mark, (n + 1u) | 0x80000000u, __ATOMIC_RELEASE, __HIP_MEMORY_SCOPE_SYSTEM);
+        int lo = azl, hi = azh;
+        int lo_all = col_ok ? tlo : -0x7fffffff, hi_all = col_ok ? thi : 0x7fffffff;
+#pragma unroll
+        for (int o = 32; o > 0; o >>= 1) {
+          lo = min(lo, __shfl_xor(lo, o, 64));
+          hi = max(hi, __shfl_xor(hi, o, 64));
+          lo_all = max(lo_all, __shfl_xor(lo_all, o, 64));
+          hi_all = min(hi_all, __shfl_xor(hi_all, o, 64));
         }
-      }
-    }
+        awv = make_int4(lo, hi, lo_all, hi_all);
+        const int w = tid >> 6, zc = tid & 63;
+        if (zc < zchunks) {
+          const int zbeg = zc * ca.zchunk, zend = min(zbeg + ca.zchunk, vp.nzs);
+          const size_t ci = (((size_t)zc * gyn + fby) * gxn + fbx) * 4 + w;
+          ac_now = ca.cs != nullptr ? (unsigned)ca.cs[ci] : 0u;
+          const HskFtRange r = {lo, hi, lo_all, hi_all};
+          averdict = hsk_ft_chunk_verdict(vp, in, W, H, aR, at, fbx, fby, w, zbeg, zend, ca.zchunk, r, ca.sparse, tw, th, ca.free_thr, ca.cull_thr, D);
+        }
+      }
+    }
+  }
+  if (solves) {
     __syncthreads();
-    if (early.slots && blockIdx.x == gridDim.x - 1) return;
-  }
-  __shared__ int4 wv_sh[4];
-  const int ncol = vp.X / 4;
-  const int gxn = (vp.X + 63) / 64, gyn = (vp.Y + 15) / 16;
-  const bool fp_block = (int)blockIdx.x < gxn * gyn;
-  const int fby = (int)blockIdx.x / gxn, fbx = (int)blockIdx.x - fby * gxn;
-  const int y = fby * 16 + (int)((threadIdx.x & 63) >> 2), lc = fbx * 16 + (int)(threadIdx.x >> 6) * 4 + (int)(threadIdx.x & 3);
-  const bool col_ok = fp_block && y < vp.Y && lc < ncol;
-  const int x0 = lc * 4;
+    if (reporter) return;
+    const bool holds = assumed && !fin_pose.lost && hsk_ft_pose_within(fin_pose.R, fin_pose.t, aR, at, eps_r, eps_t);
+    if (holds) {
+      if (col_ok) zint[(size_t)y * ncol + lc] = make_int2(azl, azh);
+      if ((tid & 63) == 0 && table_thread) wvz_out[(size_t)blockIdx.x * 4 + (tid >> 6)] = awv;
+      const int w = tid >> 6, zc = tid & 63;
+      if (zc < zchunks && table_thread) coarse_store(ca, (((size_t)zc * gyn + fby) * gxn + fbx) * 4 + w, averdict, ac_now, false);
+      return;
+    }
+    if (blockIdx.x == 0 && tid == 0) slack->fallbacks += 1u;
+  }
   int zl = 0x7fffffff, zh = -0x7fffffff;
   if (col_ok) {
-    const bool own = fin.slots != nullptr && !fin_pose.lost;
+    const bool own = solves && !fin_pose.lost;
     const float* __restrict__ Rm = own ? fin_pose.R : st->R;
     const float* __restrict__ tm = own ? fin_pose.t : st->t;
-    const float tx = tm[0], ty = tm[1], tz = tm[2];
-    const float i00 = Rm[0], i01 = Rm[3], i02 = Rm[6];
-    const float i10 = Rm[1], i11 = Rm[4], i12 = Rm[7];
-    const float i20 = Rm[2], i21 = Rm[5], i22 = Rm[8];
-    const float gy = ((float)y + 0.5f) * vp.cell[1] - ty;
-    float glo = 1e30f, ghi = -1e30f;
-#pragma unroll
-    for (int j = 0; j < 4; ++j) {
-      const float gx = ((float)(x0 + j) + 0.5f) * vp.cell[0] - tx;
-      const float ax = i00 * gx + i01 * gy, ay = i10 * gx + i11 * gy, az = i20 * gx + i21 * gy;
-      float lo = -1e30f, hi = 1e30f;
-      clip_interval(az, i22, lo, hi);
-      const float ul = 1.5f + in.cx, uh = ((float)W + 0.5f) - in.cx;
-      const float vl = 1.5f + in.cy, vh = ((float)H + 0.5f) - in.cy;
-      clip_interval(ax * in.fx + ul * az, i02 * in.fx + ul * i22, lo, hi);
-      clip_interval(uh * az - ax * in.fx, uh * i22 - i02 * in.fx, lo, hi);
-      clip_interval(ay * in.fy + vl * az, i12 * in.fy + vl * i22, lo, hi);
-      clip_interval(vh * az - ay * in.fy, vh * i22 - i12 * in.fy, lo, hi);
-      if (lo <= hi) {
-        glo = fminf(glo, lo);
-        ghi = fmaxf(ghi, hi);
-      }
-    }
-    if (glo <= ghi) {
-      const float inv_cz = __builtin_amdgcn_rcpf(vp.cell[2]);
-      const float fl = (glo + tz) * inv_cz - 2.5f, fh = (ghi + tz) * inv_cz + 1.5f;
-      const int a = fl < -1e9f ? -1000000000 : (fl > 1e9f ? 1000000000 : (int)floorf(fl));
-      const int b = fh < -1e9f ? -1000000000 : (fh > 1e9f ? 1000000000 : (int)ceilf(fh));
-      zl = a - vp.zs0;
-      zh = b - vp.zs0;
-    }
+    hsk_ft_column_range(vp, in, W, H, Rm, tm, x0, y, 0.0f, zl, zh);
     zint[(size_t)y * ncol + lc] = make_int2(zl, zh);
   }
   if (fp_block) {
@@ -265,90 +296,25 @@
       lo_all = max(lo_all, __shfl_xor(lo_all, o, 64));
       hi_all = min(hi_all, __shfl_xor(hi_all, o, 64));
     }
-    if ((threadIdx.x & 63) == 0) {
-      ((int4*)(wgz + (((size_t)gxn * gyn + 1) & ~(size_t)1)))[(size_t)blockIdx.x * 4 + (threadIdx.x >> 6)] = make_int4(lo, hi, lo_all, hi_all);
-      wv_sh[threadIdx.x >> 6] = make_int4(lo, hi, lo_all, hi_all);
+    if ((tid & 63) == 0 && table_thread) {
+      wvz_out[(size_t)blockIdx.x * 4 + (tid >> 6)] = make_int4(lo, hi, lo_all, hi_all);
+      wv_sh[tid >> 6] = make_int4(lo, hi, lo_all, hi_all);
     }
     __syncthreads();
     if (ca.cflag != nullptr) {
-      const bool own = fin.slots != nullptr && !fin_pose.lost;
-      const bool lost = fin.slots != nullptr ? fin_pose.lost != 0 : st->lost != 0;
+      const bool own = solves && !fin_pose.lost;
+      const bool lost = solves ? fin_pose.lost != 0 : st->lost != 0;
       const float* __restrict__ Rm = own ? fin_pose.R : st->R;
       const float* __restrict__ tm = own ? fin_pose.t : st->t;
-      const int zchunks = (vp.nzs + ca.zchunk - 1) / ca.zchunk;
-      const int tw16 = tw;
-      for (int item = threadIdx.x; item < 4 * zchunks; item += blockDim.x) {
+      for (int item = table_thread ? tid : 4 * zchunks; item < 4 * zchunks; item += 256) {
         const int w = item & 3, zc = item >> 2;
-        const int4 r = wv_sh[w];
+        const int4 r4 = wv_sh[w];
+        const HskFtRange r = {r4.x, r4.y, r4.z, r4.w};
         const int zbeg = zc * ca.zchunk, zend = min(zbeg + ca.zchunk, vp.nzs);
         const size_t ci = (((size_t)zc * gyn + fby) * gxn + fbx) * 4 + w;
         const unsigned c_now = ca.cs != nullptr ? (unsigned)ca.cs[ci] : 0u;
-        unsigned verdict = HSK_CF_MIXED;
-        if ((zbeg > r.y) | (zend - 1 < r.x)) {
-          verdict = HSK_CF_SKIP;
-        } else {
-          const int xa = fbx * 64 + w * 16, ya = fby * 16;
-          const int xb = min(xa + 15, vp.X - 1), yb = min(ya + 15, vp.Y - 1);
-          const bool full = (xa + 15 < vp.X) & (ya + 15 < vp.Y) & (zbeg + vp.zchunk <= vp.nzs) & (ca.zchunk == vp.zchunk);
-          const float g0[3] = {((float)xa + 0.5f) * vp.cell[0] - tm[0], ((float)ya + 0.5f) * vp.cell[1] - tm[1],
-                               ((float)(vp.zs0 + zbeg) + 0.5f) * vp.cell[2] - tm[2]};
-          const float g1[3] = {((float)xb + 0.5f) * vp.cell[0] - tm[0], ((float)yb + 0.5f) * vp.cell[1] - tm[1],
-                               ((float)(vp.zs0 + zend - 1) + 0.5f) * vp.cell[2] - tm[2]};
-          float umin = 1e30f, umax = -1e30f, vmin = 1e30f, vmax = -1e30f, zmn = 1e30f;
-#pragma unroll
-          for (int c = 0; c < 8; ++c) {
-            const float gx = (c & 1) ? g1[0] : g0[0], gy = (c & 2) ? g1[1] : g0[1], gz = (c & 4) ? g1[2] : g0[2];
-            const float cxm = (Rm[0] * gx + Rm[3] * gy) + Rm[6] * gz, cym = (Rm[1] * gx + Rm[4] * gy) + Rm[7] * gz;
-            const float czm = (Rm[2] * gx + Rm[5] * gy) + Rm[8] * gz;
-            const float rq = __builtin_amdgcn_rcpf(czm);
-            const float uq = (cxm * in.fx) * rq + in.cx, vq = (cym * in.fy) * rq + in.cy;
-            zmn = fminf(zmn, czm);
-            umin = fminf(umin, uq);
-            umax = fmaxf(umax, uq);
-            vmin = fminf(vmin, vq);
-            vmax = fmaxf(vmax, vq);
-          }
-          if (zmn > 0.05f) {
-            umin -= 1.0f; vmin -= 1.0f; umax += 1.0f; vmax += 1.0f;
-            float d_hi2 = 0.0f, d_lo2 = 0.0f;
-#pragma unroll
-            for (int a = 0; a < 3; ++a) {
-              const float p0 = g0[a] * g0[a], p1 = g1[a] * g1[a];
-              d_hi2 += fmaxf(p0, p1);
-              d_lo2 += (g0[a] <= 0.0f && g1[a] >= 0.0f) ? 0.0f : fminf(p0, p1);
-            }
-            const float d_hi = __builtin_amdgcn_sqrtf(d_hi2), d_lo = __builtin_amdgcn_sqrtf(d_lo2);
-            const bool in_img = (umin >= 0.0f) & (vmin >= 0.0f) & (umax <= (float)(W - 1)) & (vmax <= (float)(H - 1));
-            const bool off_img = (umax < 0.0f) | (vmax < 0.0f) | (umin > (float)(W - 1)) | (vmin > (float)(H - 1));
-            if (off_img) {
-              verdict = HSK_CF_SKIP;
-            } else {
-              const int tu0 = (int)fminf(fmaxf(umin, 0.0f), (float)(W - 1)) >> 4, tu1 = (int)fminf(fmaxf(umax, 0.0f), (float)(W - 1)) >> 4;
-              const int tv0 = (int)fminf(fmaxf(vmin, 0.0f), (float)(H - 1)) >> 4, tv1 = (int)fminf(fmaxf(vmax, 0.0f), (float)(H - 1)) >> 4;
-              const int nx = tu1 - tu0 + 1, ny = tv1 - tv0 + 1;
-              if ((nx <= (2 << (HSK_SPARSE_LEVELS - 1))) & (ny <= (2 << (HSK_SPARSE_LEVELS - 1)))) {
-                const int kx = min(31 - __clz(nx), HSK_SPARSE_LEVELS - 1), ky = min(31 - __clz(ny), HSK_SPARSE_LEVELS - 1);
-                const float2* __restrict__ lv = ca.sparse + (size_t)(ky * HSK_SPARSE_LEVELS + kx) * tw16 * th;
-                const int ub = tu1 - (1 << kx) + 1, vb = tv1 - (1 << ky) + 1;
-                const float2 q00 = lv[tv0 * tw16 + tu0], q01 = lv[tv0 * tw16 + ub], q10 = lv[vb * tw16 + tu0], q11 = lv[vb * tw16 + ub];
-                const float Dx = fmaxf(fmaxf(q00.x, q01.x), fmaxf(q10.x, q11.x)), Dn = fminf(fminf(q00.y, q01.y), fminf(q10.y, q11.y));
-                const bool dead = d_lo * 0.99999f - Dx > ca.cull_thr;
-                const bool in_all = (r.z <= zbeg) & (r.w >= zend - 1);
-                const bool fre = full & in_img & in_all & (d_hi * 1.00001f + ca.free_thr <= Dn);
-                verdict = dead ? HSK_CF_SKIP : (fre ? HSK_CF_FREE : HSK_CF_MIXED);
-              }
-            }
-          }
-        }
-        if (verdict == HSK_CF_FREE && ca.cs != nullptr && !lost) {
-          const unsigned c = c_now;
-          if (c >= 1u && c < 255u) {
-            ca.cs[ci] = (unsigned char)(c + 1u);
-            ca.cs[ca.dirty_off + ci] = 1;
-            verdict = HSK_CF_SKIP;
-          }
-        }
-        ca.cflag[ci] = (unsigned char)verdict;
+        const unsigned verdict = hsk_ft_chunk_verdict(vp, in, W, H, Rm, tm, fbx, fby, w, zbeg, zend, ca.zchunk, r, ca.sparse, tw, th, ca.free_thr, ca.cull_thr, 0.0f);
+        coarse_store(ca, ci, verdict, c_now, lost);
       }
     }
   }
@@ -1141,7 +1107,7 @@
 
 void launch_integrate(hipStream_t s, void* vol, const float* scaled, const TrackState* st, const VolParams& vp, int W,
                       int H, Intr in, bool count_only, unsigned long long* counter, unsigned* flags,
-                      const float* tmax, int2* zint, unsigned* queue, const IcpFinal* icp_final, unsigned char* uni, const RingOut* early) {
+                      const float* tmax, int2* zint, unsigned* queue, const IcpFinal* icp_final, unsigned char* uni, const RingOut* early, TableSlack* slack) {
   const int zchunk = vp.nzs >= vp.zchunk ? vp.zchunk : vp.nzs;
   const int zchunks = (vp.nzs + zchunk - 1) / zchunk;
   const int tw = (W + HSK_TILE - 1) / HSK_TILE, th = (H + HSK_TILE - 1) / HSK_TILE;
@@ -1162,9 +1128,9 @@
   const CoarseArgs ca = {cflag, (count_only || uni == nullptr) ? nullptr : uni + hsk_lane_sum_bytes(vp), sparse, (unsigned)hsk_chunk_bytes_padded(vp), zchunk, kc.free_thr2, kc.cull_thr2};
   const RingOut quiet_ring = {nullptr, nullptr, nullptr};
   const RingOut early_ring = (early && fin.slots && !count_only) ? *early : quiet_ring;
-  hipLaunchKernelGGL(k_column_zrange, dim3((col_blocks > dil_blocks ? col_blocks : dil_blocks) + (early_ring.slots ? 1 : 0)), dim3(256), 0, s, fin, tmax,
+  hipLaunchKernelGGL(k_column_zrange, dim3((col_blocks > dil_blocks ? col_blocks : dil_blocks) + (early_ring.slots ? 1 : 0)), dim3(fin.slots ? 320 : 256), 0, s, fin, tmax,
                      tmax + tw * th, (float2*)(tmax + 2 * tw * th), tw, th, dil_blocks, qcount, st, vp, W, H, in, zint,
-                     const_cast<TrackState*>(st), wgz, early_ring, ca);
+                     const_cast<TrackState*>(st), wgz, early_ring, ca, slack);
   dim3 block(64, 4, 1);
   const dim3 grid((vp.X + 63) / 64, (vp.Y + 15) / 16, zchunks);
   const float2* dil = (const float2*)(tmax + 2 * tw * th);
diff --git a/housescan_amd/kinfu.py b/housescan_amd/kinfu.py
--- a/housescan_amd/kinfu.py
+++ b/housescan_amd/kinfu.py
@@ -157,6 +157,14 @@
         n = C.c_uint64()
         self._ck(self.lib.hsk_submit_host_us(self.h, us, C.byref(n), int(reset)))
         return list(us), n.value
+
+    def debug_set_table_slack(self, scale):
+        self._ck(self.lib.hsk_debug_set_table_slack(self.h, float(scale)))
+
+    def debug_table_fallbacks(self):
+        n = C.c_uint64()
+        self._ck(self.lib.hsk_debug_table_fallbacks(self.h, C.byref(n)))
+        return n.value
 
     def integrate_light_entries(self):
         n = C.c_uint64()
diff --git a/include/hskinfu.h b/include/hskinfu.h
--- a/include/hskinfu.h
+++ b/include/hskinfu.h
@@ -254,6 +254,8 @@
 int hsk_stage_ms(hsk_ctx* k, double sum_ms[HSK_NSTAGES], uint64_t* n_frames, int reset);
 int hsk_icp_level_ms(hsk_ctx* k, double sum_ms[HSK_LEVELS]);
 int hsk_submit_host_us(hsk_ctx* k, double sum_us[4], uint64_t* n_submissions, int reset);
+int hsk_debug_set_table_slack(hsk_ctx* k, float scale);
+int hsk_debug_table_fallbacks(hsk_ctx* k, uint64_t* n_fallbacks);
 int hsk_integrate_queue_entries(hsk_ctx* k, uint64_t* n_entries);
 int hsk_integrate_light_entries(hsk_ctx* k, uint64_t* n_entries);
 int hsk_integrate_coarse_counts(hsk_ctx* k, uint64_t counts[4]);
```

Measured after the change: 4373. 0.959x the previous value.
